# fpthink/3D-WSIS

Hardware: AMD Instinct MI355X
Metric: scenes/sec fwd+bwd ScanNet 2cm (~150k voxels) @1/8 GPU; HBM GB/s vs roofline (higher is better)
Workload: dtype f32; 1 GPU; C2: 1 synthetic ScanNet-shaped scene on 1 GPU, 2 cm voxels, fwd+bwd+AdamW step (SubMConv3d UNet 32..160 + ECC GNN + edge affinity + MultiTaskLoss); per-batch segment CSRs / edge graph and all rulebooks are rebuilt inside every step; active_voxels=153685, points=199790, superpoints=2289, edges=20054, scenes_per_gpu=1, global_batch=1, parallelism=scene-sharded dp1

## Files before the change

### 3d-wsis_amd/csrc/bn.hip

```cpp
#include <cstdlib>
#include <initializer_list>

#include "common.h"

using namespace wsis;

namespace {

constexpr int BN_ROWS_PER_THREAD = 8;
__host__ __device__ inline int bn_rows_per_wg(int Cp) {
  const int G = Cp >> 2;
  const int R = 256 / G > 1 ? 256 / G : 1;
  return R * BN_ROWS_PER_THREAD;
}
constexpr int BN_THREADS = 256;

struct f4 {
  float v[4];
};
template <typename T>
__device__ __forceinline__ float4 bn_ld4(const T* p, int64_t t) {
  if constexpr (sizeof(T) == 4) {
    return reinterpret_cast<const float4*>(p)[t];
  } else {
// ... 510 lines not shown
}

template <bool COHERENT, typename TI = float, typename TO = float>
__device__ __forceinline__ void bn_apply_body(const TI* __restrict__ x, const float* mean,
                                              const float* var, const float* __restrict__ gamma,
                                              const float* __restrict__ beta, float eps, int relu,
                                              TO* __restrict__ y, int64_t M, int C) {
  const int64_t total = M * C;
  if ((C & 3) == 0) {
    const int64_t total4 = total >> 2;
    const unsigned C4 = (unsigned)(C >> 2);
    const int64_t stride = (int64_t)gridDim.x * blockDim.x;
    int64_t t = blockIdx.x * (int64_t)blockDim.x + threadIdx.x;
    const bool fixed_c = (stride % C4) == 0;
    unsigned cg = (unsigned)(t % C4);
    float sc[4], mu[4], bt[4];
    auto coef = [&](unsigned g) {
#pragma unroll
      for (int e = 0; e < 4; ++e) {
        const int c = (int)g * 4 + e;
        sc[e] = bn_fwd_coef(gamma ? gamma[c] : 1.0f, bn_ld_stat<COHERENT>(var + c), eps);
        mu[e] = bn_ld_stat<COHERENT>(mean + c);
        bt[e] = beta ? beta[c] : 0.0f;
      }
    };
    coef(cg);
    auto body = [&](const float4 v) {
      float o[4] = {v.x, v.y, v.z, v.w};
#pragma unroll
      for (int e = 0; e < 4; ++e) o[e] = bn_fwd_elem(o[e], mu[e], sc[e], bt[e], relu);
      return make_float4(o[0], o[1], o[2], o[3]);
    };
    if (fixed_c) {
      for (; t + stride < total4; t += 2 * stride) {
        const float4 v0 = bn_ld4(x, t);
        const float4 v1 = bn_ld4(x, t + stride);
        bn_st4(y, t, body(v0));
        bn_st4(y, t + stride, body(v1));
      }
      if (t < total4) bn_st4(y, t, body(bn_ld4(x, t)));
    } else {
      for (; t < total4; t += stride) {
        cg = (unsigned)(t % C4);
        coef(cg);
        bn_st4(y, t, body(bn_ld4(x, t)));
      }
    }
  } else {
    for (int64_t t = blockIdx.x * (int64_t)blockDim.x + threadIdx.x; t < total;
         t += (int64_t)gridDim.x * blockDim.x) {
      const int c = (int)(t % C);
      const float sc = bn_fwd_coef(gamma ? gamma[c] : 1.0f, bn_ld_stat<COHERENT>(var + c), eps);
      y[t] = (TO)bn_fwd_elem((float)x[t], bn_ld_stat<COHERENT>(mean + c), sc, beta ? beta[c] : 0.0f, relu);
    }
  }
}

__global__ void bn_apply_kernel(const float* __restrict__ x, const float* __restrict__ mean,
                                const float* __restrict__ var, const float* __restrict__ gamma,
                                const float* __restrict__ beta, float eps, int relu, float* __restrict__ y,
                                int64_t M, int C) {
  bn_apply_body<false>(x, mean, var, gamma, beta, eps, relu, y, M, C);
}

template <typename TI, typename TO>
__global__ void bn_apply_lp_kernel(const TI* __restrict__ x, const float* __restrict__ mean,
                                   const float* __restrict__ var, const float* __restrict__ gamma,
                                   const float* __restrict__ beta, float eps, int relu, TO* __restrict__ y, int64_t M,
                                   int C) {
  bn_apply_body<false, TI, TO>(x, mean, var, gamma, beta, eps, relu, y, M, C);
}

template <typename TI>
void launch_bn_apply_lp(const void* x, const float* mean, const float* var, const float* gamma, const float* beta,
                        float eps, int relu, void* y, int out_fp32, int64_t M, int C, int grid, hipStream_t st) {
  if (out_fp32)
    hipLaunchKernelGGL((bn_apply_lp_kernel<TI, float>), dim3(grid), dim3(256), 0, st, static_cast<const TI*>(x), mean,
                       var, gamma, beta, eps, relu, static_cast<float*>(y), M, C);
  else
    hipLaunchKernelGGL((bn_apply_lp_kernel<TI, TI>), dim3(grid), dim3(256), 0, st, static_cast<const TI*>(x), mean, var,
                       gamma, beta, eps, relu, static_cast<TI*>(y), M, C);
}

template <bool COHERENT, typename T, typename TO>
__device__ __forceinline__ void bn_bwd_apply_body(const T* __restrict__ x, const T* __restrict__ dy,
                                                  const float* __restrict__ mean, const float* __restrict__ var,
                                                  const float* __restrict__ gamma, const float* __restrict__ beta,
                                                  const float* dgamma, const float* dbeta,
                                                  const T* __restrict__ addend, float eps, int relu, int training,
                                                  TO* __restrict__ dx, int64_t M, int C) {
  const int64_t total = M * C;
  const float inv_m = 1.0f / (float)M;
  const bool vec = (C & 3) == 0;
  const int W = vec ? 4 : 1;
  const int64_t totalw = total / W;
  const unsigned Cw = (unsigned)(C / W);
  const int64_t stride = (int64_t)gridDim.x * blockDim.x;
  int64_t t = blockIdx.x * (int64_t)blockDim.x + threadIdx.x;
  const bool fixed_c = (stride % Cw) == 0;
  BnBwdCoef k;
  float k1[4], k2[4];
  auto coef = [&](int c0) {
#pragma unroll
    for (int e = 0; e < 4; ++e) {
      if (e < W) {
        const int c = c0 + e;
        k.load(e, c, mean, var, gamma, beta, eps);
        k1[e] = training ? bn_ld_stat<COHERENT>(dbeta + c) * inv_m : 0.0f;
        k2[e] = training ? bn_ld_stat<COHERENT>(dgamma + c) * inv_m : 0.0f;
      }
    }
  };
  if (t < totalw) coef((int)(t % Cw) * W);
  auto one = [&](const float (&xv)[4], const float (&dv)[4], const float (&av)[4], float (&ov)[4]) {
#pragma unroll
    for (int e = 0; e < 4; ++e) {
      if (e < W)
        ov[e] = bn_bwd_dx(bn_bwd_elem(xv[e], dv[e], k, e, relu), k, e, k1[e], k2[e], training, addend != nullptr, av[e]);
    }
  };
  if (vec && fixed_c) {
    for (; t + stride < totalw; t += 2 * stride) {
      const int64_t u = t + stride;
      const f4 tx0 = ld4(x + t * 4, true), td0 = ld4(dy + t * 4, true);
      const f4 tx1 = ld4(x + u * 4, true), td1 = ld4(dy + u * 4, true);
      f4 ta0, ta1;
#pragma unroll
      for (int e = 0; e < 4; ++e) ta0.v[e] = ta1.v[e] = 0.f;
      if (addend) {
        ta0 = ld4(addend + t * 4, true);
        ta1 = ld4(addend + u * 4, true);
      }
      float o0[4], o1[4];
      one(tx0.v, td0.v, ta0.v, o0);
      one(tx1.v, td1.v, ta1.v, o1);
      bn_st4(dx, t, make_float4(o0[0], o0[1], o0[2], o0[3]));
      bn_st4(dx, u, make_float4(o1[0], o1[1], o1[2], o1[3]));
    }
  }
  for (; t < totalw; t += stride) {
    if (!fixed_c) coef((int)(t % Cw) * W);
    float xv[4], dv[4], av[4] = {0.f, 0.f, 0.f, 0.f}, ov[4];
    if (vec) {
      const f4 tx = ld4(x + t * 4, true), td = ld4(dy + t * 4, true);
#pragma unroll
      for (int e = 0; e < 4; ++e) {
        xv[e] = tx.v[e];
        dv[e] = td.v[e];
      }
      if (addend) {
        const f4 ta = ld4(addend + t * 4, true);
#pragma unroll
        for (int e = 0; e < 4; ++e) av[e] = ta.v[e];
      }
    } else {
      xv[0] = (float)x[t];
      dv[0] = (float)dy[t];
      if (addend) av[0] = (float)addend[t];
    }
    one(xv, dv, av, ov);
    if (vec)
      bn_st4(dx, t, make_float4(ov[0], ov[1], ov[2], ov[3]));
    else
      dx[t] = (TO)ov[0];
  }
}

template <typename T, typename TO>
__global__ void bn_bwd_apply_kernel(const T* __restrict__ x, const T* __restrict__ dy,
                                    const float* __restrict__ mean, const float* __restrict__ var,
                                    const float* __restrict__ gamma, const float* __restrict__ beta,
                                    const float* __restrict__ dgamma, const float* __restrict__ dbeta,
                                    const T* __restrict__ addend, float eps, int relu, int training,
                                    TO* __restrict__ dx, int64_t M, int C) {
  bn_bwd_apply_body<false>(x, dy, mean, var, gamma, beta, dgamma, dbeta, addend, eps, relu, training, dx, M, C);
}

constexpr int BN_SF_ROWS = 256;

template <int NT>
__device__ __forceinline__ void bn_small_totals(const float* __restrict__ partial, int nblk, int C, int64_t M, int G, int c,
                                                bool own, double (&red)[NT][8][33], double (&T)[NT]) {
#pragma unroll
  for (int k = 0; k < NT; ++k) T[k] = 0.0;
  for (int g = 0; g < G; ++g) {
    int lo, hi;
    bn_chunk_range(nblk, G, g, lo, hi);
    double t[NT], Tg[NT];
#pragma unroll
    for (int k = 0; k < NT; ++k) t[k] = 0.0;
    bn_chunk_walk<NT>(partial, lo, hi, C, M, c, t);
    if (g) __syncthreads();
    bn_lane_fold<NT>(t, own, red, Tg);
    if (own) {
#pragma unroll
      for (int k = 0; k < NT; ++k) {
        if (G == 1)
          T[k] = Tg[k];
        else
          T[k] += Tg[k];
      }
    }
  }
}

__global__ __launch_bounds__(256) void bn_small_finish_apply_kernel(
    const float* __restrict__ partial, int nblk, int C, int64_t M, float* __restrict__ mean, float* __restrict__ var,
    float* __restrict__ running_mean, float* __restrict__ running_var, float momentum, const float* __restrict__ x,
    const float* __restrict__ gamma, const float* __restrict__ beta, float eps, int relu, float* __restrict__ y, int G) {
  __shared__ double red[3][8][33];
  __shared__ float s_mu[32], s_sc[32], s_bt[32];
  const int cgi = blockIdx.y;
  const int cl = threadIdx.x & 31;
  const int c = cgi * 32 + cl;
  const bool own = (threadIdx.x >> 5) == 0 && c < C;
  double T[3];
  bn_small_totals<3>(partial, nblk, C, M, G, c, own, red, T);
  if (own) {
    const BnMeanVar s = bn_centred_mean_var(T[0], T[1], T[2], M);
    if (blockIdx.x == 0) bn_store_stats(s, M, c, mean, var, running_mean, running_var, momentum);
    s_mu[cl] = (float)s.mu;
    s_sc[cl] = bn_fwd_coef(gamma ? gamma[c] : 1.0f, (float)s.v, eps);
    s_bt[cl] = beta ? beta[c] : 0.0f;
  }
  __syncthreads();
  const int q4 = threadIdx.x & 7, rl = threadIdx.x >> 3;
  const int c4 = cgi * 32 + q4 * 4;
  if (c4 >= C) return;
  float mu4[4], sc4[4], bt4[4];
#pragma unroll
  for (int e = 0; e < 4; ++e) {
    mu4[e] = s_mu[q4 * 4 + e];
    sc4[e] = s_sc[q4 * 4 + e];
    bt4[e] = s_bt[q4 * 4 + e];
  }
  const int64_t r0 = (int64_t)blockIdx.x * BN_SF_ROWS;
#pragma unroll 4
  for (int it = 0; it < BN_SF_ROWS / 32; ++it) {
    const int64_t r = r0 + it * 32 + rl;
    if (r < M) {
      const float4 vx = *reinterpret_cast<const float4*>(x + r * C + c4);
      float o[4] = {vx.x, vx.y, vx.z, vx.w};
#pragma unroll
      for (int e = 0; e < 4; ++e) o[e] = bn_fwd_elem(o[e], mu4[e], sc4[e], bt4[e], relu);
      *reinterpret_cast<float4*>(y + r * C + c4) = make_float4(o[0], o[1], o[2], o[3]);
    }
  }
}

__global__ __launch_bounds__(256) void bn_small_bwd_finish_apply_kernel(
    const float* __restrict__ partial, int nblk, int C, int64_t M, const float* __restrict__ x,
    const float* __restrict__ dy, const float* __restrict__ mean, const float* __restrict__ var,
    const float* __restrict__ gamma, const float* __restrict__ beta, const float* __restrict__ addend, float eps, int relu,
    float* __restrict__ dx, float* __restrict__ dgamma, float* __restrict__ dbeta, int G) {
  __shared__ double red[2][8][33];
  __shared__ float s_k1[32], s_k2[32];
  const int cgi = blockIdx.y;
  const int cl = threadIdx.x & 31;
  const int c = cgi * 32 + cl;
  const bool own = (threadIdx.x >> 5) == 0 && c < C;
  double T[2];
  bn_small_totals<2>(partial, nblk, C, M, G, c, own, red, T);
  if (own) {
    const float db = (float)T[0], dg = (float)T[1];
    if (blockIdx.x == 0) {
      dbeta[c] = db;
      dgamma[c] = dg;
    }
    const float inv_m = 1.0f / (float)M;
    s_k1[cl] = db * inv_m;
    s_k2[cl] = dg * inv_m;
  }
  __syncthreads();
  const int q4 = threadIdx.x & 7, rl = threadIdx.x >> 3;
  const int c4 = cgi * 32 + q4 * 4;
  if (c4 >= C) return;
  BnBwdCoef k;
  float k1[4], k2[4];
#pragma unroll
  for (int e = 0; e < 4; ++e) {
    k.load(e, c4 + e, mean, var, gamma, beta, eps);
    k1[e] = s_k1[q4 * 4 + e];
    k2[e] = s_k2[q4 * 4 + e];
  }
  const int64_t r0 = (int64_t)blockIdx.x * BN_SF_ROWS;
#pragma unroll 2
  for (int it = 0; it < BN_SF_ROWS / 32; ++it) {
    const int64_t r = r0 + it * 32 + rl;
    if (r < M) {
      const float4 vx = *reinterpret_cast<const float4*>(x + r * C + c4);
      const float4 vd = *reinterpret_cast<const float4*>(dy + r * C + c4);
      float4 va = make_float4(0.f, 0.f, 0.f, 0.f);
      if (addend) va = *reinterpret_cast<const float4*>(addend + r * C + c4);
      const float xv[4] = {vx.x, vx.y, vx.z, vx.w}, dv[4] = {vd.x, vd.y, vd.z, vd.w}, av[4] = {va.x, va.y, va.z, va.w};
      float ov[4];
#pragma unroll
      for (int e = 0; e < 4; ++e)
        ov[e] = bn_bwd_dx(bn_bwd_elem(xv[e], dv[e], k, e, relu), k, e, k1[e], k2[e], 1, addend != nullptr, av[e]);
      *reinterpret_cast<float4*>(dx + r * C + c4) = make_float4(ov[0], ov[1], ov[2], ov[3]);
    }
  }
}

static int bn_small_gmax() {
  const char* e = getenv("WSIS_BN_SMALL_G");
  const int g = e ? atoi(e) : 4;
  return g < 1 ? 1 : g > 8 ? 8 : g;
}
static bool bn_small_fused_on() {
  const char* e = getenv("WSIS_BN_SMALL_FUSED");
  return !e || atoi(e) != 0;
}

int bn_nblk(int64_t M, int Cp) { return (int)ceil_div(M > 0 ? M : 1, (int64_t)bn_rows_per_wg(Cp)); }

#if WSIS_EXPERIMENTAL
constexpr int BN_POLL_SLEEP = 12;
constexpr unsigned long long BN_SPIN_LIMIT = 200000000ull;

__device__ __forceinline__ void bn_wait_published(SyncSlot* s) {
  if (threadIdx.x == 0) {
    const unsigned long long t0 = __builtin_amdgcn_s_memrealtime();
    while (__hip_atomic_load(&s->flag, __ATOMIC_RELAXED, __HIP_MEMORY_SCOPE_AGENT) == 0u) {
      __builtin_amdgcn_s_sleep(BN_POLL_SLEEP);
      if (__builtin_amdgcn_s_memrealtime() - t0 > BN_SPIN_LIMIT) {
        __hip_atomic_store(&s->err, 1u, __ATOMIC_RELAXED, __HIP_MEMORY_SCOPE_AGENT);
        break;
      }
    }
    const unsigned l = atomicAdd(&s->left, 1u);
    if (l == gridDim.x - 1) {
      __hip_atomic_store(&s->left, 0u, __ATOMIC_RELAXED, __HIP_MEMORY_SCOPE_AGENT);
      __hip_atomic_store(&s->flag, 0u, __ATOMIC_RELAXED, __HIP_MEMORY_SCOPE_AGENT);
    }
  }
  __syncthreads();
}
__device__ __forceinline__ void bn_publish(bool fin, SyncSlot* s, int CG) {
  if (!fin) return;
  __threadfence();
  __syncthreads();
  if (threadIdx.x == 0) {
    const unsigned d = atomicAdd(&s->done, 1u);
    if (d == (unsigned)CG - 1) {
      __hip_atomic_store(&s->done, 0u, __ATOMIC_RELAXED, __HIP_MEMORY_SCOPE_AGENT);
      __threadfence();
      __hip_atomic_store(&s->flag, 1u, __ATOMIC_RELEASE, __HIP_MEMORY_SCOPE_AGENT);
    }
  }
}

__global__ __launch_bounds__(256) void bn_finalize_apply_kernel(
    const float* __restrict__ partial, int nblk, int C, int64_t M, double* __restrict__ chunk, int G,
    float* mean, float* var, float* __restrict__ running_mean,
    float* __restrict__ running_var, float momentum, SyncSlot* __restrict__ sync, const float* __restrict__ x,
    const float* __restrict__ gamma, const float* __restrict__ beta, float eps, int relu, float* __restrict__ y) {
  __shared__ double red[3][8][33];
  __shared__ int s_last;
  const int CG = (C + 31) / 32;
  if ((int)blockIdx.x < G * CG)
    bn_publish(bn_chunk_centred_stage(partial, nblk, C, M, chunk, mean, var, running_mean, running_var, momentum,
                                      sync->ticket, (int)blockIdx.x % G, G, (int)blockIdx.x / G, red, s_last),
               sync, CG);
  bn_wait_published(sync);
  bn_apply_body<true>(x, mean, var, gamma, beta, eps, relu, y, M, C);
}

__global__ __launch_bounds__(256) void bn_bwd_finish_apply_kernel(
    const float* __restrict__ partial, int nblk, int C, double* __restrict__ chunk, int G, float* dbeta, float* dgamma,
    SyncSlot* __restrict__ sync, const float* __restrict__ x, const float* __restrict__ dy, const float* __restrict__ mean,
    const float* __restrict__ var, const float* __restrict__ gamma, const float* __restrict__ beta,
    const float* __restrict__ addend, float eps, int relu, float* __restrict__ dx, int64_t M) {
  __shared__ double red[2][8][33];
  __shared__ int s_last;
  const int CG = (C + 31) / 32;
  if ((int)blockIdx.x < G * CG)
    bn_publish(bn_sum_chunk_stage(partial, nblk, C, chunk, dbeta, dgamma, sync->ticket, (int)blockIdx.x % G, G,
                                  (int)blockIdx.x / G, red, s_last),
               sync, CG);
  bn_wait_published(sync);
  bn_bwd_apply_body<true>(x, dy, mean, var, gamma, beta, dgamma, dbeta, addend, eps, relu, 1, dx, M, C);
}

static int bn_fused_grid(int64_t M, int C, int need_chunk_wgs, int which = 0) {
  const char* e = getenv("WSIS_BN_FUSED_APPLY");
  const int on = e ? atoi(e) : 0;
  const char* ed = getenv(which ? "WSIS_BN_FUSED_BWD" : "WSIS_BN_FUSED_FWD");
  const int on_dir = ed ? atoi(ed) : on;
  const char* g = tune_env("WSIS_BN_FUSED_GRID");
  int gmax = g ? atoi(g) : 256;
  if (gmax < 64 || gmax > 512) gmax = 256;
  int n_cu = 0;
  {
    int dev = 0, v = 0;
    n_cu = (hipGetDevice(&dev) == hipSuccess &&
            hipDeviceGetAttribute(&v, hipDeviceAttributeMultiprocessorCount, dev) == hipSuccess) ? v : 0;
  }
  if (!on_dir || (C & 3) != 0) return 0;
  const int cw = C >> 2;
  const int64_t work = (M * C) >> 2;
  int gcap = (work > 600000 && gmax == 256) ? 512 : gmax;
  if (gcap > 2 * n_cu) gcap = 2 * n_cu;
  if (gcap < 1) return 0;
  int grid = gcap - (gcap % cw);
  const int need = grid_for(work, 256);
  if (need < grid) {
    grid = need;
    if (grid > cw) grid -= grid % cw;
  }
  return (grid >= need_chunk_wgs && grid >= 1) ? grid : 0;
}
#endif


static int bn_apply_grid(int64_t M, int C) {
  const bool vec = (C & 3) == 0;
  const int64_t work = vec ? (M * C) >> 2 : M * C;
  const int cw = vec ? C >> 2 : C;
  int64_t g = ceil_div(work, (int64_t)256 * 8);
  if (g < 512) {
    g = ceil_div(work, 256);
    if (g > 512) g = 512;
  }
  if (g > 16384) g = 16384;
  if (g < 1) g = 1;
  if (g > cw) g -= g % cw;
  return (int)g;
}

template <typename T, typename TO>
static int launch_bn_bwd_apply(const T* d_x, const T* d_dy, const float* d_mean, const float* d_var,
                               const float* d_gamma, const float* d_beta, const float* d_dgamma, const float* d_dbeta,
                               const T* d_addend, float eps, int relu, int training, TO* d_dx, int64_t M, int C,
                               hipStream_t st) {
  hipLaunchKernelGGL((bn_bwd_apply_kernel<T, TO>), dim3(bn_apply_grid(M, C)), dim3(256), 0, st, d_x, d_dy, d_mean, d_var,
                     d_gamma, d_beta, d_dgamma, d_dbeta, d_addend, eps, relu, training, d_dx, M, C);
  WSIS_LAUNCH_CHECK();
  return WSIS_OK;
}

template <typename T>
static int bn_stats_run(const T* d_x, int64_t M, int C, float* d_mean, float* d_var, float* d_running_mean,
                        float* d_running_var, float momentum, void* d_ws, hipStream_t st) {
  const int Cp = (C + 3) / 4 * 4;
  const int nblk = bn_nblk(M, Cp);
  float* partial = static_cast<float*>(d_ws);
  WSIS_REQUIRE(Cp / 4 <= BN_THREADS, "C > 1024 is not supported");
  if (M <= bn_small_rows()) {
    hipLaunchKernelGGL(bn_stats_small_kernel<T>, dim3(Cp / 4), dim3(BN_SMALL_THREADS), 0, st, d_x, M, C, d_mean, d_var,
                       d_running_mean, d_running_var, momentum);
    WSIS_LAUNCH_CHECK();
    return WSIS_OK;
  }
  hipLaunchKernelGGL(bn_stats_partial_kernel<T>, dim3(nblk), dim3(BN_THREADS), 0, st, d_x, M, C, Cp, partial);
  WSIS_LAUNCH_CHECK();
  hipLaunchKernelGGL(bn_stats_final_kernel<T>, dim3(C), dim3(64), 0, st, partial, nblk, C, Cp, M, d_x, d_mean, d_var,
                     d_running_mean, d_running_var, momentum);
  WSIS_LAUNCH_CHECK();
  return WSIS_OK;
}
template <typename T>
static int bn_bwd_reduce_run(const T* d_x, const T* d_dy, const float* d_mean, const float* d_var, const float* d_gamma,
                             const float* d_beta, float eps, int relu, float* d_dgamma, float* d_dbeta, int64_t M, int C,
                             void* d_ws, hipStream_t st) {
  const int Cp = (C + 3) / 4 * 4;
  const int nblk = bn_nblk(M, Cp);
  float* partial = static_cast<float*>(d_ws);
  WSIS_REQUIRE(Cp / 4 <= BN_THREADS, "C > 1024 is not supported");
  if (M <= bn_small_rows()) {
    hipLaunchKernelGGL(bn_bwd_small_kernel<T>, dim3(Cp / 4), dim3(BN_SMALL_THREADS), 0, st, d_x, d_dy, d_mean, d_var,
                       d_gamma, d_beta, eps, relu, M, C, d_dgamma, d_dbeta);
    WSIS_LAUNCH_CHECK();
  } else {
    hipLaunchKernelGGL(bn_bwd_partial_kernel<T>, dim3(nblk), dim3(BN_THREADS), 0, st, d_x, d_dy, d_mean, d_var, d_gamma,
                       d_beta, eps, relu, M, C, Cp, partial);
    WSIS_LAUNCH_CHECK();
    hipLaunchKernelGGL(bn_bwd_final_kernel, dim3(C), dim3(64), 0, st, partial, nblk, C, Cp, d_dgamma, d_dbeta);
    WSIS_LAUNCH_CHECK();
  }
  return WSIS_OK;
}
template <typename T>
static int bn_bwd_lp_run(const void* d_x, const void* d_dy, const float* d_mean, const float* d_var, const float* d_gamma,
                         const float* d_beta, float eps, int relu, int training, void* d_dx, int out_fp32,
                         float* d_dgamma, float* d_dbeta, const void* d_addend, int64_t M, int C, void* d_ws,
                         hipStream_t st) {
  const T *x = static_cast<const T*>(d_x), *dy = static_cast<const T*>(d_dy), *ad = static_cast<const T*>(d_addend);
  const int rc = bn_bwd_reduce_run(x, dy, d_mean, d_var, d_gamma, d_beta, eps, relu, d_dgamma, d_dbeta, M, C, d_ws, st);
  if (rc != WSIS_OK || !d_dx) return rc;
  if (out_fp32)
    return launch_bn_bwd_apply(x, dy, d_mean, d_var, d_gamma, d_beta, d_dgamma, d_dbeta, ad, eps, relu, training,
                               static_cast<float*>(d_dx), M, C, st);
  return launch_bn_bwd_apply(x, dy, d_mean, d_var, d_gamma, d_beta, d_dgamma, d_dbeta, ad, eps, relu, training,
                             static_cast<T*>(d_dx), M, C, st);
}

static unsigned* bn_tickets(void* d_sync) {
  static const int on = [] {
    const char* e = tune_env("WSIS_BN_TICKET");
    return e ? atoi(e) : 1;
  }();
  if (!on || !d_sync) return nullptr;
  return static_cast<SyncSlot*>(d_sync)->ticket;
}

static bool bn_aligned16(std::initializer_list<const void*> ps) {
  for (const void* p : ps)
    if (reinterpret_cast<uintptr_t>(p) & 15) return false;
  return true;
}
static void* bn_align256(void* p) {
  return reinterpret_cast<void*>((reinterpret_cast<uintptr_t>(p) + 255) & ~(uintptr_t)255);
}

struct BnCentredPlan {
  int G, CG;
  bool ws_ok;
  double* chunk;
  unsigned* tickets;
};
static BnCentredPlan bn_centred_plan(int64_t n_part, int C, void* d_ws, int64_t ws_bytes, void* d_sync) {
  BnCentredPlan p;
  p.G = bn_fin_chunks(n_part);
  p.CG = (C + 31) / 32;
  p.ws_ok = p.G == 1 || (d_ws && ws_bytes >= wsis_bn_stats_finalize_workspace_bytes(n_part, C));
  p.chunk = static_cast<double*>(bn_align256(d_ws));
  p.tickets = bn_tickets(d_sync);
  return p;
}
static bool bn_small_fused_ok(const BnCentredPlan& p, int C, std::initializer_list<const void*> rows) {
  return p.G <= bn_small_gmax() && (p.G == 1 || p.tickets) && (C & 3) == 0 && bn_small_fused_on() && bn_aligned16(rows);
}

}

extern "C" {

int64_t wsis_bn_workspace_bytes(int64_t M, int32_t C) {
  if (M < 0 || C < 1) return -1;
  const int64_t Cp = (C + 3) / 4 * 4;
  return (int64_t)bn_nblk(M, (int)Cp) * 2 * Cp * (int64_t)sizeof(float) + 256;
}

int wsis_bn_stats(const float* d_x, int64_t M, int32_t C, float* d_mean, float* d_var, float* d_running_mean,
                  float* d_running_var, float momentum, void* d_ws, int64_t ws_bytes, void* stream) {
  WSIS_REQUIRE(M >= 1 && C >= 1 && d_x && d_mean && d_var && d_ws, "bad args");
  WSIS_REQUIRE(ws_bytes >= wsis_bn_workspace_bytes(M, C), "workspace too small");
  WSIS_REQUIRE((d_running_mean == nullptr) == (d_running_var == nullptr), "running stats come in pairs");
  return bn_stats_run(d_x, M, C, d_mean, d_var, d_running_mean, d_running_var, momentum, d_ws, as_stream(stream));
}

static bool bn_lp_domain(int C, int dtype, std::initializer_list<const void*> ps) {
  return (dtype == 0 || dtype == 1) && C % 8 == 0 && C <= 1024 && bn_aligned16(ps);
}

int wsis_bn_stats_lp(const void* d_x, int64_t M, int32_t C, float* d_mean, float* d_var, float* d_running_mean,
                     float* d_running_var, float momentum, void* d_ws, int64_t ws_bytes, int32_t dtype, void* stream) {
  WSIS_REQUIRE(M >= 1 && C >= 1 && d_x && d_mean && d_var && d_ws, "bad args");
  WSIS_REQUIRE(bn_lp_domain(C, dtype, {d_x}), "16-bit BatchNorm: dtype 0 / 1, C % 8 == 0, C <= 1024, 16-byte aligned x");
  WSIS_REQUIRE(ws_bytes >= wsis_bn_workspace_bytes(M, C), "workspace too small");
  WSIS_REQUIRE((d_running_mean == nullptr) == (d_running_var == nullptr), "running stats come in pairs");
  hipStream_t st = as_stream(stream);
  if (dtype == 0)
    return bn_stats_run(static_cast<const __bf16*>(d_x), M, C, d_mean, d_var, d_running_mean, d_running_var, momentum,
                        d_ws, st);
  return bn_stats_run(static_cast<const _Float16*>(d_x), M, C, d_mean, d_var, d_running_mean, d_running_var, momentum,
                      d_ws, st);
}


__device__ __forceinline__ void colsum_block(const bool IN, const bool OUT, const float* __restrict__ x, int64_t lo,
                                             int64_t hi, int C4, float4* red, float* __restrict__ out) {
  const int RL = 256 / C4;
  const int cl = threadIdx.x % C4, rl = threadIdx.x / C4;
  float4 a = {0.f, 0.f, 0.f, 0.f};
  if (rl < RL) {
    const float4* x4 = reinterpret_cast<const float4*>(x);
#pragma unroll 8
    for (int64_t r = lo + rl; r < hi; r += RL) {
      float4 v;
      if (IN) {
        const float* p = x + (r * C4 + cl) * 4;
        v = make_float4(ld_sc1(p), ld_sc1(p + 1), ld_sc1(p + 2), ld_sc1(p + 3));
      } else {
        v = x4[r * C4 + cl];
      }
      a.x += v.x;
      a.y += v.y;
      a.z += v.z;
      a.w += v.w;
    }
    red[rl * C4 + cl] = a;
  }
  __syncthreads();
  if (threadIdx.x < C4) {
// ... 63 lines not shown
  const BnCentredPlan p = bn_centred_plan(n_part, C, d_ws, ws_bytes, d_sync);
  WSIS_REQUIRE(p.ws_ok, "workspace too small");
  WSIS_REQUIRE(C <= 512, "more than 512 channels");
  hipLaunchKernelGGL(bn_stats_chunk_centred_kernel, dim3(p.G, p.CG), dim3(256), 0, as_stream(stream), d_partials,
                     (int)n_part, C, M, p.chunk, d_mean, d_var, d_running_mean, d_running_var, momentum, p.tickets);
  WSIS_LAUNCH_CHECK();
  if (p.G > 1 && !p.tickets) {
    hipLaunchKernelGGL(bn_stats_final_centred_kernel, dim3((C + 3) / 4), dim3(256), 0, as_stream(stream), p.chunk, p.G, C,
                       M, d_mean, d_var, d_running_mean, d_running_var, momentum);
    WSIS_LAUNCH_CHECK();
  }
  return WSIS_OK;
}

int wsis_bn_stats_finalize_apply(const float* d_partials, int64_t n_part, int64_t M, int32_t C, float* d_mean,
                                 float* d_var, float* d_running_mean, float* d_running_var, float momentum,
                                 const float* d_x, const float* d_gamma, const float* d_beta, float eps, int32_t relu,
                                 float* d_y, void* d_ws, int64_t ws_bytes, void* d_sync, void* stream) {
  WSIS_REQUIRE(n_part >= 1 && M >= 1 && C >= 1 && d_partials && d_mean && d_var && d_x && d_y, "bad args");
  WSIS_REQUIRE(n_part == (M + 31) / 32 && n_part < ((int64_t)1 << 31), "one partial per 32-row slice");
  WSIS_REQUIRE(C <= 512, "more than 512 channels");
  hipStream_t st = as_stream(stream);
  const BnCentredPlan p = bn_centred_plan(n_part, C, d_ws, ws_bytes, d_sync);
  WSIS_REQUIRE(p.ws_ok, "workspace too small");
  if (bn_small_fused_ok(p, C, {d_x, d_y})) {
    hipLaunchKernelGGL(bn_small_finish_apply_kernel, dim3((unsigned)ceil_div(M, BN_SF_ROWS), (unsigned)p.CG), dim3(256), 0,
                       st, d_partials, (int)n_part, (int)C, M, d_mean, d_var, d_running_mean, d_running_var, momentum, d_x,
                       d_gamma, d_beta, eps, (int)relu, d_y, p.G);
    WSIS_LAUNCH_CHECK();
    return WSIS_OK;
  }
#if WSIS_EXPERIMENTAL
  if (const int grid = p.tickets ? bn_fused_grid(M, C, p.G * p.CG) : 0) {
    hipLaunchKernelGGL(bn_finalize_apply_kernel, dim3(grid), dim3(256), 0, st, d_partials, (int)n_part, (int)C, M, p.chunk,
                       p.G, d_mean, d_var, d_running_mean, d_running_var, momentum, static_cast<SyncSlot*>(d_sync), d_x,
                       d_gamma, d_beta, eps, (int)relu, d_y);
    WSIS_LAUNCH_CHECK();
    return WSIS_OK;
  }
#endif
  const int rc = wsis_bn_stats_finalize(d_partials, n_part, M, C, d_mean, d_var, d_running_mean, d_running_var, momentum,
                                        d_ws, ws_bytes, d_sync, stream);
  if (rc != WSIS_OK) return rc;
  return wsis_bn_apply(d_x, d_mean, d_var, d_gamma, d_beta, eps, relu, d_y, M, C, stream);
}

int wsis_bn_apply(const float* d_x, const float* d_mean, const float* d_var, const float* d_gamma,
                  const float* d_beta, float eps, int32_t relu, float* d_y, int64_t M, int32_t C, void* stream) {
  WSIS_REQUIRE(M >= 0 && C >= 1, "bad sizes");
  if (M == 0) return WSIS_OK;
  WSIS_REQUIRE(d_x && d_mean && d_var && d_y, "null pointer");
  hipLaunchKernelGGL(bn_apply_kernel, dim3(bn_apply_grid(M, C)), dim3(256), 0, as_stream(stream), d_x, d_mean, d_var,
                     d_gamma, d_beta, eps, relu, d_y, M, C);
  WSIS_LAUNCH_CHECK();
  return WSIS_OK;
}

int wsis_bn_apply_lp(const void* d_x, const float* d_mean, const float* d_var, const float* d_gamma,
                     const float* d_beta, float eps, int32_t relu, void* d_y, int32_t out_fp32, int64_t M, int32_t C,
                     int32_t dtype, void* stream) {
  WSIS_REQUIRE(M >= 0 && C >= 1, "bad sizes");
  WSIS_REQUIRE(dtype == 0 || dtype == 1, "dtype must be 0 (bf16) or 1 (fp16)");
  if (M == 0) return WSIS_OK;
  WSIS_REQUIRE(d_x && d_mean && d_var && d_y, "null pointer");
  const int grid = bn_apply_grid(M, C);
  if ((C & 3) == 0)
    WSIS_REQUIRE((reinterpret_cast<uintptr_t>(d_x) & 7) == 0 &&
                     (reinterpret_cast<uintptr_t>(d_y) & (out_fp32 ? 15 : 7)) == 0,
                 "x and y must be aligned to a quad of elements");
  hipStream_t st = as_stream(stream);
  if (dtype == 0)
    launch_bn_apply_lp<__bf16>(d_x, d_mean, d_var, d_gamma, d_beta, eps, relu, d_y, out_fp32, M, C, grid, st);
  else
    launch_bn_apply_lp<_Float16>(d_x, d_mean, d_var, d_gamma, d_beta, eps, relu, d_y, out_fp32, M, C, grid, st);
  WSIS_LAUNCH_CHECK();
  return WSIS_OK;
}

int wsis_bn_bwd_from_partials(const float* d_partials, int64_t n_part, const float* d_x, const float* d_dy,
                              const float* d_mean, const float* d_var, const float* d_gamma, const float* d_beta,
                              float eps, int32_t relu, float* d_dx, float* d_dgamma, float* d_dbeta,
                              const float* d_addend, int64_t M, int32_t C, void* d_ws, int64_t ws_bytes, void* d_sync,
                              void* stream) {
  WSIS_REQUIRE(M >= 1 && C >= 1 && d_partials && d_x && d_dy && d_mean && d_var && d_dgamma && d_dbeta, "bad args");
  WSIS_REQUIRE(n_part == (M + 31) / 32 && n_part < ((int64_t)1 << 31), "one partial per 32-row slice");
  const BnCentredPlan p = bn_centred_plan(n_part, C, d_ws, ws_bytes, d_sync);
  WSIS_REQUIRE(p.ws_ok, "workspace too small");
  hipStream_t st = as_stream(stream);
  WSIS_REQUIRE(C <= 512, "more than 512 channels");
  if (d_dx && bn_small_fused_ok(p, C, {d_x, d_dy, d_dx, d_addend})) {
    hipLaunchKernelGGL(bn_small_bwd_finish_apply_kernel, dim3((unsigned)ceil_div(M, BN_SF_ROWS), (unsigned)p.CG), dim3(256),
                       0, st, d_partials, (int)n_part, (int)C, M, d_x, d_dy, d_mean, d_var, d_gamma, d_beta, d_addend, eps,
                       (int)relu, d_dx, d_dgamma, d_dbeta, p.G);
    WSIS_LAUNCH_CHECK();
    return WSIS_OK;
  }
#if WSIS_EXPERIMENTAL
  if (const int grid = d_dx && p.tickets ? bn_fused_grid(M, C, p.G * p.CG, 1) : 0) {
    hipLaunchKernelGGL(bn_bwd_finish_apply_kernel, dim3(grid), dim3(256), 0, st, d_partials, (int)n_part, (int)C, p.chunk,
                       p.G, d_dbeta, d_dgamma, static_cast<SyncSlot*>(d_sync), d_x, d_dy, d_mean, d_var, d_gamma, d_beta,
                       d_addend, eps, (int)relu, d_dx, M);
    WSIS_LAUNCH_CHECK();
    return WSIS_OK;
  }
#endif
  hipLaunchKernelGGL(bn_sum_chunk_kernel, dim3(p.G, p.CG), dim3(256), 0, st, d_partials, (int)n_part, C, p.chunk, d_dbeta,
                     d_dgamma, p.tickets);
  WSIS_LAUNCH_CHECK();
  if (p.G > 1 && !p.tickets) {
    hipLaunchKernelGGL(bn_sum_final_kernel, dim3((C + 3) / 4), dim3(256), 0, st, p.chunk, p.G, C, d_dbeta, d_dgamma);
    WSIS_LAUNCH_CHECK();
  }
  if (!d_dx) return WSIS_OK;
  return launch_bn_bwd_apply(d_x, d_dy, d_mean, d_var, d_gamma, d_beta, d_dgamma, d_dbeta, d_addend, eps, relu, 1, d_dx, M,
                             C, st);
}

int wsis_bn_bwd_apply(const float* d_x, const float* d_dy, const float* d_mean, const float* d_var,
                      const float* d_gamma, const float* d_beta, const float* d_sum_dz_xhat, const float* d_sum_dz,
                      float eps, int32_t relu, float* d_dx, const float* d_addend, int64_t M, int32_t C, void* stream) {
  WSIS_REQUIRE(M >= 1 && C >= 1 && d_x && d_dy && d_mean && d_var && d_sum_dz_xhat && d_sum_dz && d_dx, "bad args");
  return launch_bn_bwd_apply(d_x, d_dy, d_mean, d_var, d_gamma, d_beta, d_sum_dz_xhat, d_sum_dz, d_addend, eps, relu, 1,
                             d_dx, M, C, as_stream(stream));
}

int wsis_bn_bwd(const float* d_x, const float* d_dy, const float* d_mean, const float* d_var,
                const float* d_gamma, const float* d_beta, float eps, int32_t relu, int32_t training,
                float* d_dx, float* d_dgamma, float* d_dbeta, const float* d_addend, int64_t M, int32_t C, void* d_ws,
                int64_t ws_bytes, void* stream) {
  WSIS_REQUIRE(M >= 1 && C >= 1 && d_x && d_dy && d_mean && d_var && d_dgamma && d_dbeta && d_ws, "bad args");
  WSIS_REQUIRE(ws_bytes >= wsis_bn_workspace_bytes(M, C), "workspace too small");
  hipStream_t st = as_stream(stream);
  const int rc = bn_bwd_reduce_run(d_x, d_dy, d_mean, d_var, d_gamma, d_beta, eps, relu, d_dgamma, d_dbeta, M, C, d_ws, st);
  if (rc != WSIS_OK || !d_dx) return rc;
  return launch_bn_bwd_apply(d_x, d_dy, d_mean, d_var, d_gamma, d_beta, d_dgamma, d_dbeta, d_addend, eps, relu, training,
                             d_dx, M, C, st);
}

int wsis_bn_bwd_lp(const void* d_x, const void* d_dy, const float* d_mean, const float* d_var, const float* d_gamma,
                   const float* d_beta, float eps, int32_t relu, int32_t training, void* d_dx, int32_t out_fp32,
                   float* d_dgamma, float* d_dbeta, const void* d_addend, int64_t M, int32_t C, int32_t dtype, void* d_ws,
                   int64_t ws_bytes, void* stream) {
  WSIS_REQUIRE(M >= 1 && C >= 1 && d_x && d_dy && d_mean && d_var && d_dgamma && d_dbeta && d_ws, "bad args");
  WSIS_REQUIRE(bn_lp_domain(C, dtype, {d_x, d_dy, d_dx, d_addend}),
               "16-bit BatchNorm: dtype 0 / 1, C % 8 == 0, C <= 1024, 16-byte aligned tensors");
  WSIS_REQUIRE(ws_bytes >= wsis_bn_workspace_bytes(M, C), "workspace too small");
  hipStream_t st = as_stream(stream);
  if (dtype == 0)
    return bn_bwd_lp_run<__bf16>(d_x, d_dy, d_mean, d_var, d_gamma, d_beta, eps, relu, training, d_dx, out_fp32, d_dgamma,
                                 d_dbeta, d_addend, M, C, d_ws, st);
  return bn_bwd_lp_run<_Float16>(d_x, d_dy, d_mean, d_var, d_gamma, d_beta, eps, relu, training, d_dx, out_fp32, d_dgamma,
                                 d_dbeta, d_addend, M, C, d_ws, st);
}

int64_t wsis_sync_bytes(void) { return (int64_t)kSyncSlotsTotal * (int64_t)sizeof(SyncSlot); }

int64_t wsis_colsum_workspace_bytes(int64_t M, int32_t C) {
  if (M < 0 || C < 4) return -1;
  int64_t per, G;
  colsum_plan(M, &per, &G);
  return (G > 1 ? G : 1) * (int64_t)C * (int64_t)sizeof(float) + 256;
}

int wsis_colsum(const float* d_x, int64_t M, int32_t C, float* d_out, void* d_ws, int64_t ws_bytes, void* d_sync,
                void* stream) {
  WSIS_REQUIRE(M >= 0 && C >= 4 && C % 4 == 0 && C <= 1024 && d_out, "colsum: C must be a multiple of 4, <= 1024");
  hipStream_t st = as_stream(stream);
  if (M == 0) {
    WSIS_HIP_CHECK(hipMemsetAsync(d_out, 0, sizeof(float) * (size_t)C, st));
    return WSIS_OK;
  }
  WSIS_REQUIRE(d_x && bn_aligned16({d_x, d_out}), "colsum: 16-byte alignment");
  int64_t per, G;
  colsum_plan(M, &per, &G);
  float* chunk = nullptr;
  unsigned* ticket = nullptr;
  if (G > 1) {
    WSIS_REQUIRE(d_ws && ws_bytes >= wsis_colsum_workspace_bytes(M, C), "workspace too small");
    chunk = static_cast<float*>(bn_align256(d_ws));
    WSIS_REQUIRE(d_sync, "colsum over more than one chunk needs a sync slot");
    ticket = static_cast<SyncSlot*>(d_sync)->ticket;
  }
  hipLaunchKernelGGL(colsum_kernel, dim3((unsigned)G), dim3(256), 0, st, d_x, M, (int)C, per, chunk, d_out, ticket);
  WSIS_LAUNCH_CHECK();
  return WSIS_OK;
}

}
```

### 3d-wsis_amd/csrc/common.h

```cpp
#pragma once
#include <hip/hip_runtime.h>
#include <hip/hip_ext.h>
#include <cstdlib>

#include <cstdint>
#include <cstdio>
#include <string>
#include <vector>

#include "../../include/wsis_hip.h"

namespace wsis {
inline const char* tune_env(const char* name) {
#if WSIS_EXPERIMENTAL
  return getenv(name);
#else
  (void)name;
  return nullptr;
#endif
}
inline int tune_int(const char* name, int dflt) {
  const char* e = tune_env(name);
  return e ? atoi(e) : dflt;
}
// ... 59 lines not shown
  void bracket() {
    if (exact && stage == 1) {
      exact = false;
      stage = hipEventRecord(r.a, st) == hipSuccess ? 1 : 0;
    }
  }
  hipEvent_t ka() const { return (exact && stage == 1) ? r.a : nullptr; }
  hipEvent_t kb() const { return (exact && stage == 1) ? r.b : nullptr; }
  void stop() {
    if (stage == 1) {
      if (!exact) (void)hipEventRecord(r.b, st);
      stage = 2;
    }
  }
  void tail() {
    if (stage == 2 && hipEventCreate(&r.c) == hipSuccess) (void)hipEventRecord(r.c, st);
  }
  ~ProfScope() {
    if (stage == 2) g_prof[which].push_back(r);
  }
};


#ifdef __HIPCC__
__device__ __forceinline__ void st_sc1(float* p, float v) { __hip_atomic_store(p, v, __ATOMIC_RELAXED, __HIP_MEMORY_SCOPE_AGENT); }
__device__ __forceinline__ void st_sc1(double* p, double v) { __hip_atomic_store(p, v, __ATOMIC_RELAXED, __HIP_MEMORY_SCOPE_AGENT); }
__device__ __forceinline__ float ld_sc1(const float* p) {
  return __hip_atomic_load(const_cast<float*>(p), __ATOMIC_RELAXED, __HIP_MEMORY_SCOPE_AGENT);
}
__device__ __forceinline__ double ld_sc1(const double* p) {
  return __hip_atomic_load(const_cast<double*>(p), __ATOMIC_RELAXED, __HIP_MEMORY_SCOPE_AGENT);
}
__device__ __forceinline__ void wait_stores_left() { asm volatile("s_waitcnt vmcnt(0)" ::: "memory"); }
#endif

struct SyncSlot {
  unsigned ticket[16];
  unsigned done, flag, left, err;
  unsigned ctr[44];
  unsigned fin[960];
};
static_assert(sizeof(SyncSlot) == 4096, "sync slot layout");
constexpr int kSyncSlots = 64;
constexpr int kSyncSlotsTotal = kSyncSlots + 1;
inline SyncSlot* sync_slot(void* d_sync, int i) {
  return d_sync ? static_cast<SyncSlot*>(d_sync) + (i % kSyncSlots) : nullptr;
}
inline void* deep_sync_slot(void* d_sync) { return d_sync ? static_cast<SyncSlot*>(d_sync) + kSyncSlots : nullptr; }

struct BnMeanVar {
  double mu, v;
};
__device__ __forceinline__ void bn_store_stats(BnMeanVar s, int64_t M, int c, float* mean, float* var, float* running_mean,
                                               float* running_var, float momentum) {
  const double n = (double)M;
  mean[c] = (float)s.mu;
  var[c] = (float)s.v;
  if (running_mean) {
    const double unb = n > 1 ? s.v * n / (n - 1) : s.v;
    running_mean[c] = (float)((1.0 - momentum) * running_mean[c] + momentum * s.mu);
    running_var[c] = (float)((1.0 - momentum) * running_var[c] + momentum * unb);
  }
}
__device__ __forceinline__ BnMeanVar bn_centred_mean_var(double S, double Q, double W, int64_t M) {
  const double n = (double)M;
  const double mu = S / n;
  double v = (Q + (W - n * mu * mu)) / n;
  if (v < 0.0) v = 0.0;
  return {mu, v};
}
__device__ __forceinline__ void bn_finish_centred(double S, double Q, double W, int64_t M, int c, float* mean, float* var,
                                                  float* running_mean, float* running_var, float momentum) {
  bn_store_stats(bn_centred_mean_var(S, Q, W, M), M, c, mean, var, running_mean, running_var, momentum);
}

constexpr int kBnFinChunks = 64;
inline int bn_fin_chunks(int64_t n_part) {
  int64_t g = n_part / 64;
  if (g < 1) g = 1;
  if (g > kBnFinChunks) g = kBnFinChunks;
  return (int)g;
}

bool spconv_in_supported(int K, int Cin, int Cout);
int spconv_in_launch(const float* d_X, const int32_t* d_nbr, const int32_t* d_order, const float* d_W, const float* d_bias,
                     const float* d_residual, float* d_out, int64_t M_out, hipEvent_t ka, hipEvent_t kb, hipStream_t st);

int64_t spconv_in_dw_workspace_bytes(int64_t M_out);
int spconv_in_dw_launch(const float* d_X, const int32_t* d_nbr, const int32_t* d_order, const float* d_dY, float* d_dW,
                        int64_t M_out, void* d_ws, hipEvent_t ka, hipEvent_t kb, hipStream_t st);

int spconv_ring_plan(int64_t M_out, int K, int Cin, int Cout);
int spconv_ring_launch(int nt, const float* d_X, const int32_t* d_nbr, const int32_t* d_order, const float* d_WT, int flip,
                       const float* d_bias, const float* d_residual, float* d_out, float* d_stats, const void* epi,
                       unsigned* d_err, int64_t M_in, int64_t M_out, int K, int Cin, int Cout, hipEvent_t ka, hipEvent_t kb, hipStream_t st,
                       unsigned long long* d_dbg = nullptr);

bool dw2_supported(int K, int Cin, int Cout);
bool dw2_fits(int64_t M_in, int64_t M_out, int K, int Cin, int Cout);
int64_t dw2_workspace_bytes(int64_t M_out, int K, int Cin, int Cout);
void dw2_set_batch_rows(int64_t rows);
int64_t dw2_batch_rows();
struct DwRedRec {
  const float* partial = nullptr;
  float* dW = nullptr;
  int64_t total4 = 0;
  int32_t P = 0;
};
void dw2_set_defer(DwRedRec* slot);
int dw2_reduce_batch(const DwRedRec* recs, int n, hipStream_t st);
int dw2_launch(const float* d_X, const int32_t* d_nbr, const int32_t* d_order, const float* d_dY, float* d_dW,
               int64_t M_in, int64_t M_out, int K, int Cin, int Cout, void* d_ws, hipStream_t st);
int dw2_launch_swapped(const float* d_X, const float* d_mean, const float* d_var, const float* d_gamma, const float* d_beta,
                       float eps, int relu, const int32_t* d_nbr_b, const int32_t* d_order_b, int flip, const float* d_dY,
                       float* d_dW, int64_t M_in, int64_t M_out, int K, int Cin, int Cout, void* d_ws, hipStream_t st);

#ifdef __HIPCC__
struct RowCol {
  int64_t row;
  int col;
};
__device__ __forceinline__ RowCol row_col(int64_t t, int C, int64_t total) {
  RowCol rc;
  if ((C & (C - 1)) == 0) {
    const int sh = __ffs(C) - 1;
    rc.row = t >> sh;
    rc.col = (int)(t & (C - 1));
  } else if (total < ((int64_t)1 << 32)) {
    const uint32_t q = (uint32_t)t / (uint32_t)C;
    rc.row = q;
    rc.col = (int)((uint32_t)t - q * (uint32_t)C);
  } else {
    rc.row = t / C;
    rc.col = (int)(t - rc.row * C);
  }
  return rc;
}
#endif

constexpr int64_t kEmptyKey = -1;

__device__ __forceinline__ uint64_t mix64(uint64_t x) {
  x ^= x >> 33;
  x *= 0xff51afd7ed558ccdULL;
  x ^= x >> 33;
  x *= 0xc4ceb9fe1a85ec53ULL;
  x ^= x >> 33;
  return x;
}

__device__ __forceinline__ int32_t hash_lookup(const int64_t* __restrict__ keys,
                                               const int32_t* __restrict__ vals, uint64_t mask,
                                               int64_t key) {
  uint64_t h = mix64((uint64_t)key) & mask;
  for (;;) {
    int64_t k = keys[h];
    if (k == key) return vals[h];
    if (k == kEmptyKey) return -1;
    h = (h + 1) & mask;
  }
}

}
```

### 3d-wsis_amd/csrc/executor.hip

```cpp
#include <condition_variable>
#include <cstdlib>
#include <deque>
#include <map>
#include <mutex>
#include <string>
#include <thread>
#include <utility>
#include <vector>

#include <unistd.h>

#include <algorithm>

#include "common.h"
#if WSIS_EXPERIMENTAL
#include "deep.h"
#endif

using namespace wsis;

namespace {

constexpr int64_t ALIGN = 256;
inline int64_t up(int64_t v) { return (v + ALIGN - 1) / ALIGN * ALIGN; }
// ... 191 lines not shown
    std::lock_guard<std::mutex> lock(mu_);
    const long pid = (long)getpid();
    if (started_ && pid_ != pid) {
      started_ = false;
      q_.clear();
      st_.clear();
    }
    if (!started_) {
      started_ = true;
      pid_ = pid;
      std::thread(&DwWorker::run, this).detach();
    }
    t.owner = std::this_thread::get_id();
    q_.push_back(t);
    ++st_[t.owner].pending;
    cv_.notify_one();
  }
  int drain(std::string* msg) {
    const std::thread::id me = std::this_thread::get_id();
    std::unique_lock<std::mutex> lock(mu_);
    done_.wait(lock, [&] { return st_[me].pending == 0; });
    State& s = st_[me];
    const int rc = s.err;
    if (rc != WSIS_OK && msg) *msg = s.msg;
    s.err = WSIS_OK;
    s.msg.clear();
    return rc;
  }

 private:
  struct State {
    int pending = 0, err = WSIS_OK;
    std::string msg;
  };
  void run() {
    for (;;) {
      DwTask t;
      {
        std::unique_lock<std::mutex> lock(mu_);
        cv_.wait(lock, [this] { return !q_.empty(); });
        t = q_.front();
        q_.pop_front();
      }
      int rc = WSIS_OK;
      std::string msg;
      hipError_t he = hipSetDevice(t.dev);
      if (he == hipSuccess && t.ev) he = hipStreamWaitEvent(t.side, t.ev, 0);
      if (he != hipSuccess) {
        rc = WSIS_ERR_HIP;
        msg = std::string("dW worker: ") + hipGetErrorString(he);
      } else {
        rc = t.flush ? dw2_reduce_batch(t.flush, t.flush_n, t.side) : issue_dw(t.op, t.ws, t.ws_bytes, t.side, t.rec);
        if (rc != WSIS_OK) msg = wsis_last_error();
      }
      std::lock_guard<std::mutex> lock(mu_);
      State& s = st_[t.owner];
      if (rc != WSIS_OK && s.err == WSIS_OK) {
        s.err = rc;
        s.msg = msg;
      }
      if (--s.pending == 0) done_.notify_all();
    }
  }
  std::mutex mu_;
  std::condition_variable cv_, done_;
  std::deque<DwTask> q_;
  std::map<std::thread::id, State> st_;
  bool started_ = false;
  long pid_ = 0;
};
DwWorker& dw_worker() {
  static DwWorker* w = new DwWorker();
  return *w;
}
struct PassOptions {
  bool fwd2;
  bool dw_stream;
  bool dw_thread;
  bool dw_batch_reduce;
  bool dw_tail_main;
  bool wt_side;
  bool dw_early;
  bool slab_bn_partials;
  bool prof;
  bool capturing;
  bool dw_defer() const { return dw_batch_reduce && !prof; }
};
inline bool env_flag(const char* e, bool dflt) { return e ? atoi(e) != 0 : dflt; }
PassOptions read_pass_options(const hipStream_t* st) {
  PassOptions o;
  o.fwd2 = env_flag(getenv("WSIS_FWD2"), true);
  o.dw_stream = env_flag(getenv("WSIS_DW_STREAM"), true);
  o.dw_thread = env_flag(tune_env("WSIS_DW_THREAD"), true);
  o.dw_batch_reduce = env_flag(getenv("WSIS_DW_BATCH_REDUCE"), false);
  o.dw_tail_main = env_flag(getenv("WSIS_DW_TAIL_MAIN"), true);
  o.wt_side = env_flag(getenv("WSIS_WT_SIDE"), true);
  const char* rows = getenv("WSIS_DW_EARLY_ROWS");
  o.dw_early = env_flag(getenv("WSIS_DW_EARLY"), dw2_batch_rows() < (rows ? atoll(rows) : 500000));
  o.slab_bn_partials = env_flag(getenv("WSIS_SLAB_BN_PARTIALS"), false);
  o.prof = g_prof_on;
  hipStreamCaptureStatus cs = hipStreamCaptureStatusNone;
  o.capturing = st && (hipStreamIsCapturing(*st, &cs) != hipSuccess || cs != hipStreamCaptureStatusNone);
  return o;
}
inline bool dw_tail_on_main(const wsis_op* ops, int n, int i) {
  return i == n - 1 && ops[i].kind == WSIS_OP_CONV_BWD && ops[i].out[1] && !ops[i].out[0];
}

inline int64_t wt_bytes_of(const wsis_op& op) {
  return up((int64_t)op.K * op.Cin * op.Cout * (int64_t)sizeof(float));
}

inline bool use_fwd2(const wsis_op& op, bool on) {
  const int64_t gathered = op.kind == WSIS_OP_CONV ? op.M_in * op.Cin : op.M_out * op.Cout;
  return on && wsis_spconv_fwd_t_supported(op.K, op.Cin, op.Cout) != 0 && gathered * 4 < ((int64_t)1 << 31);
}
inline bool needs_wt(const wsis_op& op, bool on) {
  if (op.flags & WSIS_OPF_LP) return false;
  if (op.kind == WSIS_OP_CONV) return use_fwd2(op, on);
  if (op.kind == WSIS_OP_CONV_BWD) return op.out[0] != nullptr && !use_fwd2(op, on);
  return false;
}

inline bool is_lp(const wsis_op& op) { return (op.flags & WSIS_OPF_LP) != 0; }
inline bool is_lp_conv(const wsis_op& op) {
  return is_lp(op) && (op.kind == WSIS_OP_CONV || (op.kind == WSIS_OP_CONV_BWD && op.out[0]));
}
inline int64_t lp_wt_bytes_of(const wsis_op& op) { return up((int64_t)op.K * op.Cin * op.Cout * 2); }
inline bool lp_below_2g(int64_t rows, int C) { return rows * C * 2 < ((int64_t)1 << 31); }
const char* lp_refusal(const wsis_op& op) {
  if (op.kind == WSIS_OP_CAST_LP && !is_lp(op)) return "CAST_LP without WSIS_OPF_LP (its dtype)";
  if (!is_lp(op)) return (op.flags & WSIS_OPF_LP_TRAIN) ? "WSIS_OPF_LP_TRAIN without WSIS_OPF_LP" : nullptr;
  const bool train_form = (op.kind == WSIS_OP_BN_RELU && (op.flags & WSIS_OPF_TRAINING)) || op.kind == WSIS_OP_BN_RELU_BWD ||
                          op.kind == WSIS_OP_CONV_BWD || op.kind == WSIS_OP_SPLIT;
  if (train_form && !(op.flags & WSIS_OPF_LP_TRAIN))
    return "16-bit training form (training BatchNorm, CONV_BWD, BN_RELU_BWD, SPLIT) without WSIS_OPF_LP_TRAIN";
  if (op.reserved != 0 && op.reserved != 1) return "16-bit op with a dtype other than 0 (bf16) or 1 (fp16)";
  if (op.flags & (WSIS_OPF_BN_IN | WSIS_OPF_STAT_FIN | WSIS_OPF_STATS))
    return "16-bit op with a fused BatchNorm form or epilogue statistics (16-bit passes run every BatchNorm as an op)";
  switch (op.kind) {
    case WSIS_OP_CONV:
      if (!wsis_spconv_lp_supported(op.K, op.Cin, op.Cout))
        return "16-bit convolution outside wsis_spconv_lp_supported (channels multiples of 32, at most 512)";
      if (op.M_in * op.Cin * 2 >= ((int64_t)1 << 31)) return "16-bit convolution input of 2 GiB or more";
      if (!op.in[3]) return "16-bit convolution without weights";
      return nullptr;
    case WSIS_OP_BN_RELU:
      if (!op.out[0]) return "16-bit BatchNorm without output";
      if (op.flags & WSIS_OPF_TRAINING) {
        if (!op.out[1] || !op.out[2]) return "16-bit training BatchNorm without mean / var outputs";
        if (op.Cin % 8 != 0 || op.Cin > 1024) return "16-bit training BatchNorm outside C % 8 == 0, C <= 1024";
        if ((op.flags & WSIS_OPF_UPDATE_RUNNING) && (!op.in[3] || !op.in[4]))
          return "16-bit BatchNorm updates running statistics it does not have";
        return nullptr;
      }
      if (op.flags & WSIS_OPF_UPDATE_RUNNING) return "16-bit evaluation BatchNorm with WSIS_OPF_UPDATE_RUNNING";
      if (!op.in[3] || !op.in[4]) return "16-bit evaluation BatchNorm without running statistics";
      return nullptr;
    case WSIS_OP_BN_RELU_BWD:
      if (op.Cin % 8 != 0 || op.Cin > 1024) return "16-bit BatchNorm backward outside C % 8 == 0, C <= 1024";
      if (!op.in[0] || !op.in[1] || !op.in[2] || !op.in[3] || !op.out[1] || !op.out[2])
        return "16-bit BatchNorm backward without x, dy, statistics or parameter-gradient outputs";
      return nullptr;
    case WSIS_OP_CAT:
    case WSIS_OP_SPLIT:
      if ((op.Cin | op.Cout) & 1) return "16-bit concatenation / split of an odd channel count";
      return nullptr;
    case WSIS_OP_CAST_LP:
      return nullptr;
    case WSIS_OP_CONV_BWD:
      if (!op.in[0] || !op.in[2]) return "16-bit backward convolution without X or dY";
      if (!lp_below_2g(op.M_out, op.Cout)) return "16-bit backward convolution with a dY of 2 GiB or more";
      if (op.out[0]) {
        if (!wsis_spconv_lp_supported(op.K, op.Cout, op.Cin))
          return "16-bit dIn product outside wsis_spconv_lp_supported (channels multiples of 32, at most 512)";
        if (!op.in[1]) return "16-bit dIn product without weights";
      }
      if (op.out[1] && (!wsis_spconv_lp_supported(op.K, op.Cin, op.Cout) || !lp_below_2g(op.M_in, op.Cin)))
        return "16-bit weight gradient outside wsis_spconv_lp_supported or with an input of 2 GiB or more";
      return nullptr;
    default:
      return "16-bit form of an op kind that has none";
  }
}

inline int64_t dw_ws_of(const wsis_op& op) {
  if (is_lp(op)) return up(wsis_spconv_dw_lp_workspace_bytes(op.M_out, op.K, op.Cin, op.Cout));
  if (op.flags & WSIS_OPF_BN_IN) return up(wsis_spconv_dw_bn_workspace_bytes(op.M_in, op.K, op.Cin, op.Cout));
  return up(wsis_spconv_dw_workspace_bytes(op.M_out, op.K, op.Cin, op.Cout));
}

int64_t op_ws_bytes(const wsis_op& op, bool on) {
  if (lp_refusal(op)) return -1;
  switch (op.kind) {
    case WSIS_OP_CONV:
      if (is_lp(op)) return up(wsis_spconv_fwd_lp_workspace_bytes(op.M_out, op.K, op.Cin, op.Cout));
#if WSIS_EXPERIMENTAL
      if (op.flags & (WSIS_OPF_BN_IN | WSIS_OPF_STAT_FIN))
        return up(std::max(wsis_spconv_fwd_f_workspace_bytes(op.M_out, op.K, op.Cin, op.Cout),
                           wsis_spconv_fwd_t_workspace_bytes(op.M_out, op.K, op.Cin, op.Cout)));
#else
      if (op.flags & (WSIS_OPF_BN_IN | WSIS_OPF_STAT_FIN)) return -1;
#endif
      if (use_fwd2(op, on)) return up(wsis_spconv_fwd_t_workspace_bytes(op.M_out, op.K, op.Cin, op.Cout));
      return up(wsis_spconv_fwd_workspace_bytes(op.M_out, op.K, op.Cin, op.Cout));
    case WSIS_OP_BN_RELU:
      if (!(op.flags & WSIS_OPF_TRAINING)) return 0;
      return up(std::max(wsis_bn_workspace_bytes(op.M_in, op.Cin),
                         wsis_bn_stats_finalize_workspace_bytes((op.M_in + 31) / 32, op.Cin)));
    case WSIS_OP_BN_RELU_BWD:
      return up(std::max(wsis_bn_workspace_bytes(op.M_in, op.Cin),
                         wsis_bn_stats_finalize_workspace_bytes((op.M_in + 31) / 32, op.Cin)));
    case WSIS_OP_CONV_BWD:
      if (!op.out[0]) return 0;
      if (is_lp(op)) return up(wsis_spconv_fwd_lp_workspace_bytes(op.M_in, op.K, op.Cout, op.Cin));
      if (use_fwd2(op, on)) return up(wsis_spconv_fwd_t_workspace_bytes(op.M_in, op.K, op.Cout, op.Cin));
      return up(wsis_spconv_fwd_workspace_bytes(op.M_in, op.K, op.Cout, op.Cin));
    default:
      return 0;
  }
}

inline int paired_bn(const wsis_op* ops, int n, int i) {
  const wsis_op& op = ops[i];
  for (int j = i + 1; j < n && j <= i + 4; ++j)
    if (ops[j].kind == WSIS_OP_BN_RELU_BWD && ops[j].in[1] == op.out[0] && (ops[j].flags & WSIS_OPF_STATS)) return j;
  return -1;
}

struct PassPlan {
  enum { LP, WT, DW, DEEP, OP, REGIONS };
  int64_t at[REGIONS], bytes[REGIONS], total = 0;
  std::vector<int64_t> lp_off, wt_off;
  int64_t dw_max = 0;
  int n_dw = 0;
};

struct PassRun {
  const wsis_op* ops;
  int n, mark_op;
  void *d_sync, *stream, *waiter_stream;
  hipStream_t st;
  PassOptions opt;
  PassPlan plan;
  char *base, *ws;
  int64_t ws_bytes;
  SideStream* side = nullptr;
  SideStream* wt_side = nullptr;
  bool wt_pending = false;
  bool forked = false;
  bool use_worker = false, worker_busy = false;
  int cur_dev = 0;
  std::vector<DwRedRec> dw_recs;
  int dw_next = 0, dw_flushed = 0;
  int64_t dw_off = 0;
  std::vector<char> bn_unfused;

  char* region(int k) const { return base + plan.at[k]; }
  const float* wt_of(int i) const { return reinterpret_cast<const float*>(region(PassPlan::WT) + plan.wt_off[i]); }
  int start();
  int fork_weight_transposes();
  int await_transposes_before(int i);
  int dw_issue(const wsis_op& op);
  int dw_flush();
  int drain_worker();
  int milestone();
  int finish(int first_err, bool defer_join);
};

#if WSIS_EXPERIMENTAL
inline int64_t deep_rows(const wsis_op& op) {
  switch (op.kind) {
    case WSIS_OP_CONV: return op.M_out;
    case WSIS_OP_CONV_BWD: return op.out[0] ? op.M_in : 0;
    default: return op.M_in;
  }
}
inline bool aligned16(const void* p) { return (reinterpret_cast<uintptr_t>(p) & 15) == 0; }

bool deep_op_ok(const wsis_op* ops, int n, int i, bool fwd2_on) {
  const wsis_op& op = ops[i];
  if (is_lp(op)) return false;
  const int64_t R = deep_max_rows();
  int nw = 0, zs = 0;
  switch (op.kind) {
    case WSIS_OP_CONV:
      if (op.flags & (WSIS_OPF_BN_IN | WSIS_OPF_STAT_FIN)) return false;
      if (!use_fwd2(op, fwd2_on) || op.M_out < 1 || op.M_out > R) return false;
      if ((int64_t)op.K * op.M_out * 4 >= ((int64_t)1 << 31)) return false;
      return deep_conv_plan(op.M_out, op.K, op.Cin, op.Cout, &nw, &zs) && aligned16(op.in[0]) && aligned16(op.out[0]);
    case WSIS_OP_CONV_BWD: {
      if (op.flags & WSIS_OPF_BN_IN) return false;
      if (!op.out[0]) return op.M_in <= R;
      if (!use_fwd2(op, fwd2_on) || op.M_in < 1 || op.M_in > R) return false;
      if (!deep_conv_plan(op.M_in, op.K, op.Cout, op.Cin, &nw, &zs)) return false;
      if (op.flags & WSIS_OPF_STATS) {
        const int j = paired_bn(ops, n, i);
        if (j < 0 || !ops[j].in[7] || ops[j].M_in != op.M_in || ops[j].Cin != op.Cin) return false;
      }
      return aligned16(op.in[2]) && aligned16(op.out[0]);
    }
    case WSIS_OP_BN_RELU:
      if (op.M_in < 1 || op.M_in > R || op.Cin % 32 || !deep_bn_rows_ok(op.M_in)) return false;
      if (op.flags & WSIS_OPF_TRAINING) {
        if (!(op.flags & WSIS_OPF_STATS) || !op.in[5]) return false;
        if (op.in[6] && (op.K % 32 || op.K <= 0 || op.K >= op.Cin)) return false;
      } else if (!op.out[0]) {
        return false;
      }
      return aligned16(op.in[0]) && (!op.out[0] || aligned16(op.out[0]));
    case WSIS_OP_BN_RELU_BWD:
      if (op.M_in < 1 || op.M_in > R || op.Cin % 32 || !deep_bn_rows_ok(op.M_in)) return false;
      if (!(op.flags & WSIS_OPF_TRAINING) || !(op.flags & WSIS_OPF_STATS) || !op.in[7]) return false;
      return aligned16(op.in[0]) && aligned16(op.in[1]) && aligned16(op.out[0]) && (!op.in[6] || aligned16(op.in[6]));
    case WSIS_OP_CAT:
      return op.M_in >= 1 && op.M_in <= R && vec4_ok(op, op.in[0], op.in[1], op.out[0]);
    case WSIS_OP_SPLIT:
      return op.M_in >= 1 && op.M_in <= R && vec4_ok(op, op.in[0], op.out[0], op.out[1]);
    default:
      return false;
  }
}

int deep_run_end(const wsis_op* ops, int n, int i0, int stop, bool fwd2_on) {
  int i1 = i0;
  while (i1 < n && (stop < 0 || i1 <= stop) && deep_op_ok(ops, n, i1, fwd2_on)) ++i1;
  for (int i = i0; i < i1; ++i)
    if (ops[i].kind == WSIS_OP_CONV_BWD && ops[i].out[0] && (ops[i].flags & WSIS_OPF_STATS)) {
      const int j = paired_bn(ops, n, i);
      if (j >= i1) {
        i1 = i;
        break;
      }
    }
  for (int j = i0; j < i1; ++j)
    if (ops[j].kind == WSIS_OP_BN_RELU_BWD) {
      bool found = false;
      for (int i = j - 1; i >= i0 && i >= j - 4 && !found; --i)
        found = ops[i].kind == WSIS_OP_CONV_BWD && ops[i].out[0] == ops[j].in[1] && (ops[i].flags & WSIS_OPF_STATS);
// ... 134 lines not shown
    const wsis_op& op = ops[i];
    DeepOp d{};
    d.NW = 1;
    d.ZS = 1;
    switch (op.kind) {
      case WSIS_OP_CONV:
      case WSIS_OP_CONV_BWD: {
        const int rc = deep_build_conv(b, ops, n, i);
        if (rc != WSIS_OK) return rc;
        break;
      }
      case WSIS_OP_BN_RELU: {
        const bool training = (op.flags & WSIS_OPF_TRAINING) != 0;
        const bool upd = (op.flags & WSIS_OPF_UPDATE_RUNNING) != 0;
        d.kind = DK_BN_FWD;
        d.training = training ? 1 : 0;
        d.relu = (op.flags & WSIS_OPF_RELU) ? 1 : 0;
        d.Cin = op.Cin;
        d.M_in = op.M_in;
        d.eps = op.eps;
        d.momentum = op.momentum;
        d.C0 = op.in[6] ? op.K : op.Cin;
        d.p[0] = op.in[0];
        d.p[1] = op.in[1];
        d.p[2] = op.in[2];
        d.p[3] = (training && !upd) ? nullptr : op.in[3];
        d.p[4] = (training && !upd) ? nullptr : op.in[4];
        d.p[5] = op.in[5];
        d.p[6] = op.in[6];
        d.p[7] = op.out[0];
        d.p[8] = op.out[1];
        d.p[9] = op.out[2];
        b.push(d);
        break;
      }
      case WSIS_OP_BN_RELU_BWD:
        d.kind = DK_BN_BWD;
        d.relu = (op.flags & WSIS_OPF_RELU) ? 1 : 0;
        d.Cin = op.Cin;
        d.M_in = op.M_in;
        d.eps = op.eps;
        d.p[0] = op.in[0];
        d.p[1] = op.in[1];
        d.p[2] = op.in[2];
        d.p[3] = op.in[3];
        d.p[4] = op.in[4];
        d.p[5] = op.in[5];
        d.p[6] = op.in[6];
        d.p[7] = op.in[7];
        d.p[8] = op.out[0];
        d.p[9] = op.out[1];
        d.p[10] = op.out[2];
        b.push(d);
        break;
      case WSIS_OP_CAT:
        d.kind = DK_CAT;
        d.Cin = op.Cin;
        d.Cout = op.Cout;
        d.M_in = op.M_in;
        d.p[0] = op.in[0];
        d.p[1] = op.in[1];
        d.p[2] = op.out[0];
        b.push(d);
        break;
      case WSIS_OP_SPLIT:
        d.kind = DK_SPLIT;
        d.Cin = op.Cin;
        d.Cout = op.Cout;
        d.M_in = op.M_in;
        d.p[0] = op.in[0];
        d.p[1] = op.out[0];
        d.p[2] = op.out[1];
        b.push(d);
        break;
      default:
        return fail(WSIS_ERR_ARG, "deep: op %d of kind %d is not a phase", i, op.kind);
    }
  }
  return WSIS_OK;
}

int deep_issue_run(PassRun& r, int i, int* next) {
  *next = i;
  if (r.plan.bytes[PassPlan::DEEP] == 0 || !r.d_sync || r.opt.capturing || !deep_op_ok(r.ops, r.n, i, r.opt.fwd2)) return WSIS_OK;
  const int i1 = deep_run_end(r.ops, r.n, i, r.mark_op >= i ? r.mark_op : -1, r.opt.fwd2);
  if (i1 - i < kDeepMinOps) return WSIS_OK;
  *next = i1;
  std::vector<DeepOp> tab;
  std::vector<std::pair<int, std::pair<int, int>>> convs;
  char* const deep_ws = r.region(PassPlan::DEEP);
  char* slab = deep_ws + deep_table_bytes(i1 - i);
  int rc = deep_build(r.ops, r.n, i, i1, r.region(PassPlan::WT), r.plan.wt_off, slab, g_prof_on, tab, convs);
  if (rc != WSIS_OK) return rc;
  unsigned long long* d_stamps = nullptr;
  if (g_prof_on && !tab.empty()) {
    if (hipMalloc((void**)&d_stamps, (tab.size() + 1) * sizeof(unsigned long long)) != hipSuccess)
      return fail(WSIS_ERR_HIP, "deep: stamp buffer allocation failed");
    g_prof_bufs.push_back(d_stamps);
  }
  rc = deep_launch(tab.data(), (int)tab.size(), deep_ws, deep_sync_slot(r.d_sync), d_stamps, r.st);
  if (rc != WSIS_OK) return rc;
  if (d_stamps) {
    if (g_deep_log.size() > 64) g_deep_log.clear();
    g_deep_log.push_back({tab, d_stamps});
    for (const auto& cs : convs) {
      ProfRec p{};
      p.d_stamps = d_stamps;
      p.s0 = cs.second.first;
      p.sm = cs.second.first + 1;
      p.s1 = cs.second.second;
      g_prof[0].push_back(p);
    }
  }
  for (int k = i; k < i1 && rc == WSIS_OK; ++k)
    if (r.ops[k].kind == WSIS_OP_CONV_BWD && r.ops[k].out[1]) rc = r.dw_issue(r.ops[k]);
  return rc;
}

int issue_conv_fused_bn(PassRun& r, const wsis_op& op, int i) {
  if (r.plan.wt_off[i] < 0)
    return fail(WSIS_ERR_ARG, "op %d: fused BatchNorm requested from a convolution that is not on wsis_spconv_fwd_t", i);
  wsis_bn_in bi;
  bi.mean = (const float*)op.in[6];
  bi.var = (const float*)op.in[7];
  bi.gamma = (const float*)op.in[8];
  bi.beta = (const float*)op.in[9];
  bi.eps = op.eps;
  bi.relu = (op.flags & WSIS_OPF_RELU) ? 1 : 0;
  wsis_stat_target tg[2];
  int nt = 0;
  if (op.flags & WSIS_OPF_STAT_FIN) {
    tg[0].mean = (float*)op.out[2];
    tg[0].var = (float*)op.out[3];
    tg[0].running_mean = (float*)const_cast<void*>(op.in[10]);
    tg[0].running_var = (float*)const_cast<void*>(op.in[11]);
    tg[0].momentum = op.momentum;
    tg[0].reserved = 0;
    nt = 1;
    if (op.out[4]) {
      tg[1].mean = (float*)op.out[4];
      tg[1].var = (float*)op.out[5];
      tg[1].running_mean = (float*)op.out[6];
      tg[1].running_var = (float*)op.out[7];
      tg[1].momentum = op.momentum2;
      tg[1].reserved = 0;
      nt = 2;
    }
  }
  return wsis_spconv_fwd_f((const float*)op.in[0], (op.flags & WSIS_OPF_BN_IN) ? &bi : nullptr, (const int32_t*)op.in[1],
                           (const int32_t*)op.in[2], r.wt_of(i), 0, (const float*)op.in[4], (const float*)op.in[5],
                           (float*)op.out[0], (op.flags & WSIS_OPF_STATS) ? (float*)op.out[1] : nullptr, tg, nt, op.M_in,
                           op.M_out, op.K, op.Cin, op.Cout, r.ws, r.ws_bytes, sync_slot(r.d_sync, i), r.stream);
}

#else
inline int64_t deep_ws_bytes(const wsis_op*, int, bool) { return 0; }
inline int deep_issue_run(PassRun&, int i, int* next) {
  *next = i;
  return WSIS_OK;
}
inline int issue_conv_fused_bn(PassRun&, const wsis_op&, int i) {
  return fail(WSIS_ERR_ARG, "op %d: the fused BatchNorm forms of the convolution are in the EXPERIMENTAL build only", i);
}
#endif

int plan_pass(const wsis_op* ops, int n, const PassOptions& o, PassPlan& p) {
  p.lp_off.assign(n, -1);
  p.wt_off.assign(n, -1);
  int64_t lp = 0, wt = 0, dw_sum = 0, need = ALIGN;
  for (int i = 0; i < n; ++i) {
    const wsis_op& op = ops[i];
    const char* why = lp_refusal(op);
    if (why) return fail(WSIS_ERR_ARG, "wsis_run_ops: op %d: %s", i, why);
    int64_t b = op_ws_bytes(op, o.fwd2);
    if (b < 0) return fail(WSIS_ERR_ARG, "wsis_run_ops: op %d: a form this build does not run (fused BatchNorm: EXPERIMENTAL)", i);
    if (dw_tail_on_main(ops, n, i)) b = std::max(b, dw_ws_of(op));
    need = std::max(need, b);
    if (is_lp_conv(op)) {
      p.lp_off[i] = lp;
      lp += lp_wt_bytes_of(op);
    }
    if (needs_wt(op, o.fwd2)) {
      if (!(op.kind == WSIS_OP_CONV ? op.in[3] : op.in[1]))
        return fail(WSIS_ERR_ARG, "wsis_run_ops: op %d: convolution without weights", i);
      p.wt_off[i] = wt;
      wt += wt_bytes_of(op);
    }
    if (op.kind == WSIS_OP_CONV_BWD && op.out[1]) {
      const int64_t d = dw_ws_of(op);
      p.dw_max = std::max(p.dw_max, d);
      dw_sum += d;
      ++p.n_dw;
    }
  }
  const int64_t sizes[PassPlan::REGIONS] = {lp, wt, o.dw_batch_reduce ? dw_sum : p.dw_max, deep_ws_bytes(ops, n, o.fwd2),
                                            need + ALIGN};
  p.total = 0;
  for (int k = 0; k < PassPlan::REGIONS; ++k) {
    p.at[k] = p.total;
    p.bytes[k] = sizes[k];
    p.total += sizes[k];
  }
  return WSIS_OK;
}

template <typename T>
int launch_weight_batches(const wsis_op* ops, int n, const std::vector<int64_t>& off, char* base, hipStream_t st) {
  constexpr bool lp = sizeof(T) == 2;
  WtBatch b;
  b.n = 0;
  b.start[0] = 0;
  int dtype = 0;
  auto flush = [&]() -> int {
    if (b.n == 0) return WSIS_OK;
    if (!lp)
      hipLaunchKernelGGL(weight_transpose_batch_kernel<float>, dim3(b.start[b.n]), dim3(256), 0, st, b);
    else if (dtype == 0)
      hipLaunchKernelGGL(weight_transpose_batch_kernel<__bf16>, dim3(b.start[b.n]), dim3(256), 0, st, b);
    else
      hipLaunchKernelGGL(weight_transpose_batch_kernel<_Float16>, dim3(b.start[b.n]), dim3(256), 0, st, b);
    WSIS_LAUNCH_CHECK();
    b.n = 0;
    return WSIS_OK;
  };
  for (int i = 0; i < n; ++i) {
    if (off[i] < 0) continue;
    const wsis_op& op = ops[i];
    if (b.n == WT_MAX || (lp && b.n > 0 && op.reserved != dtype)) {
      const int rc = flush();
      if (rc != WSIS_OK) return rc;
    }
    const bool fwd = op.kind == WSIS_OP_CONV;
    dtype = op.reserved;
    b.src[b.n] = (const float*)(fwd ? op.in[3] : op.in[1]);
    b.dst[b.n] = base + off[i];
    b.K[b.n] = op.K;
    b.Cin[b.n] = op.Cin;
    b.Cout[b.n] = op.Cout;
    b.plain[b.n] = (lp && !fwd) ? 1 : 0;
    b.flip[b.n] = (!b.plain[b.n] && (lp || !fwd) && (op.flags & WSIS_OPF_FLIP)) ? 1 : 0;
    b.start[b.n + 1] = b.start[b.n] + op.K * ((op.Cin + WT_TILE - 1) / WT_TILE) * ((op.Cout + WT_TILE - 1) / WT_TILE);
    ++b.n;
  }
  return flush();
}

int PassRun::start() {
  side = (plan.dw_max > 0 && opt.dw_stream) ? side_stream_for(st) : nullptr;
  if (side) side->next = 0;
  use_worker = side != nullptr && opt.dw_thread && !opt.prof && !opt.capturing;
  if (use_worker && hipGetDevice(&cur_dev) != hipSuccess) return fail(WSIS_ERR_HIP, "hipGetDevice failed");
  dw_recs.resize((size_t)(opt.dw_defer() ? plan.n_dw : 0));
  bn_unfused.assign(n, 0);
  return launch_weight_batches<uint16_t>(ops, n, plan.lp_off, region(PassPlan::LP), st);
}

int PassRun::fork_weight_transposes() {
  bool any_wt = false;
  for (int i = 0; i < n && !any_wt; ++i) any_wt = plan.wt_off[i] >= 0;
  if (opt.wt_side && opt.dw_stream && !opt.capturing && any_wt && plan.wt_off[0] < 0 && !opt.prof &&
      plan.bytes[PassPlan::DEEP] == 0)
    wt_side = side_stream_for(st);
  if (wt_side) {
    hipError_t e = hipEventRecord(wt_side->wt_fork, st);
    if (e == hipSuccess) e = hipStreamWaitEvent(wt_side->stream, wt_side->wt_fork, 0);
    if (e != hipSuccess) return fail(WSIS_ERR_HIP, "weight-transpose fork failed: %s", hipGetErrorString(e));
  }
  int rc = launch_weight_batches<float>(ops, n, plan.wt_off, region(PassPlan::WT), wt_side ? wt_side->stream : st);
  if (wt_side) {
    const hipError_t e = hipEventRecord(wt_side->wt_done, wt_side->stream);
    wt_pending = e == hipSuccess;
    if (!wt_pending && rc == WSIS_OK) rc = fail(WSIS_ERR_HIP, "weight-transpose event failed: %s", hipGetErrorString(e));
  }
  return rc;
}

int PassRun::await_transposes_before(int i) {
  if (!wt_pending || plan.wt_off[i] < 0) return WSIS_OK;
  wt_pending = false;
  const hipError_t e = hipStreamWaitEvent(st, wt_side->wt_done, 0);
  return e == hipSuccess ? WSIS_OK : fail(WSIS_ERR_HIP, "weight-transpose join failed: %s", hipGetErrorString(e));
}

int PassRun::drain_worker() {
  if (!worker_busy) return WSIS_OK;
  worker_busy = false;
  std::string msg;
  const int wrc = dw_worker().drain(&msg);
  return wrc == WSIS_OK ? WSIS_OK : fail(wrc, "%s", msg.c_str());
}

int PassRun::dw_issue(const wsis_op& op) {
  void* dw_stream = stream;
  char* my_ws = region(PassPlan::DW);
  int64_t my_bytes = plan.dw_max;
  DwRedRec* rec = nullptr;
  if (opt.dw_defer() && dw_next < plan.n_dw) {
    my_bytes = dw_ws_of(op);
    my_ws += dw_off;
    dw_off += my_bytes;
    rec = &dw_recs[(size_t)dw_next++];
  }
  if (side) {
    hipEvent_t e = next_fork_event(side);
    hipError_t he = e ? hipEventRecord(e, st) : hipErrorOutOfMemory;
    if (he == hipSuccess && !use_worker) he = hipStreamWaitEvent(side->stream, e, 0);
    if (he != hipSuccess) return fail(WSIS_ERR_HIP, "dW side-stream fork failed: %s", hipGetErrorString(he));
    dw_stream = side->stream;
    forked = true;
    if (use_worker) {
      DwTask t;
      t.op = op;
      t.ev = e;
      t.dev = cur_dev;
      t.side = side->stream;
      t.ws = my_ws;
      t.ws_bytes = my_bytes;
      t.rec = rec;
      dw_worker().push(t);
      worker_busy = true;
      return WSIS_OK;
    }
  }
  return issue_dw(op, my_ws, my_bytes, dw_stream, rec);
}

int PassRun::dw_flush() {
  if (dw_flushed == dw_next) return WSIS_OK;
  const DwRedRec* recs = dw_recs.data() + dw_flushed;
  const int cnt = dw_next - dw_flushed;
  dw_flushed = dw_next;
  if (side && use_worker) {
    DwTask t;
    t.ev = nullptr;
    t.dev = cur_dev;
    t.side = side->stream;
// ... 90 lines not shown
                         op.momentum, r.ws, r.ws_bytes, r.stream);
  const int64_t n_part = (op.M_in + 31) / 32;
  const int C0 = op.in[6] ? op.K : op.Cin;
  if (!op.in[6] && op.out[0]) {
    *applied = true;
    return wsis_bn_stats_finalize_apply((const float*)op.in[5], n_part, op.M_in, op.Cin, (float*)op.out[1],
                                        (float*)op.out[2], rm, rv, op.momentum, (const float*)op.in[0],
                                        (const float*)op.in[1], (const float*)op.in[2], op.eps, relu_of(op),
                                        (float*)op.out[0], r.ws, r.ws_bytes, sync_slot(r.d_sync, i), r.stream);
  }
  int rc = wsis_bn_stats_finalize((const float*)op.in[5], n_part, op.M_in, C0, (float*)op.out[1], (float*)op.out[2], rm,
                                  rv, op.momentum, r.ws, r.ws_bytes, sync_slot(r.d_sync, i), r.stream);
  if (rc == WSIS_OK && op.in[6])
    rc = wsis_bn_stats_finalize((const float*)op.in[6], n_part, op.M_in, op.Cin - C0, (float*)op.out[1] + C0,
                                (float*)op.out[2] + C0, rm ? rm + C0 : nullptr, rv ? rv + C0 : nullptr, op.momentum,
                                r.ws, r.ws_bytes, sync_slot(r.d_sync, i), r.stream);
  return rc;
}

int bn_relu_launches(PassRun& r, const wsis_op& op, int i) {
  const bool training = (op.flags & WSIS_OPF_TRAINING) != 0;
  if (is_lp(op)) {
    if (training) {
      if (op.M_in <= 0) return WSIS_OK;
      const bool upd = (op.flags & WSIS_OPF_UPDATE_RUNNING) != 0;
      const int rc = wsis_bn_stats_lp(op.in[0], op.M_in, op.Cin, (float*)op.out[1], (float*)op.out[2],
                                      upd ? (float*)op.in[3] : nullptr, upd ? (float*)op.in[4] : nullptr, op.momentum, r.ws,
                                      r.ws_bytes, op.reserved, r.stream);
      if (rc != WSIS_OK) return rc;
    }
    return wsis_bn_apply_lp(op.in[0], (const float*)(training ? op.out[1] : op.in[3]),
                            (const float*)(training ? op.out[2] : op.in[4]), (const float*)op.in[1], (const float*)op.in[2],
                            op.eps, relu_of(op), op.out[0], (op.flags & WSIS_OPF_OUT_F32) ? 1 : 0, op.M_in, op.Cin,
                            op.reserved, r.stream);
  }
  if (training) {
    bool applied = false;
    const int rc = bn_training_stats(r, op, i, &applied);
    if (rc != WSIS_OK || applied) return rc;
  }
  if (!op.out[0]) return WSIS_OK;
  return wsis_bn_apply((const float*)op.in[0], (const float*)(training ? op.out[1] : op.in[3]),
                       (const float*)(training ? op.out[2] : op.in[4]), (const float*)op.in[1], (const float*)op.in[2],
                       op.eps, relu_of(op), (float*)op.out[0], op.M_in, op.Cin, r.stream);
}

int issue_bn_relu(PassRun& r, const wsis_op& op, int i) {
  ProfScope prof(2, r.st);
  const int rc = bn_relu_launches(r, op, i);
  prof.stop();
  return rc;
}

int issue_cat(PassRun& r, const wsis_op& op, int) {
  if (op.M_in <= 0) return WSIS_OK;
  wsis_op c = op;
  if (is_lp(op)) {
    c.Cin /= 2;
    c.Cout /= 2;
  }
  if (vec4_ok(c, c.in[0], c.in[1], c.out[0]))
    hipLaunchKernelGGL(cat_rows_kernel<4>, dim3(grid_for(c.M_in * (c.Cin + c.Cout) / 4, 256)), dim3(256), 0, r.st,
                       (const float*)c.in[0], (const float*)c.in[1], (float*)c.out[0], c.M_in, c.Cin, c.Cout);
  else
    hipLaunchKernelGGL(cat_rows_kernel<1>, dim3(grid_for(c.M_in * (c.Cin + c.Cout), 256)), dim3(256), 0, r.st,
                       (const float*)c.in[0], (const float*)c.in[1], (float*)c.out[0], c.M_in, c.Cin, c.Cout);
  return launch_status();
}

int issue_cast_lp(PassRun& r, const wsis_op& op, int) {
  const int64_t ne = op.M_in * op.Cin;
  if (ne <= 0) return WSIS_OK;
  const bool vec = ne % 4 == 0 && ((reinterpret_cast<uintptr_t>(op.in[0]) & 15) | (reinterpret_cast<uintptr_t>(op.out[0]) & 7)) == 0;
  const int64_t items = vec ? ne / 4 : ne;
  if (op.reserved == 0)
    hipLaunchKernelGGL(cast_lp_kernel<__bf16>, dim3(grid_for(items, 256)), dim3(256), 0, r.st, (const float*)op.in[0],
                       (__bf16*)op.out[0], ne, vec ? 1 : 0);
  else
    hipLaunchKernelGGL(cast_lp_kernel<_Float16>, dim3(grid_for(items, 256)), dim3(256), 0, r.st, (const float*)op.in[0],
                       (_Float16*)op.out[0], ne, vec ? 1 : 0);
  return launch_status();
}

int issue_split(PassRun& r, const wsis_op& op, int) {
  if (op.M_in <= 0) return WSIS_OK;
  wsis_op c = op;
  if (is_lp(op)) {
    c.Cin /= 2;
    c.Cout /= 2;
  }
  if (vec4_ok(c, c.in[0], c.out[0], c.out[1]))
    hipLaunchKernelGGL(split_rows_kernel<4>, dim3(grid_for(c.M_in * (c.Cin + c.Cout) / 4, 256)), dim3(256), 0, r.st,
                       (const float*)c.in[0], (float*)c.out[0], (float*)c.out[1], c.M_in, c.Cin, c.Cout);
  else
    hipLaunchKernelGGL(split_rows_kernel<1>, dim3(grid_for(c.M_in * (c.Cin + c.Cout), 256)), dim3(256), 0, r.st,
                       (const float*)c.in[0], (float*)c.out[0], (float*)c.out[1], c.M_in, c.Cin, c.Cout);
  return launch_status();
}

int issue_add(PassRun& r, const wsis_op& op, int) {
  if (op.M_in * op.Cin <= 0) return WSIS_OK;
  hipLaunchKernelGGL(add_inplace_kernel, dim3(grid_for(op.M_in * op.Cin, 256)), dim3(256), 0, r.st, (float*)op.out[0],
                     (const float*)op.in[0], op.M_in * op.Cin);
  return launch_status();
}

int issue_din(PassRun& r, const wsis_op& op, int i) {
  const float* dY = (const float*)op.in[2];
  const int32_t *nbr = (const int32_t*)op.in[5], *order = (const int32_t*)op.in[6];
  float* dX = (float*)op.out[0];
  const bool stats = (op.flags & WSIS_OPF_STATS) != 0;
  if (is_lp(op))
    return wsis_spconv_fwd_lp(op.in[2], nbr, order, r.region(PassPlan::LP) + r.plan.lp_off[i], flip_of(op), nullptr, op.out[0],
                              op.M_out, op.M_in, op.K, op.Cout, op.Cin, op.reserved, r.ws, r.ws_bytes, r.stream);
  if (r.plan.wt_off[i] >= 0) {
    if (stats)
      return fail(WSIS_ERR_ARG, "op %d: BatchNorm partials requested from a dIn pass that is not on wsis_spconv_fwd_t", i);
    return wsis_spconv_fwd(dY, nbr, order, r.wt_of(i), nullptr, nullptr, dX, op.M_out, op.M_in, op.K, op.Cout, op.Cin, r.ws,
                           r.ws_bytes, r.stream);
  }
  const int j = stats ? paired_bn(r.ops, r.n, i) : -1;
  if (stats && (j < 0 || !r.ops[j].in[7] || r.ops[j].M_in != op.M_in || r.ops[j].Cin != op.Cin))
    return fail(WSIS_ERR_ARG, "op %d: no BatchNorm backward takes the partials of this dIn pass", i);
  const bool unfused = stats && !r.opt.slab_bn_partials && wsis_spconv_fwd_t_slabs(op.M_in, op.K, op.Cout, op.Cin) > 1;
  if (unfused) r.bn_unfused[j] = 1;
  if (!stats || unfused)
    return wsis_spconv_fwd_t(dY, nbr, order, (const float*)op.in[1], flip_of(op), nullptr, nullptr, dX, nullptr, op.M_out,
                             op.M_in, op.K, op.Cout, op.Cin, r.ws, r.ws_bytes, sync_slot(r.d_sync, i), r.stream);
  const wsis_op& bn = r.ops[j];
  return wsis_spconv_fwd_t_bn(dY, nbr, order, (const float*)op.in[1], flip_of(op), dX, (float*)const_cast<void*>(bn.in[7]),
                              (const float*)bn.in[0], (const float*)bn.in[2], (const float*)bn.in[3], (const float*)bn.in[4],
                              (const float*)bn.in[5], bn.eps, relu_of(bn), op.M_out, op.M_in, op.K, op.Cout, op.Cin, r.ws,
                              r.ws_bytes, sync_slot(r.d_sync, i), r.stream);
}

int issue_conv_bwd(PassRun& r, const wsis_op& op, int i) {
  const bool early = r.opt.dw_early && op.out[1] && op.out[0] && r.side;
  int rc = early ? r.dw_issue(op) : WSIS_OK;
  if (rc == WSIS_OK && op.out[0]) rc = issue_din(r, op, i);
  if (rc != WSIS_OK || !op.out[1] || early) return rc;
  if (r.opt.dw_tail_main && r.side && dw_tail_on_main(r.ops, r.n, i))
    return issue_dw(op, r.ws, r.ws_bytes, r.stream, nullptr);
  return r.dw_issue(op);
}

int issue_bn_relu_bwd(PassRun& r, const wsis_op& op, int i) {
  ProfScope prof(2, r.st);
  int rc;
  if (is_lp(op)) {
    rc = op.M_in <= 0 ? WSIS_OK
                      : wsis_bn_bwd_lp(op.in[0], op.in[1], (const float*)op.in[2], (const float*)op.in[3],
                                       (const float*)op.in[4], (const float*)op.in[5], op.eps, relu_of(op),
                                       (op.flags & WSIS_OPF_TRAINING) ? 1 : 0, op.out[0], (op.flags & WSIS_OPF_OUT_F32) ? 1 : 0,
                                       (float*)op.out[1], (float*)op.out[2], op.in[6], op.M_in, op.Cin, op.reserved, r.ws,
                                       r.ws_bytes, r.stream);
  } else if ((op.flags & WSIS_OPF_STATS) && !r.bn_unfused[i]) {
    if (!op.in[7] || !(op.flags & WSIS_OPF_TRAINING))
      rc = fail(WSIS_ERR_ARG, "op %d: BatchNorm backward from partials needs in[7] and training mode", i);
    else
      rc = wsis_bn_bwd_from_partials((const float*)op.in[7], (op.M_in + 31) / 32, (const float*)op.in[0],
                                     (const float*)op.in[1], (const float*)op.in[2], (const float*)op.in[3],
                                     (const float*)op.in[4], (const float*)op.in[5], op.eps, relu_of(op), (float*)op.out[0],
                                     (float*)op.out[1], (float*)op.out[2], (const float*)op.in[6], op.M_in, op.Cin, r.ws,
                                     r.ws_bytes, sync_slot(r.d_sync, i), r.stream);
  } else {
    rc = wsis_bn_bwd((const float*)op.in[0], (const float*)op.in[1], (const float*)op.in[2], (const float*)op.in[3],
                     (const float*)op.in[4], (const float*)op.in[5], op.eps, relu_of(op),
                     (op.flags & WSIS_OPF_TRAINING) ? 1 : 0, (float*)op.out[0], (float*)op.out[1], (float*)op.out[2],
                     (const float*)op.in[6], op.M_in, op.Cin, r.ws, r.ws_bytes, r.stream);
  }
  prof.stop();
  return rc;
}

int issue_op(PassRun& r, const wsis_op& op, int i) {
  switch (op.kind) {
    case WSIS_OP_CONV: return issue_conv(r, op, i);
    case WSIS_OP_BN_RELU: return issue_bn_relu(r, op, i);
    case WSIS_OP_CAT: return issue_cat(r, op, i);
    case WSIS_OP_CAST_LP: return issue_cast_lp(r, op, i);
    case WSIS_OP_SPLIT: return issue_split(r, op, i);
    case WSIS_OP_ADD: return issue_add(r, op, i);
    case WSIS_OP_CONV_BWD: return issue_conv_bwd(r, op, i);
    case WSIS_OP_BN_RELU_BWD: return issue_bn_relu_bwd(r, op, i);
    default: return fail(WSIS_ERR_ARG, "wsis_run_ops: unknown op kind");
  }
}

int run_ops_impl(const wsis_op* ops, int32_t n, void* d_ws, int64_t ws_bytes, void* d_sync, void* stream, int32_t mark_op,
                 void* waiter_stream, bool defer_join = false) {
  WSIS_REQUIRE((ops || n == 0) && n >= 0, "bad op list");
  WSIS_REQUIRE(mark_op < n && (mark_op < 0 || waiter_stream), "bad milestone");
  PassRun r{ops, n, mark_op, d_sync, stream, waiter_stream, as_stream(stream)};
  r.opt = read_pass_options(&r.st);
  int err = plan_pass(ops, n, r.opt, r.plan);
  if (err != WSIS_OK) return err;
  WSIS_REQUIRE((n == 0 || ws_bytes >= r.plan.total) && (d_ws || n == 0), "workspace too small");
  r.base = static_cast<char*>(d_ws);
  r.ws = r.region(PassPlan::OP);
  r.ws_bytes = ws_bytes - r.plan.at[PassPlan::OP];
  err = r.start();
  if (err != WSIS_OK) return err;
  err = r.fork_weight_transposes();
  for (int i = 0; i < n && err == WSIS_OK; ++i) {
    err = r.await_transposes_before(i);
    int next = i;
    if (err == WSIS_OK) err = deep_issue_run(r, i, &next);
    if (err == WSIS_OK && next == i) err = issue_op(r, ops[i], i);
    if (next > i) i = next - 1;
    if (err == WSIS_OK && i == mark_op) err = r.milestone();
  }
  return r.finish(err, defer_join);
}

}

__global__ void warm_stream_kernel(int* p) {
  if (p && threadIdx.x == 0xffff) p[0] = 0;
}

extern "C" {

int wsis_warm_streams(void* stream) {
  hipStream_t st = as_stream(stream);
  SideStream* side = side_stream_for(st);
  WSIS_REQUIRE(side != nullptr, "side stream creation failed");
  hipLaunchKernelGGL(warm_stream_kernel, dim3(1), dim3(64), 0, st, (int*)nullptr);
  hipLaunchKernelGGL(warm_stream_kernel, dim3(1), dim3(64), 0, side->stream, (int*)nullptr);
  WSIS_LAUNCH_CHECK();
  WSIS_HIP_CHECK(hipStreamSynchronize(side->stream));
  return WSIS_OK;
}

int64_t wsis_run_ops_workspace_bytes(const wsis_op* ops, int32_t n) {
  if (!ops || n < 0) return -1;
  PassPlan plan;
  return plan_pass(ops, n, read_pass_options(nullptr), plan) == WSIS_OK ? plan.total : -1;
}

int wsis_debug_run_ops_layout(const wsis_op* ops, int32_t n, int64_t* out) {
  WSIS_REQUIRE((ops || n == 0) && n >= 0 && out, "bad arguments");
  PassPlan plan;
  const int rc = plan_pass(ops, n, read_pass_options(nullptr), plan);
  if (rc != WSIS_OK) return rc;
  for (int k = 0; k < PassPlan::REGIONS; ++k) {
    out[2 * k] = plan.at[k];
    out[2 * k + 1] = plan.bytes[k];
  }
  out[10] = plan.total;
  std::copy(plan.lp_off.begin(), plan.lp_off.end(), out + 11);
  std::copy(plan.wt_off.begin(), plan.wt_off.end(), out + 11 + n);
  return WSIS_OK;
}

int wsis_run_ops(const wsis_op* ops, int32_t n, void* d_ws, int64_t ws_bytes, void* d_sync, void* stream) {
  return wsis_run_ops_marked(ops, n, d_ws, ws_bytes, d_sync, stream, -1, nullptr);
}

int wsis_run_ops_part(const wsis_op* ops, int32_t n, void* d_ws, int64_t ws_bytes, void* d_sync, void* stream, int32_t last) {
  return run_ops_impl(ops, n, d_ws, ws_bytes, d_sync, stream, -1, nullptr, last == 0);
}

int wsis_run_ops_marked(const wsis_op* ops, int32_t n, void* d_ws, int64_t ws_bytes, void* d_sync, void* stream,
                        int32_t mark_op, void* waiter_stream) {
#if !WSIS_EXPERIMENTAL
  return run_ops_impl(ops, n, d_ws, ws_bytes, d_sync, stream, mark_op, waiter_stream);
#else
  const char* ge = getenv("WSIS_GRAPH");
  const int graph_mode = ge ? atoi(ge) : 0;
  if (!graph_mode || mark_op >= 0 || g_prof_on || n == 0)
    return run_ops_impl(ops, n, d_ws, ws_bytes, d_sync, stream, mark_op, waiter_stream);
  hipStream_t st = as_stream(stream);
  static std::map<std::pair<hipStream_t, int64_t>, hipGraphExec_t> cache;
  static hipStream_t cap = nullptr;
  if (!cap) WSIS_HIP_CHECK(hipStreamCreateWithFlags(&cap, hipStreamNonBlocking));
  const int target = graph_mode >= 4 ? graph_mode : 1 << 30;
  int chunk_no = 0;
  for (int i0 = 0; i0 < n; ++chunk_no) {
    int i1 = i0, pending = 0;
    while (i1 < n) {
      const wsis_op& op = ops[i1];
      if (op.kind == WSIS_OP_CONV_BWD && (op.flags & WSIS_OPF_STATS) && op.out[0]) ++pending;
      if (op.kind == WSIS_OP_BN_RELU_BWD && (op.flags & WSIS_OPF_STATS) && pending > 0) --pending;
      ++i1;
      if (i1 - i0 >= target && pending == 0) break;
    }
    WSIS_HIP_CHECK(hipStreamBeginCapture(cap, hipStreamCaptureModeRelaxed));
    const int rc = run_ops_impl(ops + i0, i1 - i0, d_ws, ws_bytes, d_sync, cap, -1, nullptr);
    hipGraph_t g = nullptr;
    const hipError_t ec = hipStreamEndCapture(cap, &g);
    if (ec != hipSuccess || !g) return fail(WSIS_ERR_HIP, "graph capture failed: %s", hipGetErrorString(ec));
    if (rc != WSIS_OK) {
      (void)hipGraphDestroy(g);
      return rc;
    }
    const auto key = std::make_pair(st, ((int64_t)ops[0].kind * 4096 + n) * 64 + chunk_no);
    hipGraphExec_t& ex = cache[key];
    bool ready = false;
    if (ex) {
      hipGraphNode_t bad = nullptr;
      hipGraphExecUpdateResult res;
      if (hipGraphExecUpdate(ex, g, &bad, &res) == hipSuccess && res == hipGraphExecUpdateSuccess) {
        ready = true;
      } else {
        (void)hipGetLastError();
        (void)hipGraphExecDestroy(ex);
        ex = nullptr;
      }
    }
    if (!ready) {
      const hipError_t ei = hipGraphInstantiate(&ex, g, nullptr, nullptr, 0);
      if (ei != hipSuccess) {
        (void)hipGraphDestroy(g);
        ex = nullptr;
        return fail(WSIS_ERR_HIP, "graph instantiate failed: %s", hipGetErrorString(ei));
      }
    }
    const hipError_t el = hipGraphLaunch(ex, st);
    (void)hipGraphDestroy(g);
    if (el != hipSuccess) return fail(WSIS_ERR_HIP, "graph launch failed: %s", hipGetErrorString(el));
    i0 = i1;
  }
  return WSIS_OK;
#endif
}

#if WSIS_EXPERIMENTAL
int wsis_debug_deep_phases(int32_t which, int32_t* info, double* us, int32_t cap) {
  if (which < 0 || which >= (int)g_deep_log.size()) return -1;
  const auto& rec = g_deep_log[which];
  const int n = (int)rec.first.size();
  if (n > cap) return -1;
  std::vector<unsigned long long> t(n + 1);
  if (hipDeviceSynchronize() != hipSuccess) return -1;
  if (hipMemcpy(t.data(), rec.second, (n + 1) * sizeof(unsigned long long), hipMemcpyDeviceToHost) != hipSuccess) return -1;
// ... 19 lines not shown
```

### 3d-wsis_amd/csrc/spconv2.hip

```cpp
#include "spconv2_body.h"

namespace {

struct ItemMap {
  int bx, by, bz;
};
__host__ __device__ __forceinline__ ItemMap item_of(int i, int gx, int gy, int gz, int band) {
  const int total = gx * gy * gz;
  ItemMap m;
  const int per = gy * gz;
  if (band < 0) {
    const int C = -band, x = i & 7, q = i >> 3;
    const int nb = total / (8 * C);
    int j = i;
    if (q < nb * C) {
      const int sb = q / C, w = q - sb * C;
      j = (sb * 8 + x) * C + ((sb & 1) ? C - 1 - w : w);
    }
    m.bx = j / per;
    const int r = j - m.bx * per;
    m.by = r / gz;
    m.bz = r - m.by * gz;
    return m;
  }
// ... 143 lines not shown
  f.tr_ok = has_table && !bn_in && M_in < ((int64_t)1 << 24) && tune_int("WSIS_FWD2_TR", 1) != 0;
  f.TR = (f.tr_ok && p.NB == 1 && p.NW == 1 && p.DA == 2 && p.BD) ? 1 : 0;
  return f;
}
}

extern "C" {

int32_t wsis_spconv_fwd_t_supported(int32_t K, int32_t Cin, int32_t Cout) {
  return (K >= 1 && K <= KMAX && Cin >= 32 && Cin % 32 == 0 && Cout >= 32 && Cout % 32 == 0) ? 1 : 0;
}

int32_t wsis_spconv_fwd_t_slabs(int64_t M_out, int32_t K, int32_t Cin, int32_t Cout) {
  if (M_out < 1 || !wsis_spconv_fwd_t_supported(K, Cin, Cout)) return 0;
  return plan2(M_out, K, Cin, Cout).ZS;
}

int64_t wsis_spconv_fwd_t_workspace_bytes(int64_t M_out, int32_t K, int32_t Cin, int32_t Cout) {
  if (M_out < 0 || !wsis_spconv_fwd_t_supported(K, Cin, Cout)) return -1;
  const Plan2 p = plan2(M_out, K, Cin, Cout);
  return p.ZS <= 1 ? 256 : (int64_t)p.ZS * M_out * Cout * (int64_t)sizeof(float) + 256;
}

static int spconv_fwd_t_impl(const float* d_X, const int32_t* d_nbr, const int32_t* d_order, const float* d_WT,
                             int32_t flip, const float* d_bias, const float* d_residual, float* d_out, float* d_stats,
                             const BnEpi& epi, int64_t M_in, int64_t M_out, int32_t K, int32_t Cin, int32_t Cout,
                             void* d_ws, int64_t ws_bytes, void* d_sync, void* stream, const wsis_bn_in* bn_in = nullptr,
                             const wsis_stat_target* targets = nullptr, int32_t n_targets = 0, bool fused = false);

#if WSIS_EXPERIMENTAL
int64_t wsis_spconv_fwd_f_workspace_bytes(int64_t M_out, int32_t K, int32_t Cin, int32_t Cout) {
  if (M_out < 0 || !wsis_spconv_fwd_t_supported(K, Cin, Cout)) return -1;
  const int64_t n_part = (M_out + 31) / 32;
  return (int64_t)bn_fin_chunks(n_part) * (Cout / 32) * 96 * (int64_t)sizeof(double) + 256;
}

int wsis_spconv_fwd_f(const float* d_X, const wsis_bn_in* bn_in, const int32_t* d_nbr, const int32_t* d_order,
                      const float* d_WT, int32_t flip, const float* d_bias, const float* d_residual, float* d_out,
                      float* d_stats, const wsis_stat_target* targets, int32_t n_targets, int64_t M_in, int64_t M_out,
                      int32_t K, int32_t Cin, int32_t Cout, void* d_ws, int64_t ws_bytes, void* d_sync, void* stream) {
  WSIS_REQUIRE(n_targets >= 0 && n_targets <= 2 && (n_targets == 0 || (targets && d_stats && d_sync)),
               "statistics targets need the partial buffer and a sync slot");
  WSIS_REQUIRE(!bn_in || (bn_in->mean && bn_in->var), "input BatchNorm without statistics");
  return spconv_fwd_t_impl(d_X, d_nbr, d_order, d_WT, flip, d_bias, d_residual, d_out, d_stats, BnEpi{}, M_in, M_out, K,
                           Cin, Cout, d_ws, ws_bytes, d_sync, stream, bn_in, targets, n_targets, true);
}

#endif

int wsis_spconv_fwd_t(const float* d_X, const int32_t* d_nbr, const int32_t* d_order, const float* d_WT, int32_t flip,
                      const float* d_bias, const float* d_residual, float* d_out, float* d_stats, int64_t M_in,
                      int64_t M_out, int32_t K, int32_t Cin, int32_t Cout, void* d_ws, int64_t ws_bytes,
                      void* d_sync, void* stream) {
  return spconv_fwd_t_impl(d_X, d_nbr, d_order, d_WT, flip, d_bias, d_residual, d_out, d_stats, BnEpi{}, M_in, M_out, K,
                           Cin, Cout, d_ws, ws_bytes, d_sync, stream);
}

int wsis_spconv_fwd_t_bn(const float* d_X, const int32_t* d_nbr, const int32_t* d_order, const float* d_WT, int32_t flip,
                         float* d_out, float* d_partials, const float* d_bn_x, const float* d_bn_mean,
                         const float* d_bn_var, const float* d_bn_gamma, const float* d_bn_beta, float eps, int32_t relu,
                         int64_t M_in, int64_t M_out, int32_t K, int32_t Cin, int32_t Cout, void* d_ws, int64_t ws_bytes,
                         void* d_sync, void* stream) {
  WSIS_REQUIRE(d_partials && d_bn_x && d_bn_mean && d_bn_var, "null pointer");
  WSIS_REQUIRE((reinterpret_cast<uintptr_t>(d_bn_x) & 15) == 0, "bn_x must be 16-byte aligned");
  BnEpi epi;
  epi.x = d_bn_x;
  epi.mean = d_bn_mean;
  epi.var = d_bn_var;
  epi.gamma = d_bn_gamma;
  epi.beta = d_bn_beta;
  epi.eps = eps;
  epi.relu = relu;
  return spconv_fwd_t_impl(d_X, d_nbr, d_order, d_WT, flip, nullptr, nullptr, d_out, d_partials, epi, M_in, M_out, K,
                           Cin, Cout, d_ws, ws_bytes, d_sync, stream);
}

static int spconv_fwd_t_impl(const float* d_X, const int32_t* d_nbr, const int32_t* d_order, const float* d_WT,
                             int32_t flip, const float* d_bias, const float* d_residual, float* d_out, float* d_stats,
                             const BnEpi& epi, int64_t M_in, int64_t M_out, int32_t K, int32_t Cin, int32_t Cout,
                             void* d_ws, int64_t ws_bytes, void* d_sync, void* stream, const wsis_bn_in* bn_in,
                             const wsis_stat_target* targets, int32_t n_targets, bool fused) {
  WSIS_REQUIRE(M_in >= 0 && M_out >= 0, "bad sizes");
  WSIS_REQUIRE(wsis_spconv_fwd_t_supported(K, Cin, Cout), "needs K <= 32 and channel counts that are multiples of 32");
  if (M_out == 0) return WSIS_OK;
  WSIS_REQUIRE(d_X && d_WT && d_out, "null pointer");
  WSIS_REQUIRE(d_nbr || (K == 1 && M_in == M_out), "nbr may be null only for the dense 1x1 case");
  WSIS_REQUIRE(M_out < (int64_t)1 << 31 && M_in < (int64_t)1 << 31, "row count exceeds int32");
  WSIS_REQUIRE(M_in * Cin * 4 < (int64_t)1 << 31, "input tensor of 2 GiB or more (32-bit gather offsets): use wsis_spconv_fwd");
  const uint32_t x_bytes = (uint32_t)(M_in * Cin * 4);
  WSIS_REQUIRE(((reinterpret_cast<uintptr_t>(d_X) | reinterpret_cast<uintptr_t>(d_WT)) & 15) == 0,
               "X and WT must be 16-byte aligned");
  const Plan2 p = plan2(M_out, K, Cin, Cout, fused);
  float* partial = nullptr;
  if (p.ZS > 1) {
    WSIS_REQUIRE(d_ws && ws_bytes >= (int64_t)p.ZS * M_out * Cout * (int64_t)sizeof(float), "workspace too small");
    WSIS_REQUIRE((reinterpret_cast<uintptr_t>(d_ws) & 15) == 0, "workspace must be 16-byte aligned");
    partial = static_cast<float*>(d_ws);
  }
  BnIn bin{};
  if (bn_in) {
    bin.mean = bn_in->mean;
    bin.var = bn_in->var;
    bin.gamma = bn_in->gamma;
    bin.beta = bn_in->beta;
    bin.eps = bn_in->eps;
    bin.relu = bn_in->relu;
    WSIS_REQUIRE(p.NB == 1 && p.BD && p.ZS == 1, "fused input BatchNorm: plan without slabs expected");
  }
  StatFin fin{};
  if (n_targets > 0) {
    const int64_t n_part = ceil_div(M_out, SL);
    WSIS_REQUIRE(p.NB == 1 && p.ZS == 1, "in-launch statistics finish: plan without slabs expected");
#if WSIS_EXPERIMENTAL
    WSIS_REQUIRE(d_ws && ws_bytes >= wsis_spconv_fwd_f_workspace_bytes(M_out, K, Cin, Cout), "workspace too small");
#else
    return fail(WSIS_ERR_ARG, "in-launch statistics finish: EXPERIMENTAL build only");
#endif
    fin.G = bn_fin_chunks(n_part);
    fin.per = (int)ceil_div(n_part, fin.G);
    WSIS_REQUIRE((int64_t)(fin.G + 1) * (Cout / 32) <= (int64_t)(sizeof(SyncSlot::fin) / sizeof(unsigned)), "too many tickets");
    fin.chunk = reinterpret_cast<double*>((reinterpret_cast<uintptr_t>(d_ws) + 255) & ~(uintptr_t)255);
    fin.tickets = static_cast<SyncSlot*>(d_sync)->fin;
    fin.n_targets = n_targets;
    for (int i = 0; i < n_targets; ++i) {
      WSIS_REQUIRE(targets[i].mean && targets[i].var, "statistics target without mean / var");
      WSIS_REQUIRE((targets[i].running_mean == nullptr) == (targets[i].running_var == nullptr), "running stats come in pairs");
      fin.mean[i] = targets[i].mean;
      fin.var[i] = targets[i].var;
      fin.rmean[i] = targets[i].running_mean;
      fin.rvar[i] = targets[i].running_var;
      fin.momentum[i] = targets[i].momentum;
    }
  }
  hipStream_t st = as_stream(stream);
  const int64_t n_items = form2_items(p, M_out, Cout);
  WSIS_REQUIRE(n_items < ((int64_t)1 << 31), "too many work items");
  const dim3 grid((unsigned)n_items, 1u, 1u);
  static int n_cu = 0;
  if (!n_cu) {
    int dev = 0, v = 0;
    WSIS_HIP_CHECK(hipGetDevice(&dev));
    WSIS_HIP_CHECK(hipDeviceGetAttribute(&v, hipDeviceAttributeMultiprocessorCount, dev));
    n_cu = v > 0 ? v : 256;
  }
  const Form2 form = form2(p, M_out, Cout, d_nbr != nullptr, bn_in != nullptr, M_in);
  const int deal_band = form.xcd_run > 0 ? -form.xcd_run : tune_int("WSIS_FWD2_SNAKE", 1) ? n_cu : 0x7fffffff;
  const char* deal_env = tune_env("WSIS_FWD2_DEAL");
  const int flip_deal = (flip ? 1 : 0) | (((deal_env ? atoi(deal_env) : 0) != 0 && p.ZS == 1) ? 2 : 0);
  ProfScope prof(0, st, true);
#if WSIS_EXPERIMENTAL
  if (!bn_in && n_targets == 0 && !fused) {
    const int nt = spconv_ring_plan(M_out, K, Cin, Cout);
    if (nt) {
      const int rc = spconv_ring_launch(nt, d_X, d_nbr, d_order, d_WT, flip ? 1 : 0, d_bias, d_residual, d_out, d_stats, &epi,
                                        d_sync ? &static_cast<SyncSlot*>(d_sync)->err : nullptr, M_in, M_out, K, Cin, Cout, prof.ka(), prof.kb(), st);
      if (rc != WSIS_OK) return rc;
      prof.stop();
      WSIS_LAUNCH_CHECK();
      return WSIS_OK;
    }
  }
  {
    const char* pe = getenv("WSIS_FWD2P");
    const int fwd2p = pe ? atoi(pe) : 0;
    static int cus = 0;
    if (!cus) {
      int dev = 0;
      WSIS_HIP_CHECK(hipGetDevice(&dev));
      WSIS_HIP_CHECK(hipDeviceGetAttribute(&cus, hipDeviceAttributeMultiprocessorCount, dev));
    }
    const int64_t items = ceil_div(M_out, SL) * (Cout / 32);
    const bool p_shape = fwd2p >= 2 ? (p.NW == 1 || p.NW == 2 || p.NW == 4) : (p.NW == 1 && K >= 16);
    if (fwd2p && !bn_in && n_targets == 0 && d_sync && p.NB == 1 && p.ZS == 1 && p.DA == 2 && p.BD && p_shape &&
        items < ((int64_t)1 << 30)) {
      const size_t ldsb = (size_t)HDR_BYTES + (size_t)Layout<1, 2, true>::WAVE_BYTES * p.NW + 16;
      int per_cu = (int)((size_t)160 * 1024 / ldsb);
      const int wave_cap = 12 / p.NW > 0 ? 12 / p.NW : 1;
      if (per_cu > wave_cap) per_cu = wave_cap;
      const int64_t resident = (int64_t)cus * per_cu;
      const char* me = tune_env("WSIS_FWD2P_MIN");
      const int64_t min_pct = me ? atoi(me) : (fwd2p >= 2 ? 110 : 400);
      if (items * 100 >= resident * min_pct) {
        unsigned* q = static_cast<SyncSlot*>(d_sync)->fin;
        const int gx = (int)ceil_div(M_out, SL);
#define WSIS_F2P(nw)                                                                                                   \
  do {                                                                                                                 \
    static bool attr = false;                                                                                          \
    if (!attr) {                                                                                                       \
      WSIS_HIP_CHECK(hipFuncSetAttribute((const void*)spconv_fwd2p_kernel<nw>, hipFuncAttributeMaxDynamicSharedMemorySize, \
                                         (int)ldsb));                                                                  \
      attr = true;                                                                                                     \
    }                                                                                                                  \
    hipExtLaunchKernelGGL((spconv_fwd2p_kernel<nw>), dim3((unsigned)resident), dim3(64 * nw), (uint32_t)ldsb, st,      \
                          prof.ka(), prof.kb(), 0u, d_X, d_nbr, d_order, d_WT, d_bias, d_residual, d_out, M_out, K, Cin, \
                          Cout, flip_deal, x_bytes, d_stats, epi, q, (int)items, gx);                                  \
  } while (0)
        if (p.NW == 1)
          WSIS_F2P(1);
        else if (p.NW == 2)
          WSIS_F2P(2);
        else
          WSIS_F2P(4);
#undef WSIS_F2P
        prof.stop();
        WSIS_LAUNCH_CHECK();
        return WSIS_OK;
      }
    }
  }
#endif
#define WSIS_F2Y(nb, nw, da, bd, fb, tr)                                                                         \
  do {                                                                                                           \
    const size_t ldsb = (size_t)((tr) ? HDR_TR_BYTES : HDR_BYTES) + (size_t)Layout<nb, da, bd>::WAVE_BYTES * nw + \
                        (fb ? (size_t)Cin * 12 : 0);                                                             \
    static size_t attr_set = 0;                                                                                  \
    if (attr_set < ldsb) {                                                                                       \
      WSIS_HIP_CHECK(hipFuncSetAttribute((const void*)spconv_fwd2_kernel<nb, nw, da, bd, false, fb, tr>,         \
                                         hipFuncAttributeMaxDynamicSharedMemorySize, (int)ldsb));               \
      attr_set = ldsb;                                                                                           \
    }                                                                                                            \
    hipExtLaunchKernelGGL((spconv_fwd2_kernel<nb, nw, da, bd, false, fb, tr>), grid, dim3(64 * nw), (uint32_t)ldsb, st, \
                          prof.ka(), prof.kb(), 0u, d_X, d_nbr, d_order, d_WT, d_bias, d_residual, d_out, partial,   \
                          M_out, K, Cin, Cout, flip_deal, x_bytes, d_stats, epi, bin, fin, (int)p.ZS, deal_band,    \
                          (unsigned long long*)nullptr);                                                            \
  } while (0)
#define WSIS_F2X(nb, nw, da, bd, fb) WSIS_F2Y(nb, nw, da, bd, fb, false)
#if WSIS_EXPERIMENTAL
#define WSIS_F2RG()            \
  do {                                                                                                           \
    const size_t ldsb = (size_t)HDR_BYTES + (fin.chunk ? (size_t)Layout<1, 2, true>::WAVE_BYTES : (size_t)RG_SCRATCH_BYTES); \
    hipExtLaunchKernelGGL((spconv_fwd2rg_kernel<false>), grid, dim3(64), (uint32_t)ldsb, st, \
                          prof.ka(), prof.kb(), 0u, d_X, d_nbr, d_order, d_WT, d_bias, d_residual, d_out, partial,   \
// ... 184 lines not shown
```

### 3d-wsis_amd/csrc/spconv2_body.h

```cpp
#pragma once
#include <cstdlib>
#include <cstdlib>
#include <type_traits>

#include "common.h"

using namespace wsis;

typedef float f32x16 __attribute__((ext_vector_type(16)));
typedef float f32x4 __attribute__((ext_vector_type(4)));

namespace {

constexpr int SL = 32;
constexpr int KMAX = 32;
constexpr int DB = 2;
constexpr int A_BYTES = SL * 128;
constexpr int HDR_BYTES = (KMAX + 2) * 128;
constexpr int HDR_TR_BYTES = 256;
constexpr int RG_SCRATCH_BYTES = 1024;

__device__ __attribute__((aligned(256))) float g_zero_row[64];

template <int NB, int DA, bool BD>
// ... 88 lines not shown
    for (int64_t b0 = lo; b0 < hi; b0 += 8) {
      float sf[4], qf[4];
#pragma unroll
      for (int i = 0; i < 4; ++i) {
        const int64_t b = b0 + ph * 4 + i;
        const int64_t bb = b < hi ? b : lo;
        sf[i] = ld_sc1(stats + (bb * 2 + 0) * Cout + c);
        qf[i] = ld_sc1(stats + (bb * 2 + 1) * Cout + c);
      }
#pragma unroll
      for (int i = 0; i < 4; ++i) {
        const int64_t b = b0 + ph * 4 + i;
        if (b < hi) {
          const int64_t left = M_out - b * 32;
          const double si = sf[i];
          s[i] += si;
          q[i] += qf[i];
          w[i] += si * si * (left < 32 ? 1.0 / (double)left : 0.03125);
        }
      }
    }
#pragma unroll
    for (int i = 0; i < 4; ++i) {
      red[(0 * 8 + ph * 4 + i) * 32 + cl] = s[i];
      red[(1 * 8 + ph * 4 + i) * 32 + cl] = q[i];
      red[(2 * 8 + ph * 4 + i) * 32 + cl] = w[i];
    }
    asm volatile("s_waitcnt lgkmcnt(0)" ::: "memory");
#pragma unroll
    for (int j = 0; j < 8; ++j) {
      S += red[(0 * 8 + j) * 32 + cl];
      Q += red[(1 * 8 + j) * 32 + cl];
      W += red[(2 * 8 + j) * 32 + cl];
    }
  }
  const int G = fin.G;
  if (G > 1) {
    double* o = fin.chunk + ((int64_t)g0 * CB + cbk) * 96;
    if (ph == 0) {
      st_sc1(o + cl, S);
      st_sc1(o + 32 + cl, Q);
      st_sc1(o + 64 + cl, W);
    }
    asm volatile("s_waitcnt vmcnt(0)" ::: "memory");
    int last2 = 0;
    if (lane == 0) {
      unsigned* tk = fin.tickets + G * CB + cbk;
      const unsigned t = atomicAdd(tk, 1u);
      last2 = t == (unsigned)G - 1u;
      if (last2) __hip_atomic_store(tk, 0u, __ATOMIC_RELAXED, __HIP_MEMORY_SCOPE_AGENT);
    }
    last2 = __builtin_amdgcn_readfirstlane(last2);
    if (!last2) return;
    double s2[4] = {0.0, 0.0, 0.0, 0.0}, q2[4] = {0.0, 0.0, 0.0, 0.0}, w2[4] = {0.0, 0.0, 0.0, 0.0};
    asm volatile("s_waitcnt lgkmcnt(0)" ::: "memory");
#pragma unroll
    for (int i = 0; i < 4; ++i) {
      for (int g = ph * 4 + i; g < G; g += 8) {
        const double* oc = fin.chunk + ((int64_t)g * CB + cbk) * 96;
        s2[i] += ld_sc1(oc + cl);
        q2[i] += ld_sc1(oc + 32 + cl);
        w2[i] += ld_sc1(oc + 64 + cl);
      }
    }
#pragma unroll
    for (int i = 0; i < 4; ++i) {
      red[(0 * 8 + ph * 4 + i) * 32 + cl] = s2[i];
      red[(1 * 8 + ph * 4 + i) * 32 + cl] = q2[i];
      red[(2 * 8 + ph * 4 + i) * 32 + cl] = w2[i];
    }
    asm volatile("s_waitcnt lgkmcnt(0)" ::: "memory");
    S = Q = W = 0.0;
#pragma unroll
    for (int j = 0; j < 8; ++j) {
      S += red[(0 * 8 + j) * 32 + cl];
      Q += red[(1 * 8 + j) * 32 + cl];
      W += red[(2 * 8 + j) * 32 + cl];
    }
  }
  if (ph == 0 && c < Cout) {
    for (int tg = 0; tg < fin.n_targets; ++tg)
      bn_finish_centred(S, Q, W, M_out, c, fin.mean[tg], fin.var[tg], fin.rmean[tg], fin.rvar[tg], fin.momentum[tg]);
  }
}

struct WgSync {
  __device__ __forceinline__ void operator()() const { __syncthreads(); }
};

struct LateVals {
  const float* bias_;
  const float* residual_;
  float* out_;
  float* partial_;
  float* stats_;
  BnEpi epi_;
  __device__ __forceinline__ const float* bias() const { return bias_; }
  __device__ __forceinline__ const float* residual() const { return residual_; }
  __device__ __forceinline__ float* out() const { return out_; }
  __device__ __forceinline__ float* partial() const { return partial_; }
  __device__ __forceinline__ float* stats() const { return stats_; }
  __device__ __forceinline__ BnEpi epi() const { return epi_; }
};

__device__ __forceinline__ int rg_min_steps(int flip_deal) {
  const int m = (flip_deal >> 8) & 255;
  return m ? m : 0x00ffffff;
}

template <int NB, int NW, int DA, bool BD, bool DIAG, bool FB, bool WT, bool TR = false, bool RG = false, bool RGH = false,
          typename Sync, typename Late>
__device__ __forceinline__ void fwd2_body(
    const float* __restrict__ X, const int32_t* __restrict__ nbrS, const int32_t* __restrict__ order,
    const float* __restrict__ WTp, const Late late, int64_t M_out, int K, int Cin, int Cout, int flip_deal,
    uint32_t x_bytes, const BnIn& bin, const StatFin* const finp,
    unsigned long long* __restrict__ dbg, const int bx, const int by, const int bz, const int gy, const int gz,
    unsigned char* const lds, const int tid, Sync& sync) {
  static_assert(!FB || (BD && NB == 1), "the fused input BatchNorm is built for the weights-to-registers form");
  static_assert(!TR || (BD && NB == 1 && NW == 1 && (DA == 2 || DA == 3) && !FB),
                "table entries in registers: the one-wave form only");
  static_assert(!RG || (BD && NB == 1 && NW == 1 && DA == 2 && !FB && !TR), "gathered rows to registers: the one-wave form only");
  static_assert(!RGH || TR, "the per-item choice of the walk lives in the table-in-registers kernel");
  const int flip = flip_deal & 1;
  const bool deal_active = (flip_deal & 2) != 0;
  unsigned long long d_t0 = 0, d_r0 = 0, d_t1 = 0, d_t2 = 0;
  if (DIAG) {
    d_r0 = __builtin_amdgcn_s_memrealtime();
    d_t0 = __builtin_amdgcn_s_memtime();
  }
  using L = Layout<NB, DA, BD>;
  const int lane = tid & 63;
  const int wave = __builtin_amdgcn_readfirstlane(tid >> 6);
  const int r31 = lane & 31, half = lane >> 5;
  constexpr int HDR = TR ? HDR_TR_BYTES : HDR_BYTES;
  int32_t* const nbT = reinterpret_cast<int32_t*>(TR ? lds + HDR_TR_BYTES : lds);
  int32_t* const rowId = TR ? reinterpret_cast<int32_t*>(lds) : nbT + KMAX * 32;
  unsigned char* const Aring = lds + HDR + wave * L::WAVE_BYTES;
  unsigned char* const Bring = Aring + DA * A_BYTES;
  float* const coef = reinterpret_cast<float*>(lds + HDR + NW * L::WAVE_BYTES);
  if (FB) {
    for (int c = lane; c < Cin; c += 64) {
      coef[c] = bin.mean[c];
      coef[Cin + c] = (bin.gamma ? bin.gamma[c] : 1.0f) * rsqrtf(bin.var[c] + bin.eps);
      coef[2 * Cin + c] = bin.beta ? bin.beta[c] : 0.0f;
    }
  }

  const int64_t t0 = (int64_t)bx * SL;
  const int col0 = by * (NB * 32);
  const int nchunk = Cin >> 5;

  const int64_t t = t0 + r31;
  const uint32_t a_pitch32 = (uint32_t)Cin * 4u;
  int32_t my_row = -1;
  if (t < M_out) my_row = order ? order[t] : (int32_t)t;
  uint32_t mask = 0u;
  {
    int32_t v[KMAX / 2];
    const int32_t* tab = nbrS ? nbrS : order;
#pragma unroll
    for (int j = 0; j < KMAX / 2; ++j) {
      const int k = 2 * j + half;
      const bool ok = k < K && t < M_out && nbrS != nullptr;
      v[j] = tab ? tab[ok ? (int64_t)k * M_out + t : 0] : 0;
    }
#pragma unroll
// ... 497 lines not shown
      for (int i = 0; i < 4; ++i) issueA1(gA, nb, aS, i);
      gen_next(gA);
      aS = aS + 1 == DA ? 0 : aS + 1;
    };
    auto issueB = [&]() {
#pragma unroll
      for (int i = 0; i < 4 * NB; ++i) issueB1(gB, bS, i);
      gen_next(gB);
      bS ^= 1;
    };
    f32x4 a0[4], a1[4], b0[NB][4], b1[NB][4];
    issueA();
    if (BD) {
      loadB(gB, b0);
      gen_next(gB);
      issueA();
    } else {
      issueB();
      issueA();
      issueB();
    }
    if (DA >= 3) issueA();
    asm volatile("s_waitcnt vmcnt(%0)" ::"n"(VM_PRE) : "memory");
    readfrag(0, 0, a0, b0);
    int arS = 1, brS = 1;
    auto iter = [&](const f32x4 (&ac)[4], const f32x4 (&bc)[NB][4], f32x4 (&an)[4], f32x4 (&bn)[NB][4]) {
      asm volatile("s_waitcnt vmcnt(%0)\n\ts_waitcnt lgkmcnt(0)" ::"n"(VM_TOP) : "memory");
      __builtin_amdgcn_sched_barrier(0);
      mfma(ac, bc, 0, 4);
      __builtin_amdgcn_sched_barrier(0);
      readfrag(arS, brS, an, bn);
      arS = arS + 1 == DA ? 0 : arS + 1;
      brS ^= 1;
      loadNb(gA, nb);
      __builtin_amdgcn_sched_barrier(0);
      if (BD) {
        loadB(gB, bn);
        __builtin_amdgcn_sched_barrier(0);
        mfma(ac, bc, 4, 8);
        __builtin_amdgcn_sched_barrier(0);
      } else {
#pragma unroll
        for (int i = 0; i < 4 * NB; ++i) {
          issueB1(gB, bS, i);
          if (i % NB == NB - 1) {
            __builtin_amdgcn_sched_barrier(0);
            mfma(ac, bc, 4 + i / NB, 5 + i / NB);
            __builtin_amdgcn_sched_barrier(0);
          }
        }
        bS ^= 1;
      }
      gen_next(gB);
#pragma unroll
      for (int i = 0; i < 4; ++i) {
        issueA1(gA, nb, aS, i);
        __builtin_amdgcn_sched_barrier(0);
        mfma(ac, bc, 8 + i, 9 + i);
        __builtin_amdgcn_sched_barrier(0);
      }
      gen_next(gA);
      aS = aS + 1 == DA ? 0 : aS + 1;
      mfma(ac, bc, 12, 16);
    };
    for (int s = 0; s < T; s += 2) {
      iter(a0, b0, a1, b1);
      if (s + 1 < T) iter(a1, b1, a0, b0);
    }
  }
  asm volatile("s_waitcnt vmcnt(0) lgkmcnt(0)" ::: "memory");
  if (DIAG) d_t2 = __builtin_amdgcn_s_memtime();

  const float* bias = late.bias();
  const float* residual = late.residual();
  float* const stats = late.stats();
  const BnEpi epi = late.epi();
  const bool final_pass = gz == 1;
  float* const dst = final_pass ? late.out() : late.partial() + (int64_t)bz * M_out * Cout;
  if (!final_pass) {
    bias = nullptr;
    residual = nullptr;
  }
  if (NW == 1) {
    auto store_tile = [&](auto has_res) {
#pragma unroll
      for (int cb = 0; cb < NB; ++cb) {
        const int c = col0 + cb * 32 + r31;
        const float bv = bias ? bias[c] : 0.0f;
        int32_t rows[16];
        float val[16];
#pragma unroll
        for (int reg = 0; reg < 16; ++reg) rows[reg] = rowId[(reg & 3) + 8 * (reg >> 2) + 4 * half];
        if (decltype(has_res)::value) {
          float rv[16];
#pragma unroll
          for (int reg = 0; reg < 16; ++reg)
            rv[reg] = residual[(int64_t)(rows[reg] >= 0 ? rows[reg] : 0) * Cout + c];
#pragma unroll
          for (int reg = 0; reg < 16; ++reg) val[reg] = (acc[cb][reg] + bv) + rv[reg];
        } else {
#pragma unroll
          for (int reg = 0; reg < 16; ++reg) val[reg] = acc[cb][reg] + bv;
        }
#pragma unroll
        for (int reg = 0; reg < 16; ++reg) asm volatile("" : "+v"(val[reg]));
#pragma unroll
        for (int reg = 0; reg < 16; ++reg)
          if (rows[reg] >= 0) {
            if (WT)
              st_sc1(dst + (int64_t)rows[reg] * Cout + c, val[reg]);
            else
              dst[(int64_t)rows[reg] * Cout + c] = val[reg];
          }
        if (stats && final_pass && epi.x) {
          const BnCoef kc = bn_coef(epi, c);
          float xv[16];
#pragma unroll
          for (int reg = 0; reg < 16; ++reg) xv[reg] = epi.x[(int64_t)(rows[reg] >= 0 ? rows[reg] : 0) * Cout + c];
          float sa = 0.0f, sb = 0.0f;
#pragma unroll
          for (int reg = 0; reg < 16; ++reg) {
            float dz, dzx;
            bn_terms(kc, epi.relu, val[reg], xv[reg], dz, dzx);
            sa += rows[reg] >= 0 ? dz : 0.0f;
            sb += rows[reg] >= 0 ? dzx : 0.0f;
          }
          sa += __shfl_xor(sa, 32, 64);
          sb += __shfl_xor(sb, 32, 64);
          if (half == 0) {
            if (WT) {
              st_sc1(stats + ((int64_t)bx * 2 + 0) * Cout + c, sa);
              st_sc1(stats + ((int64_t)bx * 2 + 1) * Cout + c, sb);
            } else {
              stats[((int64_t)bx * 2 + 0) * Cout + c] = sa;
              stats[((int64_t)bx * 2 + 1) * Cout + c] = sb;
            }
          }
        } else if (stats && final_pass) {
          float sa = 0.0f, sb = 0.0f;
#pragma unroll
          for (int reg = 0; reg < 16; ++reg) sa += rows[reg] >= 0 ? val[reg] : 0.0f;
          sa += __shfl_xor(sa, 32, 64);
          const int64_t left = M_out - t0;
          const float mean_s = sa / (float)(left < SL ? left : SL);
#pragma unroll
          for (int reg = 0; reg < 16; ++reg) {
            const float d = rows[reg] >= 0 ? val[reg] - mean_s : 0.0f;
            sb += d * d;
          }
          sb += __shfl_xor(sb, 32, 64);
          if (half == 0) {
            st_sc1(stats + ((int64_t)bx * 2 + 0) * Cout + c, sa);
            st_sc1(stats + ((int64_t)bx * 2 + 1) * Cout + c, sb);
          }
          if (NB == 1 && finp && finp->chunk)
            stat_finish(*finp, stats, M_out, Cout, (int64_t)bx, col0, gy, by,
                        reinterpret_cast<double*>(Aring));
        }
      }
    };
    if (residual)
      store_tile(std::true_type{});
    else
      store_tile(std::false_type{});
  } else {
    const int32_t* rowId0 = rowId;
    constexpr int PER = (32 * NB * 32) / (64 * NW);
    float keep[PER];
    bool live[PER];
    float sa = 0.0f, sq = 0.0f;
    const bool bn_mode = stats && final_pass && epi.x;
    BnCoef kc = {0.0f, 0.0f, 0.0f, 0.0f};
    const int cc = (int)(tid % (NB * 32)), c = col0 + cc;
    if (bn_mode) kc = bn_coef(epi, c);
    const float bv = bias ? bias[c] : 0.0f;
    int64_t off[PER];
    float rv[PER], xv[PER];
#pragma unroll
    for (int it = 0; it < PER; ++it) {
      const int rr = (tid + it * 64 * NW) / (NB * 32);
      const int32_t r = rowId0[rr];
      live[it] = r >= 0;
      off[it] = (int64_t)(r >= 0 ? r : 0) * Cout + c;
    }
#pragma unroll
    for (int it = 0; it < PER; ++it) rv[it] = residual ? residual[off[it]] : 0.0f;
#pragma unroll
    for (int it = 0; it < PER; ++it) xv[it] = bn_mode ? epi.x[off[it]] : 0.0f;
    float* red = reinterpret_cast<float*>(Aring);
#pragma unroll
    for (int cb = 0; cb < NB; ++cb)
#pragma unroll
      for (int reg = 0; reg < 16; ++reg) {
        const int rr = (reg & 3) + 8 * (reg >> 2) + 4 * half;
        red[rr * (NB * 32) + cb * 32 + r31] = acc[cb][reg];
      }
    sync();
#pragma unroll
    for (int it = 0; it < PER; ++it) {
      const int e = tid + it * 64 * NW;
      float v = 0.0f;
#pragma unroll
      for (int w = 0; w < NW; ++w)
        v += reinterpret_cast<const float*>(lds + HDR + w * L::WAVE_BYTES)[e];
      if (bias) v += bv;
      if (residual) v += rv[it];
      keep[it] = live[it] ? v : 0.0f;
      if (live[it]) {
        if (WT)
          st_sc1(dst + off[it], v);
        else
          dst[off[it]] = v;
      }
      if (bn_mode) {
        float dz, dzx;
        bn_terms(kc, epi.relu, v, xv[it], dz, dzx);
        sa += live[it] ? dz : 0.0f;
        sq += live[it] ? dzx : 0.0f;
      } else {
        sa += live[it] ? v : 0.0f;
      }
    }
    if (bn_mode) {
      sync();
      float* sred = reinterpret_cast<float*>(lds + HDR);
      const int colw = NB * 32;
      sred[tid] = sa;
      sred[64 * NW + tid] = sq;
      sync();
      if (tid < colw) {
        float ta = 0.0f, tb = 0.0f;
        for (int j = tid; j < 64 * NW; j += colw) {
          ta += sred[j];
          tb += sred[64 * NW + j];
        }
        const int c = col0 + tid;
        if (WT) {
          st_sc1(stats + ((int64_t)bx * 2 + 0) * Cout + c, ta);
          st_sc1(stats + ((int64_t)bx * 2 + 1) * Cout + c, tb);
        } else {
          stats[((int64_t)bx * 2 + 0) * Cout + c] = ta;
          stats[((int64_t)bx * 2 + 1) * Cout + c] = tb;
        }
      }
    } else if (stats && final_pass) {
      sync();
      float* sred = reinterpret_cast<float*>(lds + HDR);
// ... 258 lines not shown
```

### include/wsis_hip.h

```cpp
#ifndef WSIS_HIP_H_
#define WSIS_HIP_H_

#include <stdint.h>

#ifdef __cplusplus
extern "C" {
#endif

#define WSIS_ABI_VERSION 2

#define WSIS_OK 0
#define WSIS_ERR_ARG (-1)
#define WSIS_ERR_HIP (-2)
#define WSIS_ERR_OVERFLOW (-3)


int wsis_host_version(void);
const char* wsis_host_last_error(void);

int wsis_host_voxelize_idx_map(const int64_t* h_coords, int64_t N, int32_t* h_p2v, int64_t* M,
                               int32_t* max_active);
int wsis_host_voxelize_idx_fill(const int64_t* h_coords, int64_t N, const int32_t* h_p2v, int64_t M,
                                int32_t max_active, int64_t* h_voxel_locs, int32_t* h_v2p);

// ... 1 lines not shown
                                const int32_t* h_start_len, int64_t N, int32_t threshold,
                                int32_t* h_point_cluster, int32_t* h_order, int64_t* n_clusters,
                                int64_t* n_points);
int wsis_host_bfs_cluster_fill(const int32_t* h_point_cluster, const int32_t* h_order, int64_t N,
                               int64_t n_clusters, int64_t n_points, int32_t* h_cluster_idxs,
                               int32_t* h_cluster_offsets);

int wsis_host_graph_bfs(const int32_t* h_label, const uint8_t* h_class_valid, int32_t n_class,
                        const float* h_centre, const float* h_ins_size, const int32_t* h_adj_off,
                        const int32_t* h_adj, int64_t S, int32_t* h_group, int64_t* n_groups);


int wsis_version(void);
const char* wsis_last_error(void);
int wsis_device_count(void);

int wsis_voxelize_fwd(const float* d_feats, const int32_t* d_v2p, float* d_out, int64_t M, int32_t C,
                      int32_t stride, int32_t mode, void* stream);
int wsis_voxelize_bwd(const float* d_dout, const int32_t* d_v2p, float* d_dfeats, int64_t M, int32_t C,
                      int32_t stride, int32_t mode, void* stream);

int64_t wsis_voxelize_idx_workspace_bytes(int64_t N);
int wsis_voxelize_idx_map(const int64_t* d_coords, int64_t N, int32_t* d_p2v, int32_t* d_counts2, void* d_ws,
                          int64_t ws_bytes, void* stream);
int wsis_voxelize_idx_fill(const int64_t* d_coords, int64_t N, int64_t M, int32_t max_active,
                           int64_t* d_voxel_locs, int32_t* d_v2p, void* d_ws, int64_t ws_bytes, void* stream);

int wsis_hash_build(const int32_t* d_indices, int64_t M, const int32_t* h_shape3, int64_t* d_keys,
                    int32_t* d_vals, int64_t cap, void* stream);
int wsis_rulebook_subm(const int32_t* d_indices, int64_t M, const int32_t* h_shape3,
                       const int32_t* h_ksize3, const int32_t* h_pad3, const int64_t* d_keys,
                       const int32_t* d_vals, int64_t cap, int32_t* d_nbr, uint32_t* d_mask,
                       void* stream);
int64_t wsis_rulebook_down_ncand(int64_t M_in, const int32_t* h_ksize3, const int32_t* h_stride3,
                                 const int32_t* h_pad3);
int64_t wsis_rulebook_down_workspace_bytes(int64_t n_cand);
int wsis_rulebook_down_keys(const int32_t* d_indices_in, int64_t M_in, const int32_t* h_in_shape3,
                            const int32_t* h_out_shape3, const int32_t* h_ksize3,
                            const int32_t* h_stride3, const int32_t* h_pad3, int64_t* d_cand,
                            int64_t* d_out_keys, int32_t* d_count, void* d_ws, int64_t ws_bytes,
                            void* stream);
int wsis_rulebook_down_fill(const int32_t* d_indices_in, int64_t M_in, const int32_t* h_in_shape3,
                            const int32_t* h_out_shape3, const int32_t* h_ksize3,
                            const int32_t* h_stride3, const int32_t* h_pad3,
                            const int64_t* d_out_keys, int64_t M_out, int32_t* d_indices_out,
                            int64_t* d_keys, int32_t* d_vals, int64_t cap, int32_t* d_nbr_down,
                            int32_t* d_nbr_up, uint32_t* d_mask_down, uint32_t* d_mask_up,
                            void* stream);
int64_t wsis_mask_order_workspace_bytes(int64_t M);
int64_t wsis_tile_order_workspace_bytes(int64_t M);
int wsis_tile_order(const int32_t* d_indices, const uint32_t* d_mask, int64_t M, int32_t block_shift,
                    int32_t* d_order, void* d_ws, int64_t ws_bytes, void* stream);
int wsis_mask_order(const uint32_t* d_mask, int64_t M, int32_t* d_order, void* d_ws, int64_t ws_bytes,
                    void* stream);
int64_t wsis_tile_order_batch_workspace_bytes(int64_t N);
int wsis_tile_order_batch(int32_t n, const void* const* h_indices, const void* const* h_mask, const int64_t* h_M,
                          int32_t block_shift, int32_t batch_size, int32_t* d_order_all, void* d_ws,
                          int64_t ws_bytes, void* stream);

int wsis_rulebook_pack(const int32_t* d_nbr, const int32_t* d_order, int32_t* d_nbr_packed, int64_t M,
                       int32_t K, void* stream);
int wsis_rulebook_pack_batch(int32_t n, const void* const* h_nbr, const void* const* h_order,
                             void* const* h_nbr_packed, const int64_t* h_M, const int32_t* h_K, void* stream);

enum {
  WSIS_PYR_ROWS = 0, WSIS_PYR_CAP, WSIS_PYR_INDICES, WSIS_PYR_KEYS, WSIS_PYR_VALS, WSIS_PYR_SUBM_NBR, WSIS_PYR_SUBM_MASK,
  WSIS_PYR_SUBM_ORDER, WSIS_PYR_SUBM_NBR_P, WSIS_PYR_CAND, WSIS_PYR_OUT_KEYS, WSIS_PYR_COUNT, WSIS_PYR_DOWN_WS,
  WSIS_PYR_DOWN_NBR, WSIS_PYR_UP_NBR, WSIS_PYR_DOWN_MASK, WSIS_PYR_UP_MASK, WSIS_PYR_DOWN_ORDER, WSIS_PYR_UP_ORDER,
  WSIS_PYR_DOWN_NBR_P, WSIS_PYR_UP_NBR_P, WSIS_PYR_FIELDS
};
int64_t wsis_rulebook_pyramid_layout(int64_t M0, const int64_t* h_counts, int32_t n_levels, int64_t* h_layout);
int wsis_rulebook_pyramid(const int32_t* d_indices0, int64_t M0, const int32_t* h_shape3, const int64_t* h_counts,
                          int32_t n_levels, int32_t batch_size, int32_t block_shift, void* d_arena, int64_t arena_bytes,
                          void* stream);

int64_t wsis_spconv_fwd_workspace_bytes(int64_t M_out, int32_t K, int32_t Cin, int32_t Cout);
int wsis_spconv_fwd(const float* d_X, const int32_t* d_nbr, const int32_t* d_order, const float* d_W,
                    const float* d_bias, const float* d_residual, float* d_out, int64_t M_in,
                    int64_t M_out, int32_t K, int32_t Cin, int32_t Cout, void* d_ws, int64_t ws_bytes,
                    void* stream);
int32_t wsis_spconv_fwd_t_supported(int32_t K, int32_t Cin, int32_t Cout);
int32_t wsis_spconv_fwd_t_slabs(int64_t M_out, int32_t K, int32_t Cin, int32_t Cout);
int64_t wsis_spconv_fwd_t_workspace_bytes(int64_t M_out, int32_t K, int32_t Cin, int32_t Cout);
int wsis_spconv_fwd_t(const float* d_X, const int32_t* d_nbr, const int32_t* d_order, const float* d_WT, int32_t flip,
                      const float* d_bias, const float* d_residual, float* d_out, float* d_stats, int64_t M_in,
                      int64_t M_out, int32_t K, int32_t Cin, int32_t Cout, void* d_ws, int64_t ws_bytes,
                      void* d_sync, void* stream);
int wsis_spconv_fwd_t_bn(const float* d_X, const int32_t* d_nbr, const int32_t* d_order, const float* d_WT, int32_t flip,
                         float* d_out, float* d_partials, const float* d_bn_x, const float* d_bn_mean,
                         const float* d_bn_var, const float* d_bn_gamma, const float* d_bn_beta, float eps, int32_t relu,
                         int64_t M_in, int64_t M_out, int32_t K, int32_t Cin, int32_t Cout, void* d_ws, int64_t ws_bytes,
                         void* d_sync, void* stream);
typedef struct wsis_bn_in {
  const float* mean;
  const float* var;
  const float* gamma;
  const float* beta;
  float eps;
  int32_t relu;
} wsis_bn_in;
typedef struct wsis_stat_target {
  float* mean;
  float* var;
  float* running_mean;
  float* running_var;
  float momentum;
  int32_t reserved;
} wsis_stat_target;
#if defined(WSIS_EXPERIMENTAL) && WSIS_EXPERIMENTAL
int64_t wsis_spconv_fwd_f_workspace_bytes(int64_t M_out, int32_t K, int32_t Cin, int32_t Cout);
int wsis_spconv_fwd_f(const float* d_X, const wsis_bn_in* bn_in, const int32_t* d_nbr, const int32_t* d_order,
                      const float* d_WT, int32_t flip, const float* d_bias, const float* d_residual, float* d_out,
                      float* d_stats, const wsis_stat_target* targets, int32_t n_targets, int64_t M_in, int64_t M_out,
                      int32_t K, int32_t Cin, int32_t Cout, void* d_ws, int64_t ws_bytes, void* d_sync, void* stream);
#endif
int wsis_weight_transpose(const float* d_W, float* d_WT, int32_t K, int32_t Cin, int32_t Cout,
                          int32_t flip, void* stream);
int64_t wsis_spconv_dw_workspace_bytes(int64_t M_out, int32_t K, int32_t Cin, int32_t Cout);
int wsis_spconv_dw(const float* d_X, const int32_t* d_nbr, const int32_t* d_order, const float* d_dY,
                   float* d_dW, int64_t M_in, int64_t M_out, int32_t K, int32_t Cin, int32_t Cout, void* d_ws,
                   int64_t ws_bytes, void* stream);

int32_t wsis_spconv_lp_supported(int32_t K, int32_t Cin, int32_t Cout);
int32_t wsis_spconv_lp_plan(int64_t M_out, int32_t K, int32_t Cin, int32_t Cout, int32_t* out);
int64_t wsis_spconv_fwd_lp_workspace_bytes(int64_t M_out, int32_t K, int32_t Cin, int32_t Cout);
int wsis_spconv_fwd_lp(const void* d_X, const int32_t* d_nbr, const int32_t* d_order, const void* d_WT, int32_t flip,
                       const float* d_bias, void* d_out, int64_t M_in, int64_t M_out, int32_t K, int32_t Cin,
                       int32_t Cout, int32_t dtype, void* d_ws, int64_t ws_bytes, void* stream);
int wsis_spconv_fwd_lp_res(const void* d_X, const int32_t* d_nbr, const int32_t* d_order, const void* d_WT,
                           int32_t flip, const float* d_bias, const void* d_residual, void* d_out, int64_t M_in,
                           int64_t M_out, int32_t K, int32_t Cin, int32_t Cout, int32_t dtype, void* d_ws,
                           int64_t ws_bytes, void* stream);
int64_t wsis_spconv_dw_lp_workspace_bytes(int64_t M_out, int32_t K, int32_t Cin, int32_t Cout);
int wsis_spconv_dw_lp(const void* d_X, const int32_t* d_nbr, const int32_t* d_order, const void* d_dY, float* d_dW,
                      int64_t M_in, int64_t M_out, int32_t K, int32_t Cin, int32_t Cout, int32_t dtype, void* d_ws,
                      int64_t ws_bytes, void* stream);
int wsis_weight_cast_lp(const float* d_W, void* d_out, int32_t K, int32_t Cin, int32_t Cout, int32_t transpose,
                        int32_t flip, int32_t dtype, void* stream);

int32_t wsis_spconv_dw_bn_supported(int32_t K, int32_t Cin, int32_t Cout);
int64_t wsis_spconv_dw_bn_workspace_bytes(int64_t M_in, int32_t K, int32_t Cin, int32_t Cout);
int wsis_spconv_dw_bn(const float* d_X, const float* d_mean, const float* d_var, const float* d_gamma,
                      const float* d_beta, float eps, int32_t relu, const int32_t* d_nbr_b, const int32_t* d_order_b,
                      int32_t flip, const float* d_dY, float* d_dW, int64_t M_in, int64_t M_out, int32_t K, int32_t Cin,
                      int32_t Cout, void* d_ws, int64_t ws_bytes, void* stream);

int wsis_prof_enable(int32_t on);
int wsis_prof_summary(int32_t which, double* total_ms, int64_t* launches);
int wsis_prof_records(int32_t which, double* h_main_ms, double* h_total_ms, int64_t cap, int64_t* n);

int64_t wsis_sync_bytes(void);

int64_t wsis_bn_workspace_bytes(int64_t M, int32_t C);
int wsis_bn_stats(const float* d_x, int64_t M, int32_t C, float* d_mean, float* d_var, float* d_running_mean,
                  float* d_running_var, float momentum, void* d_ws, int64_t ws_bytes, void* stream);
int64_t wsis_bn_stats_finalize_workspace_bytes(int64_t n_part, int32_t C);
int wsis_bn_stats_finalize(const float* d_partials, int64_t n_part, int64_t M, int32_t C, float* d_mean, float* d_var,
                           float* d_running_mean, float* d_running_var, float momentum, void* d_ws, int64_t ws_bytes,
                           void* d_sync, void* stream);
int wsis_bn_stats_finalize_apply(const float* d_partials, int64_t n_part, int64_t M, int32_t C, float* d_mean,
                                 float* d_var, float* d_running_mean, float* d_running_var, float momentum,
                                 const float* d_x, const float* d_gamma, const float* d_beta, float eps, int32_t relu,
                                 float* d_y, void* d_ws, int64_t ws_bytes, void* d_sync, void* stream);
int wsis_bn_bwd_from_partials(const float* d_partials, int64_t n_part, const float* d_x, const float* d_dy,
                              const float* d_mean, const float* d_var, const float* d_gamma, const float* d_beta,
                              float eps, int32_t relu, float* d_dx, float* d_dgamma, float* d_dbeta,
// ... 315 lines not shown
```

Baseline: 134.7 scenes/s.

## Write BN backward dx directly into two split destinations and add row-product spconv path

BN backward apply kernels gain a split-destination mode that writes the first Ca columns of dx to one buffer and the rest to another. The executor can then send BN gradients straight into the concat-split halves instead of copying them afterwards. A separate single-wave row-product spconv kernel with a double-buffered LDS pipeline is also added, but its mode flag defaults off and is only reachable through a debug entry. The split store adds per-element branch and index math, and it disables the experimental fused finish path.

After: 135.6 scenes/s, median of 4. No clear change (+0.6%).

```diff
diff --git a/3d-wsis_amd/csrc/bn.hip b/3d-wsis_amd/csrc/bn.hip
--- a/3d-wsis_amd/csrc/bn.hip
+++ b/3d-wsis_amd/csrc/bn.hip
@@ -616,13 +616,38 @@
                        gamma, beta, eps, relu, static_cast<TI*>(y), M, C);
 }
 
-template <bool COHERENT, typename T, typename TO>
+template <typename TO>
+struct BnSplitDst {
+  TO *a, *b;
+  int Ca, quad;
+};
+template <typename TO>
+__device__ __forceinline__ void bn_split_store(const BnSplitDst<TO>& s, int64_t row, int c, int C, int W,
+                                               const float (&o)[4]) {
+  const int Cb = C - s.Ca;
+  if (W == 4 && s.quad) {
+    bn_st4(c < s.Ca ? s.a + row * s.Ca + c : s.b + row * Cb + (c - s.Ca), 0, make_float4(o[0], o[1], o[2], o[3]));
+    return;
+  }
+#pragma unroll
+  for (int e = 0; e < 4; ++e)
+    if (e < W) {
+      const int ce = c + e;
+      if (ce < s.Ca)
+        s.a[row * s.Ca + ce] = (TO)o[e];
+      else
+        s.b[row * Cb + (ce - s.Ca)] = (TO)o[e];
+    }
+}
+
+template <bool COHERENT, bool SPLIT, typename T, typename TO>
 __device__ __forceinline__ void bn_bwd_apply_body(const T* __restrict__ x, const T* __restrict__ dy,
                                                   const float* __restrict__ mean, const float* __restrict__ var,
                                                   const float* __restrict__ gamma, const float* __restrict__ beta,
                                                   const float* dgamma, const float* dbeta,
                                                   const T* __restrict__ addend, float eps, int relu, int training,
-                                                  TO* __restrict__ dx, int64_t M, int C) {
+                                                  TO* __restrict__ dx, int64_t M, int C,
+                                                  const BnSplitDst<TO> split = BnSplitDst<TO>{}) {
   const int64_t total = M * C;
   const float inv_m = 1.0f / (float)M;
   const bool vec = (C & 3) == 0;
@@ -653,6 +678,13 @@
         ov[e] = bn_bwd_dx(bn_bwd_elem(xv[e], dv[e], k, e, relu), k, e, k1[e], k2[e], training, addend != nullptr, av[e]);
     }
   };
+  auto put4 = [&](int64_t q, const float (&o)[4]) {
+    if (SPLIT) {
+      const RowCol rc = row_col(q, (int)Cw, totalw);
+      bn_split_store(split, rc.row, rc.col * 4, C, 4, o);
+    } else
+      bn_st4(dx, q, make_float4(o[0], o[1], o[2], o[3]));
+  };
   if (vec && fixed_c) {
     for (; t + stride < totalw; t += 2 * stride) {
       const int64_t u = t + stride;
@@ -668,8 +700,8 @@
       float o0[4], o1[4];
       one(tx0.v, td0.v, ta0.v, o0);
       one(tx1.v, td1.v, ta1.v, o1);
-      bn_st4(dx, t, make_float4(o0[0], o0[1], o0[2], o0[3]));
-      bn_st4(dx, u, make_float4(o1[0], o1[1], o1[2], o1[3]));
+      put4(t, o0);
+      put4(u, o1);
     }
   }
   for (; t < totalw; t += stride) {
@@ -694,8 +726,11 @@
     }
     one(xv, dv, av, ov);
     if (vec)
-      bn_st4(dx, t, make_float4(ov[0], ov[1], ov[2], ov[3]));
-    else
+      put4(t, ov);
+    else if (SPLIT) {
+      const RowCol rc = row_col(t, C, total);
+      bn_split_store(split, rc.row, rc.col, C, 1, ov);
+    } else
       dx[t] = (TO)ov[0];
   }
 }
@@ -707,7 +742,17 @@
                                     const float* __restrict__ dgamma, const float* __restrict__ dbeta,
                                     const T* __restrict__ addend, float eps, int relu, int training,
                                     TO* __restrict__ dx, int64_t M, int C) {
-  bn_bwd_apply_body<false>(x, dy, mean, var, gamma, beta, dgamma, dbeta, addend, eps, relu, training, dx, M, C);
+  bn_bwd_apply_body<false, false>(x, dy, mean, var, gamma, beta, dgamma, dbeta, addend, eps, relu, training, dx, M, C);
+}
+template <typename T, typename TO>
+__global__ void bn_bwd_apply_split_kernel(const T* __restrict__ x, const T* __restrict__ dy,
+                                          const float* __restrict__ mean, const float* __restrict__ var,
+                                          const float* __restrict__ gamma, const float* __restrict__ beta,
+                                          const float* __restrict__ dgamma, const float* __restrict__ dbeta,
+                                          const T* __restrict__ addend, float eps, int relu, int training,
+                                          BnSplitDst<TO> split, int64_t M, int C) {
+  bn_bwd_apply_body<false, true>(x, dy, mean, var, gamma, beta, dgamma, dbeta, addend, eps, relu, training, (TO*)nullptr, M,
+                                 C, split);
 }
 
 constexpr int BN_SF_ROWS = 256;
@@ -786,7 +831,8 @@
     const float* __restrict__ partial, int nblk, int C, int64_t M, const float* __restrict__ x,
     const float* __restrict__ dy, const float* __restrict__ mean, const float* __restrict__ var,
     const float* __restrict__ gamma, const float* __restrict__ beta, const float* __restrict__ addend, float eps, int relu,
-    float* __restrict__ dx, float* __restrict__ dgamma, float* __restrict__ dbeta, int G) {
+    float* __restrict__ dx, float* __restrict__ dgamma, float* __restrict__ dbeta, int G,
+    const BnSplitDst<float> split) {
   __shared__ double red[2][8][33];
   __shared__ float s_k1[32], s_k2[32];
   const int cgi = blockIdx.y;
@@ -831,7 +877,10 @@
 #pragma unroll
       for (int e = 0; e < 4; ++e)
         ov[e] = bn_bwd_dx(bn_bwd_elem(xv[e], dv[e], k, e, relu), k, e, k1[e], k2[e], 1, addend != nullptr, av[e]);
-      *reinterpret_cast<float4*>(dx + r * C + c4) = make_float4(ov[0], ov[1], ov[2], ov[3]);
+      if (split.a)
+        bn_split_store(split, r, c4, C, 4, ov);
+      else
+        *reinterpret_cast<float4*>(dx + r * C + c4) = make_float4(ov[0], ov[1], ov[2], ov[3]);
     }
   }
 }
@@ -913,7 +962,7 @@
                                   (int)blockIdx.x / G, red, s_last),
                sync, CG);
   bn_wait_published(sync);
-  bn_bwd_apply_body<true>(x, dy, mean, var, gamma, beta, dgamma, dbeta, addend, eps, relu, 1, dx, M, C);
+  bn_bwd_apply_body<true, false>(x, dy, mean, var, gamma, beta, dgamma, dbeta, addend, eps, relu, 1, dx, M, C);
 }
 
 static int bn_fused_grid(int64_t M, int C, int need_chunk_wgs, int which = 0) {
@@ -966,9 +1015,13 @@
 static int launch_bn_bwd_apply(const T* d_x, const T* d_dy, const float* d_mean, const float* d_var,
                                const float* d_gamma, const float* d_beta, const float* d_dgamma, const float* d_dbeta,
                                const T* d_addend, float eps, int relu, int training, TO* d_dx, int64_t M, int C,
-                               hipStream_t st) {
-  hipLaunchKernelGGL((bn_bwd_apply_kernel<T, TO>), dim3(bn_apply_grid(M, C)), dim3(256), 0, st, d_x, d_dy, d_mean, d_var,
-                     d_gamma, d_beta, d_dgamma, d_dbeta, d_addend, eps, relu, training, d_dx, M, C);
+                               hipStream_t st, const BnSplitDst<TO>& split = BnSplitDst<TO>{}) {
+  if (split.a)
+    hipLaunchKernelGGL((bn_bwd_apply_split_kernel<T, TO>), dim3(bn_apply_grid(M, C)), dim3(256), 0, st, d_x, d_dy, d_mean,
+                       d_var, d_gamma, d_beta, d_dgamma, d_dbeta, d_addend, eps, relu, training, split, M, C);
+  else
+    hipLaunchKernelGGL((bn_bwd_apply_kernel<T, TO>), dim3(bn_apply_grid(M, C)), dim3(256), 0, st, d_x, d_dy, d_mean, d_var,
+                       d_gamma, d_beta, d_dgamma, d_dbeta, d_addend, eps, relu, training, d_dx, M, C);
   WSIS_LAUNCH_CHECK();
   return WSIS_OK;
 }
@@ -1045,6 +1098,15 @@
 }
 static void* bn_align256(void* p) {
   return reinterpret_cast<void*>((reinterpret_cast<uintptr_t>(p) + 255) & ~(uintptr_t)255);
+}
+static BnSplitDst<float> bn_split_dst(float* d_dx, const BnSplit& s) {
+  BnSplitDst<float> d{};
+  if (!s.dx2) return d;
+  d.a = d_dx;
+  d.b = s.dx2;
+  d.Ca = s.Ca;
+  d.quad = (s.Ca % 4 == 0 && bn_aligned16({d_dx, s.dx2})) ? 1 : 0;
+  return d;
 }
 
 struct BnCentredPlan {
@@ -1274,21 +1336,34 @@
                               float eps, int32_t relu, float* d_dx, float* d_dgamma, float* d_dbeta,
                               const float* d_addend, int64_t M, int32_t C, void* d_ws, int64_t ws_bytes, void* d_sync,
                               void* stream) {
+  return bn_bwd_from_partials_run(d_partials, n_part, d_x, d_dy, d_mean, d_var, d_gamma, d_beta, eps, relu, d_dx, d_dgamma,
+                                  d_dbeta, d_addend, M, C, d_ws, ws_bytes, d_sync, stream, BnSplit{});
+}
+
+}
+
+int wsis::bn_bwd_from_partials_run(const float* d_partials, int64_t n_part, const float* d_x, const float* d_dy,
+                                   const float* d_mean, const float* d_var, const float* d_gamma, const float* d_beta,
+                                   float eps, int32_t relu, float* d_dx, float* d_dgamma, float* d_dbeta,
+                                   const float* d_addend, int64_t M, int32_t C, void* d_ws, int64_t ws_bytes, void* d_sync,
+                                   void* stream, const BnSplit& split) {
   WSIS_REQUIRE(M >= 1 && C >= 1 && d_partials && d_x && d_dy && d_mean && d_var && d_dgamma && d_dbeta, "bad args");
   WSIS_REQUIRE(n_part == (M + 31) / 32 && n_part < ((int64_t)1 << 31), "one partial per 32-row slice");
+  WSIS_REQUIRE(!split.dx2 || (d_dx && split.Ca >= 1 && split.Ca < C), "two destinations need dx and a column inside the row");
   const BnCentredPlan p = bn_centred_plan(n_part, C, d_ws, ws_bytes, d_sync);
   WSIS_REQUIRE(p.ws_ok, "workspace too small");
   hipStream_t st = as_stream(stream);
   WSIS_REQUIRE(C <= 512, "more than 512 channels");
-  if (d_dx && bn_small_fused_ok(p, C, {d_x, d_dy, d_dx, d_addend})) {
+  const BnSplitDst<float> sd = bn_split_dst(d_dx, split);
+  if (d_dx && bn_small_fused_ok(p, C, {d_x, d_dy, sd.a ? nullptr : d_dx, d_addend})) {
     hipLaunchKernelGGL(bn_small_bwd_finish_apply_kernel, dim3((unsigned)ceil_div(M, BN_SF_ROWS), (unsigned)p.CG), dim3(256),
                        0, st, d_partials, (int)n_part, (int)C, M, d_x, d_dy, d_mean, d_var, d_gamma, d_beta, d_addend, eps,
-                       (int)relu, d_dx, d_dgamma, d_dbeta, p.G);
+                       (int)relu, d_dx, d_dgamma, d_dbeta, p.G, sd);
     WSIS_LAUNCH_CHECK();
     return WSIS_OK;
   }
 #if WSIS_EXPERIMENTAL
-  if (const int grid = d_dx && p.tickets ? bn_fused_grid(M, C, p.G * p.CG, 1) : 0) {
+  if (const int grid = d_dx && !sd.a && p.tickets ? bn_fused_grid(M, C, p.G * p.CG, 1) : 0) {
     hipLaunchKernelGGL(bn_bwd_finish_apply_kernel, dim3(grid), dim3(256), 0, st, d_partials, (int)n_part, (int)C, p.chunk,
                        p.G, d_dbeta, d_dgamma, static_cast<SyncSlot*>(d_sync), d_x, d_dy, d_mean, d_var, d_gamma, d_beta,
                        d_addend, eps, (int)relu, d_dx, M);
@@ -1305,8 +1380,24 @@
   }
   if (!d_dx) return WSIS_OK;
   return launch_bn_bwd_apply(d_x, d_dy, d_mean, d_var, d_gamma, d_beta, d_dgamma, d_dbeta, d_addend, eps, relu, 1, d_dx, M,
-                             C, st);
-}
+                             C, st, sd);
+}
+
+int wsis::bn_bwd_run(const float* d_x, const float* d_dy, const float* d_mean, const float* d_var, const float* d_gamma,
+                     const float* d_beta, float eps, int32_t relu, int32_t training, float* d_dx, float* d_dgamma,
+                     float* d_dbeta, const float* d_addend, int64_t M, int32_t C, void* d_ws, int64_t ws_bytes, void* stream,
+                     const BnSplit& split) {
+  WSIS_REQUIRE(M >= 1 && C >= 1 && d_x && d_dy && d_mean && d_var && d_dgamma && d_dbeta && d_ws, "bad args");
+  WSIS_REQUIRE(ws_bytes >= wsis_bn_workspace_bytes(M, C), "workspace too small");
+  WSIS_REQUIRE(!split.dx2 || (d_dx && split.Ca >= 1 && split.Ca < C), "two destinations need dx and a column inside the row");
+  hipStream_t st = as_stream(stream);
+  const int rc = bn_bwd_reduce_run(d_x, d_dy, d_mean, d_var, d_gamma, d_beta, eps, relu, d_dgamma, d_dbeta, M, C, d_ws, st);
+  if (rc != WSIS_OK || !d_dx) return rc;
+  return launch_bn_bwd_apply(d_x, d_dy, d_mean, d_var, d_gamma, d_beta, d_dgamma, d_dbeta, d_addend, eps, relu, training,
+                             d_dx, M, C, st, bn_split_dst(d_dx, split));
+}
+
+extern "C" {
 
 int wsis_bn_bwd_apply(const float* d_x, const float* d_dy, const float* d_mean, const float* d_var,
                       const float* d_gamma, const float* d_beta, const float* d_sum_dz_xhat, const float* d_sum_dz,
@@ -1320,13 +1411,8 @@
                 const float* d_gamma, const float* d_beta, float eps, int32_t relu, int32_t training,
                 float* d_dx, float* d_dgamma, float* d_dbeta, const float* d_addend, int64_t M, int32_t C, void* d_ws,
                 int64_t ws_bytes, void* stream) {
-  WSIS_REQUIRE(M >= 1 && C >= 1 && d_x && d_dy && d_mean && d_var && d_dgamma && d_dbeta && d_ws, "bad args");
-  WSIS_REQUIRE(ws_bytes >= wsis_bn_workspace_bytes(M, C), "workspace too small");
-  hipStream_t st = as_stream(stream);
-  const int rc = bn_bwd_reduce_run(d_x, d_dy, d_mean, d_var, d_gamma, d_beta, eps, relu, d_dgamma, d_dbeta, M, C, d_ws, st);
-  if (rc != WSIS_OK || !d_dx) return rc;
-  return launch_bn_bwd_apply(d_x, d_dy, d_mean, d_var, d_gamma, d_beta, d_dgamma, d_dbeta, d_addend, eps, relu, training,
-                             d_dx, M, C, st);
+  return bn_bwd_run(d_x, d_dy, d_mean, d_var, d_gamma, d_beta, eps, relu, training, d_dx, d_dgamma, d_dbeta, d_addend, M, C,
+                    d_ws, ws_bytes, stream, BnSplit{});
 }
 
 int wsis_bn_bwd_lp(const void* d_x, const void* d_dy, const float* d_mean, const float* d_var, const float* d_gamma,
diff --git a/3d-wsis_amd/csrc/common.h b/3d-wsis_amd/csrc/common.h
--- a/3d-wsis_amd/csrc/common.h
+++ b/3d-wsis_amd/csrc/common.h
@@ -165,6 +165,18 @@
   return (int)g;
 }
 
+struct BnSplit {
+  float* dx2 = nullptr;
+  int Ca = 0;
+};
+int bn_bwd_from_partials_run(const float* d_partials, int64_t n_part, const float* d_x, const float* d_dy, const float* d_mean,
+                             const float* d_var, const float* d_gamma, const float* d_beta, float eps, int32_t relu,
+                             float* d_dx, float* d_dgamma, float* d_dbeta, const float* d_addend, int64_t M, int32_t C,
+                             void* d_ws, int64_t ws_bytes, void* d_sync, void* stream, const BnSplit& split);
+int bn_bwd_run(const float* d_x, const float* d_dy, const float* d_mean, const float* d_var, const float* d_gamma,
+               const float* d_beta, float eps, int32_t relu, int32_t training, float* d_dx, float* d_dgamma, float* d_dbeta,
+               const float* d_addend, int64_t M, int32_t C, void* d_ws, int64_t ws_bytes, void* stream, const BnSplit& split);
+
 bool spconv_in_supported(int K, int Cin, int Cout);
 int spconv_in_launch(const float* d_X, const int32_t* d_nbr, const int32_t* d_order, const float* d_W, const float* d_bias,
                      const float* d_residual, float* d_out, int64_t M_out, hipEvent_t ka, hipEvent_t kb, hipStream_t st);
@@ -178,6 +190,12 @@
                        const float* d_bias, const float* d_residual, float* d_out, float* d_stats, const void* epi,
                        unsigned* d_err, int64_t M_in, int64_t M_out, int K, int Cin, int Cout, hipEvent_t ka, hipEvent_t kb, hipStream_t st,
                        unsigned long long* d_dbg = nullptr);
+
+bool spconv_row_takes(bool one_src, bool has_table, int K, bool has_stats, int NW, int ZS, int64_t items);
+int spconv_row_launch(const float* d_X, const int32_t* d_nbr, const int32_t* d_order, const float* d_WT, int flip,
+                      const float* d_bias, const float* d_residual, float* d_out, float* d_stats, const void* epi,
+                      int64_t M_out, int K, int Cin, int Cout, uint32_t x_bytes, hipEvent_t ka, hipEvent_t kb,
+                      hipStream_t st);
 
 bool dw2_supported(int K, int Cin, int Cout);
 bool dw2_fits(int64_t M_in, int64_t M_out, int K, int Cin, int Cout);
diff --git a/3d-wsis_amd/csrc/executor.hip b/3d-wsis_amd/csrc/executor.hip
--- a/3d-wsis_amd/csrc/executor.hip
+++ b/3d-wsis_amd/csrc/executor.hip
@@ -297,11 +297,13 @@
   bool wt_side;
   bool dw_early;
   bool slab_bn_partials;
+  bool bn_split;
   bool prof;
   bool capturing;
   bool dw_defer() const { return dw_batch_reduce && !prof; }
 };
 inline bool env_flag(const char* e, bool dflt) { return e ? atoi(e) != 0 : dflt; }
+bool g_bn_split_on = true;
 PassOptions read_pass_options(const hipStream_t* st) {
   PassOptions o;
   o.fwd2 = env_flag(getenv("WSIS_FWD2"), true);
@@ -313,6 +315,7 @@
   const char* rows = getenv("WSIS_DW_EARLY_ROWS");
   o.dw_early = env_flag(getenv("WSIS_DW_EARLY"), dw2_batch_rows() < (rows ? atoll(rows) : 500000));
   o.slab_bn_partials = env_flag(getenv("WSIS_SLAB_BN_PARTIALS"), false);
+  o.bn_split = g_bn_split_on;
   o.prof = g_prof_on;
   hipStreamCaptureStatus cs = hipStreamCaptureStatusNone;
   o.capturing = st && (hipStreamIsCapturing(*st, &cs) != hipSuccess || cs != hipStreamCaptureStatusNone);
@@ -443,10 +446,37 @@
   return -1;
 }
 
+inline bool ranges_overlap(const void* a, int64_t a_bytes, const void* b, int64_t b_bytes) {
+  if (!a || !b) return false;
+  const uintptr_t a0 = reinterpret_cast<uintptr_t>(a), b0 = reinterpret_cast<uintptr_t>(b);
+  return a0 < b0 + (uintptr_t)b_bytes && b0 < a0 + (uintptr_t)a_bytes;
+}
+bool bn_feeds_split(const wsis_op* ops, int n, int i) {
+  if (i + 1 >= n) return false;
+  const wsis_op &bn = ops[i], &sp = ops[i + 1];
+  if (bn.kind != WSIS_OP_BN_RELU_BWD || sp.kind != WSIS_OP_SPLIT || ((bn.flags | sp.flags) & WSIS_OPF_LP)) return false;
+  if (!bn.out[0] || sp.in[0] != bn.out[0] || !sp.out[0] || !sp.out[1]) return false;
+  if (bn.M_in < 1 || sp.M_in != bn.M_in || sp.Cin < 1 || sp.Cout < 1 || sp.Cin + sp.Cout != bn.Cin) return false;
+  for (int j = 0; j < n; ++j) {
+    if (j == i + 1) continue;
+    for (const void* p : ops[j].in)
+      if (p == bn.out[0]) return false;
+    for (int k = 0; k < 8; ++k)
+      if (ops[j].out[k] == bn.out[0] && !(j == i && k == 0)) return false;
+  }
+  const int64_t full = bn.M_in * bn.Cin * 4;
+  const void* reads[3] = {bn.in[0], bn.in[1], bn.in[6]};
+  for (const void* p : reads)
+    if (ranges_overlap(p, full, sp.out[0], sp.M_in * sp.Cin * 4) || ranges_overlap(p, full, sp.out[1], sp.M_in * sp.Cout * 4))
+      return false;
+  return !ranges_overlap(sp.out[0], sp.M_in * sp.Cin * 4, sp.out[1], sp.M_in * sp.Cout * 4);
+}
+
 struct PassPlan {
   enum { LP, WT, DW, DEEP, OP, REGIONS };
   int64_t at[REGIONS], bytes[REGIONS], total = 0;
   std::vector<int64_t> lp_off, wt_off;
+  std::vector<char> bn_split;
   int64_t dw_max = 0;
   int n_dw = 0;
 };
@@ -470,6 +500,7 @@
   int dw_next = 0, dw_flushed = 0;
   int64_t dw_off = 0;
   std::vector<char> bn_unfused;
+  std::vector<char> split_done;
 
   char* region(int k) const { return base + plan.at[k]; }
   const float* wt_of(int i) const { return reinterpret_cast<const float*>(region(PassPlan::WT) + plan.wt_off[i]); }
@@ -770,6 +801,7 @@
 
 int deep_issue_run(PassRun& r, int i, int* next) {
   *next = i;
+  if (r.split_done[i]) return WSIS_OK;
   if (r.plan.bytes[PassPlan::DEEP] == 0 || !r.d_sync || r.opt.capturing || !deep_op_ok(r.ops, r.n, i, r.opt.fwd2)) return WSIS_OK;
   const int i1 = deep_run_end(r.ops, r.n, i, r.mark_op >= i ? r.mark_op : -1, r.opt.fwd2);
   if (i1 - i < kDeepMinOps) return WSIS_OK;
@@ -855,9 +887,11 @@
 int plan_pass(const wsis_op* ops, int n, const PassOptions& o, PassPlan& p) {
   p.lp_off.assign(n, -1);
   p.wt_off.assign(n, -1);
+  p.bn_split.assign(n, 0);
   int64_t lp = 0, wt = 0, dw_sum = 0, need = ALIGN;
   for (int i = 0; i < n; ++i) {
     const wsis_op& op = ops[i];
+    p.bn_split[i] = (o.bn_split && bn_feeds_split(ops, n, i)) ? 1 : 0;
     const char* why = lp_refusal(op);
     if (why) return fail(WSIS_ERR_ARG, "wsis_run_ops: op %d: %s", i, why);
     int64_t b = op_ws_bytes(op, o.fwd2);
@@ -940,6 +974,7 @@
   if (use_worker && hipGetDevice(&cur_dev) != hipSuccess) return fail(WSIS_ERR_HIP, "hipGetDevice failed");
   dw_recs.resize((size_t)(opt.dw_defer() ? plan.n_dw : 0));
   bn_unfused.assign(n, 0);
+  split_done.assign(n, 0);
   return launch_weight_batches<uint16_t>(ops, n, plan.lp_off, region(PassPlan::LP), st);
 }
 
@@ -1196,8 +1231,8 @@
   return launch_status();
 }
 
-int issue_split(PassRun& r, const wsis_op& op, int) {
-  if (op.M_in <= 0) return WSIS_OK;
+int issue_split(PassRun& r, const wsis_op& op, int i) {
+  if (op.M_in <= 0 || r.split_done[i]) return WSIS_OK;
   wsis_op c = op;
   if (is_lp(op)) {
     c.Cin /= 2;
@@ -1261,6 +1296,15 @@
 int issue_bn_relu_bwd(PassRun& r, const wsis_op& op, int i) {
   ProfScope prof(2, r.st);
   int rc;
+  BnSplit split;
+  float* dx = (float*)op.out[0];
+  if (r.plan.bn_split[i]) {
+    const wsis_op& sp = r.ops[i + 1];
+    dx = (float*)sp.out[0];
+    split.dx2 = (float*)sp.out[1];
+    split.Ca = sp.Cin;
+    r.split_done[i + 1] = 1;
+  }
   if (is_lp(op)) {
     rc = op.M_in <= 0 ? WSIS_OK
                       : wsis_bn_bwd_lp(op.in[0], op.in[1], (const float*)op.in[2], (const float*)op.in[3],
@@ -1272,16 +1316,16 @@
     if (!op.in[7] || !(op.flags & WSIS_OPF_TRAINING))
       rc = fail(WSIS_ERR_ARG, "op %d: BatchNorm backward from partials needs in[7] and training mode", i);
     else
-      rc = wsis_bn_bwd_from_partials((const float*)op.in[7], (op.M_in + 31) / 32, (const float*)op.in[0],
-                                     (const float*)op.in[1], (const float*)op.in[2], (const float*)op.in[3],
-                                     (const float*)op.in[4], (const float*)op.in[5], op.eps, relu_of(op), (float*)op.out[0],
-                                     (float*)op.out[1], (float*)op.out[2], (const float*)op.in[6], op.M_in, op.Cin, r.ws,
-                                     r.ws_bytes, sync_slot(r.d_sync, i), r.stream);
+      rc = bn_bwd_from_partials_run((const float*)op.in[7], (op.M_in + 31) / 32, (const float*)op.in[0],
+                                    (const float*)op.in[1], (const float*)op.in[2], (const float*)op.in[3],
+                                    (const float*)op.in[4], (const float*)op.in[5], op.eps, relu_of(op), dx,
+                                    (float*)op.out[1], (float*)op.out[2], (const float*)op.in[6], op.M_in, op.Cin, r.ws,
+                                    r.ws_bytes, sync_slot(r.d_sync, i), r.stream, split);
   } else {
-    rc = wsis_bn_bwd((const float*)op.in[0], (const float*)op.in[1], (const float*)op.in[2], (const float*)op.in[3],
-                     (const float*)op.in[4], (const float*)op.in[5], op.eps, relu_of(op),
-                     (op.flags & WSIS_OPF_TRAINING) ? 1 : 0, (float*)op.out[0], (float*)op.out[1], (float*)op.out[2],
-                     (const float*)op.in[6], op.M_in, op.Cin, r.ws, r.ws_bytes, r.stream);
+    rc = bn_bwd_run((const float*)op.in[0], (const float*)op.in[1], (const float*)op.in[2], (const float*)op.in[3],
+                    (const float*)op.in[4], (const float*)op.in[5], op.eps, relu_of(op),
+                    (op.flags & WSIS_OPF_TRAINING) ? 1 : 0, dx, (float*)op.out[1], (float*)op.out[2],
+                    (const float*)op.in[6], op.M_in, op.Cin, r.ws, r.ws_bytes, r.stream, split);
   }
   prof.stop();
   return rc;
@@ -1365,6 +1409,12 @@
   std::copy(plan.lp_off.begin(), plan.lp_off.end(), out + 11);
   std::copy(plan.wt_off.begin(), plan.wt_off.end(), out + 11 + n);
   return WSIS_OK;
+}
+
+int wsis_debug_bn_split_store(int on) {
+  const int old = g_bn_split_on ? 1 : 0;
+  g_bn_split_on = on != 0;
+  return old;
 }
 
 int wsis_run_ops(const wsis_op* ops, int32_t n, void* d_ws, int64_t ws_bytes, void* d_sync, void* stream) {
diff --git a/3d-wsis_amd/csrc/spconv2.hip b/3d-wsis_amd/csrc/spconv2.hip
--- a/3d-wsis_amd/csrc/spconv2.hip
+++ b/3d-wsis_amd/csrc/spconv2.hip
@@ -249,6 +249,8 @@
                              const wsis_stat_target* targets, int32_t n_targets, bool fused) {
   WSIS_REQUIRE(M_in >= 0 && M_out >= 0, "bad sizes");
   WSIS_REQUIRE(wsis_spconv_fwd_t_supported(K, Cin, Cout), "needs K <= 32 and channel counts that are multiples of 32");
+  const bool one_src = d_nbr == nullptr || (flip & WSIS_FLIP_ONE_SRC) != 0;
+  flip &= 1;
   if (M_out == 0) return WSIS_OK;
   WSIS_REQUIRE(d_X && d_WT && d_out, "null pointer");
   WSIS_REQUIRE(d_nbr || (K == 1 && M_in == M_out), "nbr may be null only for the dense 1x1 case");
@@ -315,6 +317,15 @@
   const char* deal_env = tune_env("WSIS_FWD2_DEAL");
   const int flip_deal = (flip ? 1 : 0) | (((deal_env ? atoi(deal_env) : 0) != 0 && p.ZS == 1) ? 2 : 0);
   ProfScope prof(0, st, true);
+  if (!bn_in && n_targets == 0 && !fused && spconv_row_takes(one_src, d_nbr != nullptr, K, d_stats != nullptr, p.NW, p.ZS,
+                                                                    ceil_div(M_out, SL) * (Cout / 32))) {
+    const int rc = spconv_row_launch(d_X, d_nbr, d_order, d_WT, flip, d_bias, d_residual, d_out, d_stats, &epi, M_out, K, Cin,
+                                     Cout, x_bytes, prof.ka(), prof.kb(), st);
+    if (rc != WSIS_OK) return rc;
+    prof.stop();
+    WSIS_LAUNCH_CHECK();
+    return WSIS_OK;
+  }
 #if WSIS_EXPERIMENTAL
   if (!bn_in && n_targets == 0 && !fused) {
     const int nt = spconv_ring_plan(M_out, K, Cin, Cout);
diff --git a/3d-wsis_amd/csrc/spconv2_body.h b/3d-wsis_amd/csrc/spconv2_body.h
--- a/3d-wsis_amd/csrc/spconv2_body.h
+++ b/3d-wsis_amd/csrc/spconv2_body.h
@@ -194,6 +194,94 @@
     for (int tg = 0; tg < fin.n_targets; ++tg)
       bn_finish_centred(S, Q, W, M_out, c, fin.mean[tg], fin.var[tg], fin.rmean[tg], fin.rvar[tg], fin.momentum[tg]);
   }
+}
+
+template <int NB, bool WT>
+__device__ __forceinline__ void fwd2_epilogue_1w(const f32x16 (&acc)[NB], const int32_t* const rowId, const float* bias,
+                                                 const float* residual, float* const dst, float* const stats,
+                                                 const BnEpi& epi, const bool final_pass, const StatFin* const finp,
+                                                 const int64_t M_out, const int Cout, const int64_t t0, const int bx,
+                                                 const int by, const int gy, const int col0, const int r31, const int half,
+                                                 double* const fin_red) {
+  auto store_tile = [&](auto has_res) {
+#pragma unroll
+    for (int cb = 0; cb < NB; ++cb) {
+      const int c = col0 + cb * 32 + r31;
+      const float bv = bias ? bias[c] : 0.0f;
+      int32_t rows[16];
+      float val[16];
+#pragma unroll
+      for (int reg = 0; reg < 16; ++reg) rows[reg] = rowId[(reg & 3) + 8 * (reg >> 2) + 4 * half];
+      if (decltype(has_res)::value) {
+        float rv[16];
+#pragma unroll
+        for (int reg = 0; reg < 16; ++reg)
+          rv[reg] = residual[(int64_t)(rows[reg] >= 0 ? rows[reg] : 0) * Cout + c];
+#pragma unroll
+        for (int reg = 0; reg < 16; ++reg) val[reg] = (acc[cb][reg] + bv) + rv[reg];
+      } else {
+#pragma unroll
+        for (int reg = 0; reg < 16; ++reg) val[reg] = acc[cb][reg] + bv;
+      }
+#pragma unroll
+      for (int reg = 0; reg < 16; ++reg) asm volatile("" : "+v"(val[reg]));
+#pragma unroll
+      for (int reg = 0; reg < 16; ++reg)
+        if (rows[reg] >= 0) {
+          if (WT)
+            st_sc1(dst + (int64_t)rows[reg] * Cout + c, val[reg]);
+          else
+            dst[(int64_t)rows[reg] * Cout + c] = val[reg];
+        }
+      if (stats && final_pass && epi.x) {
+        const BnCoef kc = bn_coef(epi, c);
+        float xv[16];
+#pragma unroll
+        for (int reg = 0; reg < 16; ++reg) xv[reg] = epi.x[(int64_t)(rows[reg] >= 0 ? rows[reg] : 0) * Cout + c];
+        float sa = 0.0f, sb = 0.0f;
+#pragma unroll
+        for (int reg = 0; reg < 16; ++reg) {
+          float dz, dzx;
+          bn_terms(kc, epi.relu, val[reg], xv[reg], dz, dzx);
+          sa += rows[reg] >= 0 ? dz : 0.0f;
+          sb += rows[reg] >= 0 ? dzx : 0.0f;
+        }
+        sa += __shfl_xor(sa, 32, 64);
+        sb += __shfl_xor(sb, 32, 64);
+        if (half == 0) {
+          if (WT) {
+            st_sc1(stats + ((int64_t)bx * 2 + 0) * Cout + c, sa);
+            st_sc1(stats + ((int64_t)bx * 2 + 1) * Cout + c, sb);
+          } else {
+            stats[((int64_t)bx * 2 + 0) * Cout + c] = sa;
+            stats[((int64_t)bx * 2 + 1) * Cout + c] = sb;
+          }
+        }
+      } else if (stats && final_pass) {
+        float sa = 0.0f, sb = 0.0f;
+#pragma unroll
+        for (int reg = 0; reg < 16; ++reg) sa += rows[reg] >= 0 ? val[reg] : 0.0f;
+        sa += __shfl_xor(sa, 32, 64);
+        const int64_t left = M_out - t0;
+        const float mean_s = sa / (float)(left < SL ? left : SL);
+#pragma unroll
+        for (int reg = 0; reg < 16; ++reg) {
+          const float d = rows[reg] >= 0 ? val[reg] - mean_s : 0.0f;
+          sb += d * d;
+        }
+        sb += __shfl_xor(sb, 32, 64);
+        if (half == 0) {
+          st_sc1(stats + ((int64_t)bx * 2 + 0) * Cout + c, sa);
+          st_sc1(stats + ((int64_t)bx * 2 + 1) * Cout + c, sb);
+        }
+        if (NB == 1 && finp && finp->chunk) stat_finish(*finp, stats, M_out, Cout, (int64_t)bx, col0, gy, by, fin_red);
+      }
+    }
+  };
+  if (residual)
+    store_tile(std::true_type{});
+  else
+    store_tile(std::false_type{});
 }
 
 struct WgSync {
@@ -857,87 +945,8 @@
     residual = nullptr;
   }
   if (NW == 1) {
-    auto store_tile = [&](auto has_res) {
-#pragma unroll
-      for (int cb = 0; cb < NB; ++cb) {
-        const int c = col0 + cb * 32 + r31;
-        const float bv = bias ? bias[c] : 0.0f;
-        int32_t rows[16];
-        float val[16];
-#pragma unroll
-        for (int reg = 0; reg < 16; ++reg) rows[reg] = rowId[(reg & 3) + 8 * (reg >> 2) + 4 * half];
-        if (decltype(has_res)::value) {
-          float rv[16];
-#pragma unroll
-          for (int reg = 0; reg < 16; ++reg)
-            rv[reg] = residual[(int64_t)(rows[reg] >= 0 ? rows[reg] : 0) * Cout + c];
-#pragma unroll
-          for (int reg = 0; reg < 16; ++reg) val[reg] = (acc[cb][reg] + bv) + rv[reg];
-        } else {
-#pragma unroll
-          for (int reg = 0; reg < 16; ++reg) val[reg] = acc[cb][reg] + bv;
-        }
-#pragma unroll
-        for (int reg = 0; reg < 16; ++reg) asm volatile("" : "+v"(val[reg]));
-#pragma unroll
-        for (int reg = 0; reg < 16; ++reg)
-          if (rows[reg] >= 0) {
-            if (WT)
-              st_sc1(dst + (int64_t)rows[reg] * Cout + c, val[reg]);
-            else
-              dst[(int64_t)rows[reg] * Cout + c] = val[reg];
-          }
-        if (stats && final_pass && epi.x) {
-          const BnCoef kc = bn_coef(epi, c);
-          float xv[16];
-#pragma unroll
-          for (int reg = 0; reg < 16; ++reg) xv[reg] = epi.x[(int64_t)(rows[reg] >= 0 ? rows[reg] : 0) * Cout + c];
-          float sa = 0.0f, sb = 0.0f;
-#pragma unroll
-          for (int reg = 0; reg < 16; ++reg) {
-            float dz, dzx;
-            bn_terms(kc, epi.relu, val[reg], xv[reg], dz, dzx);
-            sa += rows[reg] >= 0 ? dz : 0.0f;
-            sb += rows[reg] >= 0 ? dzx : 0.0f;
-          }
-          sa += __shfl_xor(sa, 32, 64);
-          sb += __shfl_xor(sb, 32, 64);
-          if (half == 0) {
-            if (WT) {
-              st_sc1(stats + ((int64_t)bx * 2 + 0) * Cout + c, sa);
-              st_sc1(stats + ((int64_t)bx * 2 + 1) * Cout + c, sb);
-            } else {
-              stats[((int64_t)bx * 2 + 0) * Cout + c] = sa;
-              stats[((int64_t)bx * 2 + 1) * Cout + c] = sb;
-            }
-          }
-        } else if (stats && final_pass) {
-          float sa = 0.0f, sb = 0.0f;
-#pragma unroll
-          for (int reg = 0; reg < 16; ++reg) sa += rows[reg] >= 0 ? val[reg] : 0.0f;
-          sa += __shfl_xor(sa, 32, 64);
-          const int64_t left = M_out - t0;
-          const float mean_s = sa / (float)(left < SL ? left : SL);
-#pragma unroll
-          for (int reg = 0; reg < 16; ++reg) {
-            const float d = rows[reg] >= 0 ? val[reg] - mean_s : 0.0f;
-            sb += d * d;
-          }
-          sb += __shfl_xor(sb, 32, 64);
-          if (half == 0) {
-            st_sc1(stats + ((int64_t)bx * 2 + 0) * Cout + c, sa);
-            st_sc1(stats + ((int64_t)bx * 2 + 1) * Cout + c, sb);
-          }
-          if (NB == 1 && finp && finp->chunk)
-            stat_finish(*finp, stats, M_out, Cout, (int64_t)bx, col0, gy, by,
-                        reinterpret_cast<double*>(Aring));
-        }
-      }
-    };
-    if (residual)
-      store_tile(std::true_type{});
-    else
-      store_tile(std::false_type{});
+    fwd2_epilogue_1w<NB, WT>(acc, rowId, bias, residual, dst, stats, epi, final_pass, finp, M_out, Cout, t0, bx, by, gy, col0,
+                             r31, half, reinterpret_cast<double*>(Aring));
   } else {
     const int32_t* rowId0 = rowId;
     constexpr int PER = (32 * NB * 32) / (64 * NW);
diff --git a/3d-wsis_amd/csrc/spconv_row.hip b/3d-wsis_amd/csrc/spconv_row.hip
--- /dev/null
+++ b/3d-wsis_amd/csrc/spconv_row.hip
@@ -0,0 +1,204 @@
+#include "spconv2_body.h"
+
+namespace {
+
+constexpr int ROW_KMAX = 8;
+constexpr int ROW_LDS_BYTES = 2 * A_BYTES + 128;
+constexpr int ROW_WAVES_PER_CU = 12;
+
+constexpr int64_t ROW_MIN_ITEMS = 1024;
+int g_row_mode = 0;
+long long g_row_launches = 0;
+
+typedef int32_t i32x8 __attribute__((ext_vector_type(8)));
+struct RowHdr {
+  int32_t row;
+  i32x8 v;
+};
+static_assert(ROW_KMAX == 8, "RowHdr holds eight entries");
+
+__global__ __launch_bounds__(64) void spconv_row_kernel(
+    const float* __restrict__ X, const int32_t* __restrict__ nbrS, const int32_t* __restrict__ order,
+    const float* __restrict__ WTp, const float* __restrict__ bias, const float* __restrict__ residual,
+    float* __restrict__ out, int64_t M_out, int K, int Cin, int Cout, int flip, uint32_t x_bytes,
+    float* __restrict__ stats, BnEpi epi, int n_items) {
+  extern __shared__ __attribute__((aligned(16))) unsigned char lds[];
+  const int lane = (int)threadIdx.x & 63;
+  const int r31 = lane & 31, half = lane >> 5;
+  const int d_row = lane >> 3, d_piece = lane & 7;
+  int32_t* const rowId = reinterpret_cast<int32_t*>(lds + 2 * A_BYTES);
+  const int gy = Cout >> 5, nchunk = Cin >> 5;
+  const uint32_t a_pitch32 = (uint32_t)Cin * 4u;
+  const rsrc_t rsX = __builtin_amdgcn_make_buffer_rsrc(const_cast<float*>(X), (short)0, (int)x_bytes, 0x00020000);
+  uint32_t a_po[4];
+#pragma unroll
+  for (int i = 0; i < 4; ++i) a_po[i] = (uint32_t)((d_piece ^ swz(i * 8 + d_row)) << 4);
+  const char* const Wb = reinterpret_cast<const char*>(WTp);
+
+  auto load_hdr = [&](int item) {
+    const int64_t t = (int64_t)(item / gy) * SL + r31;
+    const bool live = t < M_out;
+    const int64_t tc = live ? t : 0;
+    RowHdr h;
+    const int32_t row = order ? order[tc] : (int32_t)tc;
+    h.row = live ? row : -1;
+#pragma unroll
+    for (int k = 0; k < ROW_KMAX; ++k) {
+      const int32_t e = nbrS ? nbrS[(int64_t)(k < K ? k : 0) * M_out + tc] : row;
+      h.v[k] = (live && k < K) ? e : -1;
+    }
+    return h;
+  };
+  auto mask_of = [&](const RowHdr& h) {
+    uint32_t m = 0u;
+#pragma unroll
+    for (int k = 0; k < ROW_KMAX; ++k)
+      if (__ballot(h.v[k] >= 0) != 0ull) m |= 1u << k;
+    return (uint32_t)__builtin_amdgcn_readfirstlane((int)m);
+  };
+  auto entry_of = [&](const RowHdr& h, int k) {
+    int32_t e = h.v[0];
+#pragma unroll
+    for (int j = 1; j < ROW_KMAX; ++j) e = j == k ? h.v[j] : e;
+    return e;
+  };
+  auto issueA = [&](const RowHdr& h, int k, int c, int slot) {
+    const int32_t mine = entry_of(h, k);
+#pragma unroll
+    for (int i = 0; i < 4; ++i) {
+      const int32_t s = __shfl(mine, i * 8 + d_row, 64);
+      const uint32_t off = s >= 0 ? (uint32_t)s * a_pitch32 + a_po[i] : NO_ROW;
+      bdma16(rsX, off, (uint32_t)c * 128u, lds + slot * A_BYTES + i * 1024);
+    }
+  };
+
+  int item = (int)blockIdx.x;
+  if (item >= n_items) return;
+  const int stride = (int)gridDim.x;
+  RowHdr cur = load_hdr(item);
+  uint32_t kmask = mask_of(cur);
+  int slot = 0;
+  bool issued = false;
+  while (item < n_items) {
+    const int nxt = item + stride;
+    const bool has_next = nxt < n_items;
+    const RowHdr nh = load_hdr(has_next ? nxt : item);
+    uint32_t nmask = 0u;
+    bool nmask_known = false;
+    const int bx = item / gy, by = item - bx * gy;
+    const int col0 = by * 32;
+    if (lane < 32) rowId[lane] = cur.row;
+    f32x16 acc[1];
+#pragma unroll
+    for (int i = 0; i < 16; ++i) acc[0][i] = 0.0f;
+    if (kmask != 0u && !issued) issueA(cur, __builtin_ctz(kmask), 0, slot);
+    issued = false;
+    uint32_t rem = kmask;
+    while (rem) {
+      const int k = __builtin_ctz(rem);
+      rem &= rem - 1u;
+      const int kk = flip ? K - 1 - k : k;
+      for (int c = 0; c < nchunk; ++c) {
+        asm volatile("s_waitcnt vmcnt(0)" ::: "memory");
+        f32x4 a[4], b[4];
+        {
+          const unsigned char* arow = lds + slot * A_BYTES + r31 * 128;
+          const int sw = swz(r31);
+#pragma unroll
+          for (int q = 0; q < 4; ++q) a[q] = *reinterpret_cast<const f32x4*>(arow + (((half * 4 + q) ^ sw) << 4));
+        }
+        asm volatile("s_waitcnt lgkmcnt(0)" ::: "memory");
+        __builtin_amdgcn_sched_barrier(0);
+        {
+          const char* src = Wb + (((int64_t)kk * Cout + col0 + r31) * Cin + c * 32 + half * 16) * 4;
+          asm volatile("global_load_dwordx4 %0, %1, off" : "=v"(b[0]) : "v"(src) : "memory");
+          asm volatile("global_load_dwordx4 %0, %1, off offset:16" : "=v"(b[1]) : "v"(src) : "memory");
+          asm volatile("global_load_dwordx4 %0, %1, off offset:32" : "=v"(b[2]) : "v"(src) : "memory");
+          asm volatile("global_load_dwordx4 %0, %1, off offset:48" : "=v"(b[3]) : "v"(src) : "memory");
+        }
+        bool pieces = true;
+        __builtin_amdgcn_sched_barrier(0);
+        if (c + 1 < nchunk) {
+          issueA(cur, k, c + 1, slot ^ 1);
+        } else if (rem) {
+          issueA(cur, __builtin_ctz(rem), 0, slot ^ 1);
+        } else if (has_next) {
+          nmask = mask_of(nh);
+          nmask_known = true;
+          if (nmask != 0u) {
+            issueA(nh, __builtin_ctz(nmask), 0, slot ^ 1);
+            issued = true;
+          } else {
+            pieces = false;
+          }
+        } else {
+          pieces = false;
+        }
+        __builtin_amdgcn_sched_barrier(0);
+        if (pieces)
+          asm volatile("s_waitcnt vmcnt(4)" ::: "memory");
+        else
+          asm volatile("s_waitcnt vmcnt(0)" ::: "memory");
+        asm volatile("" : "+v"(b[0]), "+v"(b[1]), "+v"(b[2]), "+v"(b[3])::"memory");
+        __builtin_amdgcn_sched_barrier(0);
+#pragma unroll
+        for (int s = 0; s < 16; ++s)
+          acc[0] = __builtin_amdgcn_mfma_f32_32x32x2f32(a[s >> 2][s & 3], b[s >> 2][s & 3], acc[0], 0, 0, 0);
+        slot ^= 1;
+      }
+    }
+    fwd2_epilogue_1w<1, false>(acc, rowId, bias, residual, out, stats, epi, true, nullptr, M_out, Cout, (int64_t)bx * SL, bx,
+                               by, gy, col0, r31, half, nullptr);
+    if (!has_next) break;
+    kmask = nmask_known ? nmask : mask_of(nh);
+    cur = nh;
+    item = nxt;
+  }
+}
+
+}
+
+namespace wsis {
+
+bool spconv_row_takes(bool one_src, bool has_table, int K, bool has_stats, int NW, int ZS, int64_t items) {
+  if (g_row_mode == 0 || !one_src) return false;
+  if (has_table ? K > ROW_KMAX : K != 1) return false;
+  if (has_stats && !(NW == 1 && ZS == 1)) return false;
+  return g_row_mode == 2 || (!has_table && items >= ROW_MIN_ITEMS);
+}
+
+int spconv_row_launch(const float* d_X, const int32_t* d_nbr, const int32_t* d_order, const float* d_WT, int flip,
+                      const float* d_bias, const float* d_residual, float* d_out, float* d_stats, const void* epi,
+                      int64_t M_out, int K, int Cin, int Cout, uint32_t x_bytes, hipEvent_t ka, hipEvent_t kb,
+                      hipStream_t st) {
+  const int64_t items = ceil_div(M_out, SL) * (Cout / 32);
+  WSIS_REQUIRE(items >= 1 && items < ((int64_t)1 << 31), "too many work items");
+  static int n_cu = 0;
+  if (!n_cu) {
+    int dev = 0, v = 0;
+    WSIS_HIP_CHECK(hipGetDevice(&dev));
+    WSIS_HIP_CHECK(hipDeviceGetAttribute(&v, hipDeviceAttributeMultiprocessorCount, dev));
+    n_cu = v > 0 ? v : 256;
+  }
+  const int64_t cap = (int64_t)n_cu * ROW_WAVES_PER_CU;
+  const unsigned grid = (unsigned)(items < cap ? items : cap);
+  hipExtLaunchKernelGGL(spconv_row_kernel, dim3(grid), dim3(64), (uint32_t)ROW_LDS_BYTES, st, ka, kb, 0u, d_X, d_nbr, d_order,
+                        d_WT, d_bias, d_residual, d_out, M_out, K, Cin, Cout, flip ? 1 : 0, x_bytes, d_stats,
+                        *static_cast<const BnEpi*>(epi), (int)items);
+  ++g_row_launches;
+  return WSIS_OK;
+}
+
+}
+
+extern "C" {
+
+int wsis_debug_row_product(int mode) {
+  const int old = g_row_mode;
+  g_row_mode = mode < 0 ? 0 : mode > 2 ? 2 : mode;
+  return old;
+}
+
+long long wsis_debug_row_launches(void) { return g_row_launches; }
+
+}
diff --git a/include/wsis_hip.h b/include/wsis_hip.h
--- a/include/wsis_hip.h
+++ b/include/wsis_hip.h
@@ -107,6 +107,7 @@
 int32_t wsis_spconv_fwd_t_supported(int32_t K, int32_t Cin, int32_t Cout);
 int32_t wsis_spconv_fwd_t_slabs(int64_t M_out, int32_t K, int32_t Cin, int32_t Cout);
 int64_t wsis_spconv_fwd_t_workspace_bytes(int64_t M_out, int32_t K, int32_t Cin, int32_t Cout);
+enum { WSIS_FLIP_ONE_SRC = 2 };
 int wsis_spconv_fwd_t(const float* d_X, const int32_t* d_nbr, const int32_t* d_order, const float* d_WT, int32_t flip,
                       const float* d_bias, const float* d_residual, float* d_out, float* d_stats, int64_t M_in,
                       int64_t M_out, int32_t K, int32_t Cin, int32_t Cout, void* d_ws, int64_t ws_bytes,
```
